# openGemini/openGemini

Measured on NVIDIA H100. Metric: decoded+aggregated rows/s, higher is better.
Workload: dtype f64

## Files before the change

include/ogpu.h:

```cpp
#ifndef OGPU_H
#define OGPU_H

#include <stddef.h>
#include <stdint.h>

#ifdef __cplusplus
extern "C" {
#endif

#define OG_API __attribute__((visibility("default")))

enum {
    OG_OK = 0,
    OG_EOF = 1,
    OG_E_INVAL = -1,
    OG_E_CUDA = -2,
    OG_E_NOMEM = -3,
    OG_E_UNSUPPORTED = -4,
    OG_E_CORRUPT = -5,
    OG_E_ABORTED = -6,
    OG_E_TYPE = -7,
    OG_E_STATE = -8
};

enum { OG_TYPE_INT = 1, OG_TYPE_FLOAT = 3, OG_TYPE_STRING = 4, OG_TYPE_BOOL = 5 };

enum { OG_AGG_COUNT = 1, OG_AGG_SUM = 2, OG_AGG_MIN = 3, OG_AGG_MAX = 4, OG_AGG_FIRST = 5, OG_AGG_LAST = 6 };

enum { OG_F_TERM = 0, OG_F_AND = 1, OG_F_OR = 2 };
enum { OG_OP_LT = 0, OG_OP_LTE = 1, OG_OP_GT = 2, OG_OP_GTE = 3, OG_OP_EQ = 4, OG_OP_NEQ = 5 };

typedef struct og_filter_item {
    int32_t kind;
    int32_t column;
    int32_t op;
    int32_t const_is_float;
    double fval;
    int64_t ival;
} og_filter_item;

typedef struct og_call {
    int32_t func;
    int32_t column;
} og_call;

enum { OG_GROUP_ALL = 0, OG_GROUP_PER_SERIES = 1, OG_GROUP_MAP = 2 };
enum {
    OG_Q_STRICT_ORDER = 1u << 0
    ,
    OG_Q_NO_FUSED = 1u << 1
    ,
    OG_Q_NO_FAST = 1u << 2
    ,
    OG_Q_RESERVED_8 = 1u << 3
    ,
    OG_Q_QUERY_GRID = 1u << 4
};

typedef struct og_query_desc {
    int64_t interval;
    int64_t offset;
    int64_t tmin, tmax;
    int32_t ascending;
    uint32_t n_calls;
    const og_call *calls;
    uint32_t n_filter;
    const og_filter_item *filter;
    int32_t group_mode;
    uint32_t n_groups;
    const uint32_t *series_group;
    int32_t chunk_size;
    uint32_t flags;
} og_query_desc;

typedef struct og_column_desc {
    const char *name;
    int32_t type;
    const uint64_t *page_off;
    const uint32_t *page_len;
} og_column_desc;

enum {
    OG_SHARD_DEVICE_DATA = 1u << 0
};

typedef struct og_shard_desc {
    const uint8_t *data;
    uint64_t data_len;
    uint32_t n_series;
    const uint64_t *sids;
    const uint32_t *series_seg_begin;
    uint32_t n_segments;
    const int64_t *seg_tmin;
    const int64_t *seg_tmax;
    uint32_t n_columns;
    const og_column_desc *columns;
    const uint64_t *time_page_off;
    const uint32_t *time_page_len;
    uint32_t flags;
} og_shard_desc;

typedef struct og_colval_view {
    const uint8_t *val;
    uint64_t val_bytes;
    const uint8_t *bitmap;
    const int64_t *times;
    int32_t type;
    int32_t len;
    int32_t nil_count;
    int32_t bitmap_offset;
} og_colval_view;

typedef struct og_record_view {
    uint32_t n_cols;
    const og_colval_view *cols;
    const int64_t *times;
    int32_t rows;
    uint32_t group;
    uint64_t sid;
} og_record_view;

typedef struct og_dense_col {
    void *values;
    uint8_t *valid;
    int64_t *times;
    int32_t type;
    int32_t func;
} og_dense_col;

typedef struct og_dense_view {
    uint32_t n_groups;
    uint32_t n_buckets;
    int64_t start;
    int64_t interval;
    uint32_t n_cols;
    const og_dense_col *cols;
    void *stream;
} og_dense_view;

typedef struct og_stats {
    uint64_t rows_decoded;
    uint64_t segments_scanned;
    uint64_t page_bytes;
    uint64_t dir_bytes;
    uint64_t out_bytes;
    double kernel_ms;
    double h2d_ms;
    double main_kernel_ms;
    uint32_t kernel_launches;
    int32_t path;
    int32_t il_state;
    int32_t per_series_cells_used;
    double il_build_ms;
    uint64_t il_bytes;
    uint64_t general_segments;
    double merge_ms;
    uint64_t il_packed_segments;
} og_stats;

typedef struct og_shard og_shard;
typedef struct og_query og_query;

OG_API int og_init(int device_ordinal);
OG_API int og_device_count(void);
OG_API const char *og_strerror(int status);
OG_API const char *og_last_error(void);
OG_API const char *og_version(void);
OG_API int og_release_cached_memory(void);

typedef struct og_tssp og_tssp;
OG_API int og_tssp_parse(const uint8_t *file, uint64_t len, og_tssp **out);
OG_API int og_tssp_desc(const og_tssp *t, og_shard_desc *out);
OG_API const char *og_tssp_measurement(const og_tssp *t);
OG_API int og_tssp_time_range(const og_tssp *t, int64_t *min_time, int64_t *max_time);
OG_API void og_tssp_free(og_tssp *t);

OG_API int og_shard_open(const og_shard_desc *desc, og_shard **out);
OG_API void og_shard_close(og_shard *s);
OG_API int og_shard_info(const og_shard *s, uint64_t *n_series, uint64_t *n_segments, uint64_t *n_rows,
                         uint64_t *page_bytes, int64_t *tmin, int64_t *tmax);

enum { OG_FILE_OUT_OF_ORDER = 1u << 0 };
OG_API int og_shard_open_files(const og_shard_desc *files, const uint32_t *file_flags, uint32_t n_files, og_shard **out);
typedef struct og_merge_info {
    uint32_t n_files, n_out_of_order_files;
    uint64_t series_merged;
    uint64_t out_of_order_rows;
    uint64_t rows_replaced;
    uint64_t rows_after_merge;
    uint64_t segments_kept;
    uint64_t segments_rewritten_in, segments_rewritten_out;
    double merge_ms;
} og_merge_info;
OG_API int og_shard_merge_info(const og_shard *s, og_merge_info *out);

OG_API int og_shard_append_files(og_shard *s, const og_shard_desc *files, const uint32_t *file_flags, uint32_t n_files);

OG_API int og_query_create(og_shard *s, const og_query_desc *desc, og_query **out);
OG_API int og_query_run(og_query *q);
OG_API int og_query_next(og_query *q, og_record_view *out);
OG_API int og_query_dense(og_query *q, og_dense_view *out);
OG_API int og_query_stats(const og_query *q, og_stats *out);
OG_API void og_query_abort(og_query *q);
OG_API void og_query_destroy(og_query *q);

OG_API int og_query_merge_dense(og_query *q, const og_dense_view *other);

typedef struct og_comm og_comm;
OG_API int og_comm_unique_id(uint8_t id[128]);
OG_API int og_comm_init_rank(const uint8_t id[128], int rank, int world, og_comm **out);
OG_API void og_comm_destroy(og_comm *c);
OG_API int og_comm_info(const og_comm *c, int *rank, int *world, int *nccl_version);
OG_API int og_comm_allreduce_f64(og_comm *c, double *vals, int n, int op_max);
OG_API int og_query_allreduce(og_query *q, og_comm *c);

OG_API int og_decode_segment(og_shard *s, uint32_t segment, og_record_view *out);
enum { OG_DECODE_DESCENDING = 1u << 0 };
OG_API int og_decode_segment_ex(og_shard *s, uint32_t segment, uint32_t flags, og_record_view *out);
OG_API int og_decode_column_device(og_shard *s, uint32_t column, uint32_t seg_begin, uint32_t seg_end,
                                   void *d_values, uint64_t value_stride_bytes, uint32_t *d_rows_out);

enum { OG_SYNTH_F_HI = 0, OG_SYNTH_F_LO = 1, OG_SYNTH_INT_WALK = 2, OG_SYNTH_BOOL = 3 };
typedef struct og_synth_column {
    int32_t type;
    int32_t dist;
    uint32_t null_permille;
} og_synth_column;
typedef struct og_synth_desc {
    uint32_t n_series;
    uint32_t rows_per_series;
    uint32_t rows_per_segment;
    int64_t t0;
    int64_t dt;
    uint64_t seed;
    uint32_t n_columns;
    const og_synth_column *columns;
    uint32_t series_base;
} og_synth_desc;
OG_API int og_shard_synth(const og_synth_desc *desc, og_shard **out);
typedef struct og_shard_layout {
    uint64_t data_len;
    uint32_t n_series, n_segments, n_columns;
} og_shard_layout;
OG_API int og_shard_layout_get(const og_shard *s, og_shard_layout *out);
OG_API int og_shard_export(const og_shard *s, uint8_t *data, uint64_t *sids, uint32_t *series_seg_begin,
                           int64_t *seg_tmin, int64_t *seg_tmax, uint64_t *page_off ,
                           uint32_t *page_len, int32_t *col_types );

OG_API int og_encode_pages(int32_t type, int32_t is_time, const void *d_values, const uint8_t *d_valid,
                           const uint32_t *d_rows , uint32_t n_segments,
                           uint32_t rows_per_segment, uint8_t *d_out, uint64_t out_cap, uint64_t *d_page_off,
                           uint32_t *d_page_len, uint64_t *total_bytes_out);

typedef struct og_downsampled og_downsampled;
OG_API int og_downsample(og_shard *s, uint32_t column, int64_t interval, int64_t tmin, int64_t tmax, og_downsampled **out);

typedef struct og_downsample_ops {
    int32_t type;
    uint32_t n_funcs;
    const int32_t *funcs;
} og_downsample_ops;
typedef struct og_downsample_desc {
    int64_t interval, tmin, tmax;
    uint32_t n_types;
    const og_downsample_ops *ops;
} og_downsample_desc;
OG_API int og_downsample_shard(og_shard *s, const og_downsample_desc *d, og_downsampled **out);
OG_API int og_downsampled_timing(const og_downsampled *d, double phase_ms[4]);
OG_API int og_downsampled_desc(const og_downsampled *d, og_shard_desc *desc, uint64_t *rows );
OG_API int og_downsampled_export(const og_downsampled *d, uint8_t *host_data );
OG_API void og_downsampled_free(og_downsampled *d);

typedef struct og_tssp_write_desc {
    const char *measurement;
    uint32_t series_begin, series_end;
    uint32_t flags;
} og_tssp_write_desc;
typedef struct og_tssp_image og_tssp_image;
OG_API int og_shard_write_tssp(og_shard *s, const og_tssp_write_desc *d, og_tssp_image **out);
OG_API int og_tssp_image_size(const og_tssp_image *f, uint64_t *bytes);
OG_API int og_tssp_image_export(const og_tssp_image *f, uint8_t *host);
OG_API int og_tssp_image_timing(const og_tssp_image *f, double phase_ms[4]);
OG_API void og_tssp_image_free(og_tssp_image *f);

#ifdef __cplusplus
}
#endif
#endif
```

opengemini_b200/_lib.py:

```python
import ctypes as C
import os

_HERE = os.path.dirname(os.path.abspath(__file__))
LIB_PATH = os.environ.get("OGPU_LIB") or os.path.join(_HERE, "libogpu.so")

OG_OK, OG_EOF = 0, 1
OG_E_INVAL, OG_E_CUDA, OG_E_NOMEM, OG_E_UNSUPPORTED, OG_E_CORRUPT, OG_E_ABORTED, OG_E_TYPE, OG_E_STATE = -1, -2, -3, -4, -5, -6, -7, -8
TYPE_INT, TYPE_FLOAT, TYPE_STRING, TYPE_BOOL = 1, 3, 4, 5
AGG_COUNT, AGG_SUM, AGG_MIN, AGG_MAX, AGG_FIRST, AGG_LAST = 1, 2, 3, 4, 5, 6
F_TERM, F_AND, F_OR = 0, 1, 2
OP_LT, OP_LTE, OP_GT, OP_GTE, OP_EQ, OP_NEQ = 0, 1, 2, 3, 4, 5
GROUP_ALL, GROUP_PER_SERIES, GROUP_MAP = 0, 1, 2
Q_STRICT_ORDER = 1
Q_NO_FUSED = 2
Q_NO_FAST = 4
Q_QUERY_GRID = 16
SYNTH_F_HI, SYNTH_F_LO, SYNTH_INT_WALK, SYNTH_BOOL = 0, 1, 2, 3
SHARD_DEVICE_DATA = 1
FILE_OUT_OF_ORDER = 1

u8p, u32p, u64p, i64p, i32p = C.POINTER(C.c_uint8), C.POINTER(C.c_uint32), C.POINTER(C.c_uint64), C.POINTER(C.c_int64), C.POINTER(C.c_int32)


class FilterItem(C.Structure):
    _fields_ = [("kind", C.c_int32), ("column", C.c_int32), ("op", C.c_int32), ("const_is_float", C.c_int32),
                ("fval", C.c_double), ("ival", C.c_int64)]


class Call(C.Structure):
    _fields_ = [("func", C.c_int32), ("column", C.c_int32)]


class QueryDesc(C.Structure):
    _fields_ = [("interval", C.c_int64), ("offset", C.c_int64), ("tmin", C.c_int64), ("tmax", C.c_int64),
                ("ascending", C.c_int32), ("n_calls", C.c_uint32), ("calls", C.POINTER(Call)),
                ("n_filter", C.c_uint32), ("filter", C.POINTER(FilterItem)), ("group_mode", C.c_int32),
                ("n_groups", C.c_uint32), ("series_group", u32p), ("chunk_size", C.c_int32), ("flags", C.c_uint32)]


class ColumnDesc(C.Structure):
    _fields_ = [("name", C.c_char_p), ("type", C.c_int32), ("page_off", u64p), ("page_len", u32p)]


class ShardDesc(C.Structure):
    _fields_ = [("data", u8p), ("data_len", C.c_uint64), ("n_series", C.c_uint32), ("sids", u64p),
                ("series_seg_begin", u32p), ("n_segments", C.c_uint32), ("seg_tmin", i64p), ("seg_tmax", i64p),
                ("n_columns", C.c_uint32), ("columns", C.POINTER(ColumnDesc)), ("time_page_off", u64p),
                ("time_page_len", u32p), ("flags", C.c_uint32)]


class ColValView(C.Structure):
    _fields_ = [("val", u8p), ("val_bytes", C.c_uint64), ("bitmap", u8p), ("times", i64p), ("type", C.c_int32),
                ("len", C.c_int32), ("nil_count", C.c_int32), ("bitmap_offset", C.c_int32)]


class RecordView(C.Structure):
    _fields_ = [("n_cols", C.c_uint32), ("cols", C.POINTER(ColValView)), ("times", i64p), ("rows", C.c_int32),
                ("group", C.c_uint32), ("sid", C.c_uint64)]


class DenseCol(C.Structure):
    _fields_ = [("values", C.c_void_p), ("valid", C.c_void_p), ("times", C.c_void_p), ("type", C.c_int32), ("func", C.c_int32)]


class DenseView(C.Structure):
    _fields_ = [("n_groups", C.c_uint32), ("n_buckets", C.c_uint32), ("start", C.c_int64), ("interval", C.c_int64),
                ("n_cols", C.c_uint32), ("cols", C.POINTER(DenseCol)), ("stream", C.c_void_p)]


class Stats(C.Structure):
    _fields_ = [("rows_decoded", C.c_uint64), ("segments_scanned", C.c_uint64), ("page_bytes", C.c_uint64),
                ("dir_bytes", C.c_uint64), ("out_bytes", C.c_uint64), ("kernel_ms", C.c_double), ("h2d_ms", C.c_double), ("main_kernel_ms", C.c_double),
                ("kernel_launches", C.c_uint32), ("path", C.c_int32), ("il_state", C.c_int32), ("per_series_cells_used", C.c_int32),
                ("il_build_ms", C.c_double), ("il_bytes", C.c_uint64), ("general_segments", C.c_uint64), ("merge_ms", C.c_double),
                ("il_packed_segments", C.c_uint64)]


class SynthColumn(C.Structure):
    _fields_ = [("type", C.c_int32), ("dist", C.c_int32), ("null_permille", C.c_uint32)]


class SynthDesc(C.Structure):
    _fields_ = [("n_series", C.c_uint32), ("rows_per_series", C.c_uint32), ("rows_per_segment", C.c_uint32),
                ("t0", C.c_int64), ("dt", C.c_int64), ("seed", C.c_uint64), ("n_columns", C.c_uint32),
                ("columns", C.POINTER(SynthColumn)), ("series_base", C.c_uint32)]


class ShardLayout(C.Structure):
    _fields_ = [("data_len", C.c_uint64), ("n_series", C.c_uint32), ("n_segments", C.c_uint32), ("n_columns", C.c_uint32)]


class DownsampleOps(C.Structure):
    _fields_ = [("type", C.c_int32), ("n_funcs", C.c_uint32), ("funcs", i32p)]


class DownsampleDesc(C.Structure):
    _fields_ = [("interval", C.c_int64), ("tmin", C.c_int64), ("tmax", C.c_int64), ("n_types", C.c_uint32),
                ("ops", C.POINTER(DownsampleOps))]


class MergeInfo(C.Structure):
    _fields_ = [("n_files", C.c_uint32), ("n_out_of_order_files", C.c_uint32), ("series_merged", C.c_uint64),
                ("out_of_order_rows", C.c_uint64), ("rows_replaced", C.c_uint64), ("rows_after_merge", C.c_uint64),
                ("segments_kept", C.c_uint64), ("segments_rewritten_in", C.c_uint64), ("segments_rewritten_out", C.c_uint64),
                ("merge_ms", C.c_double)]


class TsspWriteDesc(C.Structure):
    _fields_ = [("measurement", C.c_char_p), ("series_begin", C.c_uint32), ("series_end", C.c_uint32), ("flags", C.c_uint32)]


EXPORTS = [
    "og_init", "og_device_count", "og_strerror", "og_last_error", "og_version", "og_shard_open", "og_shard_close",
    "og_shard_info", "og_query_create", "og_query_run", "og_query_next", "og_query_dense", "og_query_stats",
    "og_query_abort", "og_query_destroy", "og_query_merge_dense", "og_decode_segment", "og_decode_segment_ex", "og_decode_column_device",
    "og_shard_synth", "og_shard_layout_get", "og_shard_export", "og_encode_pages",
    "og_release_cached_memory", "og_comm_unique_id", "og_comm_init_rank", "og_comm_destroy", "og_comm_info", "og_comm_allreduce_f64", "og_query_allreduce",
    "og_downsample", "og_downsampled_desc", "og_downsampled_export", "og_downsampled_free",
    "og_downsample_shard", "og_downsampled_timing",
    "og_tssp_parse", "og_tssp_desc", "og_tssp_measurement", "og_tssp_time_range", "og_tssp_free",
    "og_shard_open_files", "og_shard_merge_info", "og_shard_append_files",
    "og_shard_write_tssp", "og_tssp_image_size", "og_tssp_image_export", "og_tssp_image_timing", "og_tssp_image_free",
]

_lib = None


class OgpuError(RuntimeError):
    def __init__(self, status, where):
        self.status = status
        msg = lib().og_last_error().decode(errors="replace")
        super().__init__(f"{where}: {lib().og_strerror(status).decode()} ({status}) {msg}")


def lib():
    global _lib
    if _lib is not None:
        return _lib
    if not os.path.exists(LIB_PATH):
        raise RuntimeError(f"{LIB_PATH} is missing: run `python -c 'import __graft_entry__ as g; g.build()'` "
                           "(nvcc, sm_90a). There is no CPU fallback for the scan/aggregate path.")
    L = C.CDLL(LIB_PATH)
    L.og_strerror.restype = C.c_char_p
    L.og_strerror.argtypes = [C.c_int]
    L.og_last_error.restype = C.c_char_p
    L.og_version.restype = C.c_char_p
    L.og_init.argtypes = [C.c_int]
    L.og_shard_open.argtypes = [C.POINTER(ShardDesc), C.POINTER(C.c_void_p)]
    L.og_shard_open_files.argtypes = [C.POINTER(ShardDesc), u32p, C.c_uint32, C.POINTER(C.c_void_p)]
    L.og_shard_merge_info.argtypes = [C.c_void_p, C.POINTER(MergeInfo)]
    L.og_shard_append_files.argtypes = [C.c_void_p, C.POINTER(ShardDesc), u32p, C.c_uint32]
    L.og_shard_close.argtypes = [C.c_void_p]
    L.og_shard_close.restype = None
    L.og_shard_info.argtypes = [C.c_void_p, u64p, u64p, u64p, u64p, i64p, i64p]
    L.og_query_create.argtypes = [C.c_void_p, C.POINTER(QueryDesc), C.POINTER(C.c_void_p)]
    L.og_query_run.argtypes = [C.c_void_p]
    L.og_query_next.argtypes = [C.c_void_p, C.POINTER(RecordView)]
    L.og_query_dense.argtypes = [C.c_void_p, C.POINTER(DenseView)]
    L.og_query_stats.argtypes = [C.c_void_p, C.POINTER(Stats)]
    L.og_query_abort.argtypes = [C.c_void_p]
    L.og_query_abort.restype = None
    L.og_query_destroy.argtypes = [C.c_void_p]
    L.og_query_destroy.restype = None
    L.og_query_merge_dense.argtypes = [C.c_void_p, C.POINTER(DenseView)]
    L.og_decode_segment.argtypes = [C.c_void_p, C.c_uint32, C.POINTER(RecordView)]
    L.og_downsample.argtypes = [C.c_void_p, C.c_uint32, C.c_int64, C.c_int64, C.c_int64, C.POINTER(C.c_void_p)]
    L.og_downsample_shard.argtypes = [C.c_void_p, C.POINTER(DownsampleDesc), C.POINTER(C.c_void_p)]
    L.og_downsampled_timing.argtypes = [C.c_void_p, C.POINTER(C.c_double)]
    L.og_downsampled_desc.argtypes = [C.c_void_p, C.POINTER(ShardDesc), C.POINTER(C.c_uint64)]
    L.og_downsampled_export.argtypes = [C.c_void_p, C.c_void_p]
    L.og_downsampled_free.argtypes = [C.c_void_p]
    L.og_downsampled_free.restype = None
    L.og_tssp_parse.argtypes = [C.c_void_p, C.c_uint64, C.POINTER(C.c_void_p)]
    L.og_tssp_desc.argtypes = [C.c_void_p, C.POINTER(ShardDesc)]
    L.og_tssp_measurement.argtypes = [C.c_void_p]
    L.og_tssp_measurement.restype = C.c_char_p
    L.og_tssp_time_range.argtypes = [C.c_void_p, C.POINTER(C.c_int64), C.POINTER(C.c_int64)]
    L.og_tssp_free.argtypes = [C.c_void_p]
    L.og_tssp_free.restype = None
    L.og_shard_write_tssp.argtypes = [C.c_void_p, C.POINTER(TsspWriteDesc), C.POINTER(C.c_void_p)]
    L.og_tssp_image_size.argtypes = [C.c_void_p, u64p]
    L.og_tssp_image_export.argtypes = [C.c_void_p, C.c_void_p]
    L.og_tssp_image_timing.argtypes = [C.c_void_p, C.POINTER(C.c_double)]
    L.og_tssp_image_free.argtypes = [C.c_void_p]
    L.og_tssp_image_free.restype = None
    L.og_decode_segment_ex.argtypes = [C.c_void_p, C.c_uint32, C.c_uint32, C.POINTER(RecordView)]
    L.og_decode_column_device.argtypes = [C.c_void_p, C.c_uint32, C.c_uint32, C.c_uint32, C.c_void_p, C.c_uint64, C.c_void_p]
    L.og_shard_synth.argtypes = [C.POINTER(SynthDesc), C.POINTER(C.c_void_p)]
    L.og_shard_layout_get.argtypes = [C.c_void_p, C.POINTER(ShardLayout)]
    L.og_shard_export.argtypes = [C.c_void_p, C.c_void_p, C.c_void_p, C.c_void_p, C.c_void_p, C.c_void_p, C.c_void_p, C.c_void_p, C.c_void_p]
    L.og_encode_pages.argtypes = [C.c_int32, C.c_int32, C.c_void_p, C.c_void_p, C.c_void_p, C.c_uint32, C.c_uint32,
                                  C.c_void_p, C.c_uint64, C.c_void_p, C.c_void_p, u64p]
    L.og_comm_unique_id.argtypes = [C.c_void_p]
    L.og_comm_init_rank.argtypes = [C.c_void_p, C.c_int, C.c_int, C.POINTER(C.c_void_p)]
    L.og_comm_destroy.argtypes = [C.c_void_p]
    L.og_comm_destroy.restype = None
    L.og_comm_info.argtypes = [C.c_void_p, C.POINTER(C.c_int), C.POINTER(C.c_int), C.POINTER(C.c_int)]
    L.og_comm_allreduce_f64.argtypes = [C.c_void_p, C.POINTER(C.c_double), C.c_int, C.c_int]
    L.og_query_allreduce.argtypes = [C.c_void_p, C.c_void_p]
    _lib = L
    return L


def check(status, where):
    if status != OG_OK:
        raise OgpuError(status, where)
```

opengemini_b200/csrc/agg_kernels.cuh:

```cuda
#pragma once
#include "agg_ops.cuh"
#include "decode.cuh"
#include "internal.h"

namespace ogpu {

#define OG_NO_BUCKET 0xFFFFFFFFu

struct DirP {
    const uint8_t *data;
    const uint64_t *page_off;
    const uint32_t *page_len;
    const uint32_t *seg_series, *seg_rows, *series_seg_begin;
    const int64_t *seg_tmin, *seg_tmax;
    uint32_t n_segments, n_columns;
};

struct ChunkP {
    uint32_t series_begin, series_end;
    uint32_t seg_begin, seg_end;
    Tri cells[OG_MAX_CALLS];
    uint32_t nb;
    Tri edges[OG_MAX_CALLS];
    uint32_t *edge_bucket;
    Tri gcells[OG_MAX_CALLS];
    uint32_t gc_cols, gc_tail0, gc_edge0, gc_col0;
    uint32_t J;
    int *err;
    int *flags;
};

__device__ __forceinline__ size_t cell_idx(const ChunkP &ch, uint32_t series, uint32_t b) { return (size_t)(series - ch.series_begin) * ch.nb + b; }

__device__ __forceinline__ void report_err(int *err, int code, uint32_t seg) {
    if (atomicCAS(&err[0], 0, code) == 0) err[1] = (int)seg;
}

__device__ __forceinline__ void store_part(const Tri &a, size_t i, const Part &p) {
    a.val[i] = p.v; a.ok[i] = (uint8_t)p.ok;
    if (a.tim) a.tim[i] = p.t;
}
__device__ __forceinline__ Part load_part(const Tri &a, size_t i) {
    Part p; p.ok = a.ok[i]; p.v = a.val[i]; p.t = a.tim ? a.tim[i] : 0; return p;
}
__device__ __forceinline__ void store_cell(const ChunkP &ch, int call, uint32_t series, uint32_t b, const Part &p) {
    store_part(ch.cells[call], cell_idx(ch, series, b), p);
    ch.flags[0] = 1;
}

struct SegWindows {
    const QueryP &q; const ChunkP &ch;
    const uint32_t seg; const size_t e; const uint32_t series;
    uint32_t cur_b = OG_NO_BUCKET, head_b = OG_NO_BUCKET; bool head_done = false;
    int64_t we = 0;

    __device__ __forceinline__ SegWindows(const QueryP &q_, const ChunkP &ch_, uint32_t seg_, size_t e_, uint32_t series_)
        : q(q_), ch(ch_), seg(seg_), e(e_), series(series_) {}
    template <int NC> __device__ __forceinline__ void flush(const Part (&parts)[NC], bool final) {
        if (cur_b == OG_NO_BUCKET) return;
#pragma unroll
        for (int c = 0; c < NC; c++) {
            if (!head_done) store_part(ch.edges[c], e, parts[c]);
            else if (final) store_part(ch.edges[c], e + 1, parts[c]);
            else if (parts[c].ok) store_cell(ch, c, series, cur_b, parts[c]);
        }
        if (!head_done) { head_done = true; head_b = cur_b; }
    }
    template <int NC> __device__ __forceinline__ bool enter(int64_t t, Part (&parts)[NC]) {
        if (cur_b != OG_NO_BUCKET && t < we) return true;
        flush(parts, false);
        cur_b = bucket_of(t, q.start, q.interval);
        if (cur_b >= q.n_buckets) { report_err(ch.err, D_CORRUPT, seg); cur_b = OG_NO_BUCKET; return false; }
        we = q.start + (int64_t)(cur_b + 1) * q.interval;
#pragma unroll
        for (int c = 0; c < NC; c++) parts[c] = part_empty();
        return true;
    }
    template <int NC> __device__ __forceinline__ void end(const Part (&parts)[NC]) {
        const uint32_t last_b = cur_b;
        const bool single = !head_done;
        flush(parts, true);
        ch.edge_bucket[e] = head_b;
        ch.edge_bucket[e + 1] = (single || head_b == OG_NO_BUCKET) ? OG_NO_BUCKET : last_b;
        if (head_b != OG_NO_BUCKET) ch.flags[1] = 1;
    }
};

__global__ void k_validate(DirP d, const int32_t *col_types, uint32_t *seg_rows, unsigned long long *totals ,
                           uint32_t *max_rows, int *err) {
    uint32_t seg = blockIdx.x * blockDim.x + threadIdx.x;
    if (seg >= d.n_segments) return;
    size_t ti = (size_t)d.n_columns * d.n_segments + seg;
    TimeDesc t;
    int rc = parse_time_page(d.data + d.page_off[ti], d.page_len[ti], t);
    if (rc == D_OK && t.rows == 0) rc = D_CORRUPT;
    if (rc == D_OK) {
        int64_t last = t.t0; bool unsorted = false;
        if (t.kind == 0) last = (int64_t)((uint64_t)t.t0 + (uint64_t)(t.rows - 1) * t.delta);
        else {
            TimeIter it; it.init(t);
            for (uint32_t i = 0; i < t.rows; i++) { const int64_t x = it.next(); unsorted |= x < last; last = x; }
            it.finish(); rc = it.err;
        }
        if (rc == D_OK && (t.t0 < d.seg_tmin[seg] || last > d.seg_tmax[seg] || last < t.t0 || unsorted)) rc = D_CORRUPT;
    }
    if (rc != D_OK) { report_err(err, rc, seg); seg_rows[seg] = 0; return; }
    seg_rows[seg] = t.rows;
    unsigned long long bytes = d.page_len[ti];
    for (uint32_t c = 0; c < d.n_columns; c++) {
        size_t pi = (size_t)c * d.n_segments + seg;
        uint32_t len = d.page_len[pi];
        if (len == 0) continue;
        bytes += len;
        PageHdr h;
        rc = parse_field_header(d.data + d.page_off[pi], len, col_types[c], t.rows, h);
        if (rc == D_OK && h.rows != t.rows) rc = D_CORRUPT;
        if (rc == D_OK && h.bitmap && hdr_valid_rows(h) != h.rows - h.nil_count) rc = D_CORRUPT;
        if (rc == D_OK && !h.one_row && h.nil_count < h.rows) {
            if (h.block_len < 1) rc = D_CORRUPT;
            else {
                int tag = __ldg(h.block) >> 4, ty = col_types[c];
                if (ty == OG_TYPE_FLOAT) rc = (tag == 0 || tag == 3 || tag == 4 || tag == 5) ? D_OK : (tag == 1 || tag == 2 || tag == 6) ? D_UNSUPPORTED : D_CORRUPT;
                else if (ty == OG_TYPE_INT) rc = (tag == 1 || tag == 2 || tag == 4) ? D_OK : tag == 3 ? D_UNSUPPORTED : D_CORRUPT;
                else if (ty == OG_TYPE_BOOL) rc = tag == 1 ? D_OK : D_CORRUPT;
                else if (ty == OG_TYPE_STRING) rc = D_OK;
                else rc = D_UNSUPPORTED;
            }
        }
        if (rc != D_OK) { report_err(err, rc, seg); return; }
    }
    atomicAdd(&totals[0], (unsigned long long)t.rows);
    atomicAdd(&totals[1], bytes);
    atomicMax(max_rows, t.rows);
    if (t.kind != 0 && t.kind != 3) atomicAdd(&totals[2], 1ull);
}

__global__ void k_fill_seg_series(const uint32_t *series_seg_begin, uint32_t n_series, uint32_t *seg_series) {
    uint32_t s = blockIdx.x;
    if (s >= n_series) return;
    for (uint32_t g = series_seg_begin[s] + threadIdx.x; g < series_seg_begin[s + 1]; g += blockDim.x) seg_series[g] = s;
}

struct TileP {
    uint32_t tile_begin, tile_end, R;
    uint32_t S;
    uint64_t *vals[OG_MAX_COLS];
    uint8_t *okb[OG_MAX_COLS];
    int64_t *times;
    uint8_t *keep;
};

__global__ void k_decode_tile(DirP d, QueryP q, TileP tp, int *err) {
    uint32_t seg = tp.tile_begin + blockIdx.x * blockDim.x + threadIdx.x;
    if (seg >= tp.tile_end) return;
    uint32_t slot = blockIdx.y;
    const size_t base = seg - tp.tile_begin, S = tp.S;
    uint32_t rows = d.seg_rows[seg];
    if (slot == q.n_cols) {
        size_t ti = (size_t)d.n_columns * d.n_segments + seg;
        TimeDesc t;
        int rc = parse_time_page(d.data + d.page_off[ti], d.page_len[ti], t);
        if (rc == D_OK) {
            TimeIter it; it.init(t);
            for (uint32_t i = 0; i < t.rows; i++) tp.times[base + i * S] = it.next();
            it.finish(); rc = it.err;
        }
        if (rc != D_OK) report_err(err, rc, seg);
        return;
    }
    size_t pi = (size_t)q.col_index[slot] * d.n_segments + seg;
    uint64_t *out = tp.vals[slot] + base; uint8_t *okb = tp.okb[slot] + base;
    ColIter it;
    it.init(d.data + d.page_off[pi], d.page_len[pi], q.col_type[slot], rows);
    for (uint32_t i = 0; i < rows; i++) { uint64_t v = 0; okb[i * S] = it.next(v); out[i * S] = v; }
    it.finish();
    if (it.err != D_OK) report_err(err, it.err, seg);
}

__device__ __forceinline__ bool term_pass(const FilterP &f, uint64_t raw) {
    if (f.type == OG_TYPE_FLOAT || (f.type == OG_TYPE_INT && f.const_is_float)) {
        double v = f.type == OG_TYPE_FLOAT ? u2d(raw) : (double)(int64_t)raw;
        double c = f.const_is_float ? f.fval : (double)f.ival;
        switch (f.op) {
        case OG_OP_LT: return !(v >= c);
        case OG_OP_LTE: return !(v > c);
        case OG_OP_GT: return !(v <= c);
        case OG_OP_GTE: return !(v < c);
        case OG_OP_EQ: return !(v != c);
        default: return !(v == c);
        }
    }
    int64_t v = f.type == OG_TYPE_BOOL ? (int64_t)(raw != 0) : (int64_t)raw, c = f.ival;
    switch (f.op) {
    case OG_OP_LT: return !(v >= c);
    case OG_OP_LTE: return !(v > c);
    case OG_OP_GT: return !(v <= c);
    case OG_OP_GTE: return !(v < c);
    case OG_OP_EQ: return !(v != c);
    default: return !(v == c);
    }
}

__global__ void k_filter_tile(DirP d, QueryP q, TileP tp) {
    size_t idx = (size_t)blockIdx.x * blockDim.x + threadIdx.x;
    size_t total = (size_t)tp.S * tp.R;
    if (idx >= total) return;
    uint32_t row = (uint32_t)(idx / tp.S), sl = (uint32_t)(idx % tp.S);
    if (sl >= tp.tile_end - tp.tile_begin) return;
    if (row >= d.seg_rows[tp.tile_begin + sl]) { tp.keep[idx] = 0; return; }
    int64_t t = tp.times[idx];
    bool keep = t >= q.tmin && t <= q.tmax;
    if (keep && q.n_filter) {
        uint32_t stack = 0; int sp = 0;
        for (uint32_t i = 0; i < q.n_filter; i++) {
            const FilterP &f = q.filter[i];
            if (f.kind == OG_F_TERM) {
                bool pass = tp.okb[f.col_slot][idx] && term_pass(f, tp.vals[f.col_slot][idx]);
                stack |= (uint32_t)pass << sp; sp++;
            } else {
                uint32_t b = (stack >> (sp - 1)) & 1, a = (stack >> (sp - 2)) & 1;
                uint32_t r = f.kind == OG_F_AND ? (a & b) : (a | b);
                sp -= 2; stack &= ~(3u << sp); stack |= r << sp; sp++;
            }
        }
        keep = stack & 1;
    }
    tp.keep[idx] = keep;
}

__global__ void k_window_reduce(DirP d, QueryP q, TileP tp, ChunkP ch) {
    uint32_t sl = blockIdx.x * blockDim.x + threadIdx.x;
    uint32_t seg = tp.tile_begin + sl;
    if (seg >= tp.tile_end) return;
    const uint32_t rows = d.seg_rows[seg], series = d.seg_series[seg];
    const size_t S = tp.S, e = 2 * (size_t)(seg - ch.seg_begin);
    Part parts[OG_MAX_CALLS];
    uint32_t cur_b = OG_NO_BUCKET, head_b = OG_NO_BUCKET; bool head_done = false;
    int64_t we = 0;
    auto flush = [&](bool final) {
        if (cur_b == OG_NO_BUCKET) return;
        for (uint32_t c = 0; c < q.n_calls; c++) {
            if (!head_done) store_part(ch.edges[c], e, parts[c]);
            else if (final) store_part(ch.edges[c], e + 1, parts[c]);
            else if (parts[c].ok) store_cell(ch, (int)c, series, cur_b, parts[c]);
        }
        if (!head_done) { head_done = true; head_b = cur_b; }
    };
    for (uint32_t r = 0; r < rows; r++) {
        const size_t ix = (size_t)r * S + sl;
        const int64_t t = tp.times[ix];
        if (t < q.tmin) continue;
        if (t > q.tmax) break;
        if (cur_b == OG_NO_BUCKET || t >= we) {
            flush(false);
            cur_b = bucket_of(t, q.start, q.interval);
            if (cur_b >= q.n_buckets) { report_err(ch.err, D_CORRUPT, seg); cur_b = OG_NO_BUCKET; break; }
            we = q.start + (int64_t)(cur_b + 1) * q.interval;
#pragma unroll
            for (uint32_t c = 0; c < OG_MAX_CALLS; c++) parts[c] = part_empty();
        }
        if (!tp.keep[ix]) continue;
#pragma unroll
        for (uint32_t c = 0; c < OG_MAX_CALLS; c++) {
            if (c >= q.n_calls) break;
            const CallP &cp = q.calls[c];
            if (tp.okb[cp.col_slot][ix]) acc_row(cp.func, cp.type, parts[c], tp.vals[cp.col_slot][ix], t);
        }
    }
    flush(true);
    ch.edge_bucket[e] = head_b;
    ch.edge_bucket[e + 1] = (head_b == OG_NO_BUCKET || cur_b == head_b) ? OG_NO_BUCKET : cur_b;
}

struct EdgeRuns { uint32_t hb, tb, s_end; bool head_leader; };
__device__ __forceinline__ EdgeRuns edge_runs(const DirP &d, const ChunkP &ch, uint32_t seg, uint32_t series) {
    EdgeRuns r;
    const uint32_t s_first = d.series_seg_begin[series];
    r.s_end = d.series_seg_begin[series + 1];
    const uint32_t *eb = ch.edge_bucket;
    const size_t e = 2 * (size_t)(seg - ch.seg_begin);
    r.hb = eb[e]; r.tb = eb[e + 1];
    r.head_leader = true;
    if (r.hb != OG_NO_BUCKET && seg > s_first) {
        const size_t pe = e - 2;
        const uint32_t pb = eb[pe + 1] != OG_NO_BUCKET ? eb[pe + 1] : eb[pe];
        if (pb != OG_NO_BUCKET && pb == r.hb) r.head_leader = false;
    }
    return r;
}
__device__ __forceinline__ Part edge_stitch(const QueryP &q, const ChunkP &ch, const EdgeRuns &r, uint32_t seg, int which, uint32_t c) {
    const CallP &cp = q.calls[c];
    const uint32_t *eb = ch.edge_bucket;
    const size_t e = 2 * (size_t)(seg - ch.seg_begin);
    const uint32_t b = which == 0 ? r.hb : r.tb;
    Part acc = load_part(ch.edges[c], e + which);
    if (which == 1 || r.tb == OG_NO_BUCKET) {
        for (uint32_t nx = seg + 1; nx < r.s_end; nx++) {
            const size_t ne = 2 * (size_t)(nx - ch.seg_begin);
            if (eb[ne] != b) break;
            acc = series_merge(cp.func, cp.type, acc, load_part(ch.edges[c], ne));
            if (eb[ne + 1] != OG_NO_BUCKET) break;
        }
    }
    return acc;
}

__global__ void k_fix_edges(DirP d, QueryP q, ChunkP ch) {
    uint32_t seg = ch.seg_begin + blockIdx.x * blockDim.x + threadIdx.x;
    if (seg >= ch.seg_end) return;
    const uint32_t series = d.seg_series[seg];
    const EdgeRuns r = edge_runs(d, ch, seg, series);
    if (r.hb == OG_NO_BUCKET) return;
    for (int which = 0; which < 2; which++) {
        if (which == 0 && !r.head_leader) continue;
        if (which == 1 && r.tb == OG_NO_BUCKET) continue;
        const uint32_t b = which == 0 ? r.hb : r.tb;
        if (b >= q.n_buckets) { report_err(ch.err, D_CORRUPT, seg); continue; }
        for (uint32_t c = 0; c < q.n_calls; c++) {
            const Part acc = edge_stitch(q, ch, r, seg, which, c);
            if (acc.ok) store_cell(ch, (int)c, series, b, acc);
        }
    }
}

__device__ __forceinline__ Part shfl_xor_part(const Part &p, int o, bool with_time) {
    Part r; r.v = __shfl_xor_sync(0xffffffffu, p.v, o); r.ok = __shfl_xor_sync(0xffffffffu, p.ok, o);
    r.t = with_time ? __shfl_xor_sync(0xffffffffu, p.t, o) : 0;
    return r;
}
__device__ __forceinline__ Part warp_fold(int func, int type, bool multi, Part p, bool with_time) {
#pragma unroll
    for (int o = 16; o; o >>= 1) { const Part other = shfl_xor_part(p, o, with_time); group_update(func, type, multi, p, other); }
    return p;
}
__device__ __forceinline__ bool call_has_time(const QueryP &q, uint32_t c) { return q.calls[c].func >= OG_AGG_MIN && !(q.multi && q.calls[c].func <= OG_AGG_MAX); }
__device__ __forceinline__ int call_ftype(const QueryP &q, uint32_t c) { return q.calls[c].func == OG_AGG_COUNT ? OG_TYPE_INT : q.calls[c].type; }

__global__ void k_fix_edges_fold(DirP d, QueryP q, ChunkP ch) {
    if (ch.flags[1] == 0) return;
    const uint32_t w = (blockIdx.x * blockDim.x + threadIdx.x) >> 5, lane = threadIdx.x & 31;
    const uint32_t n_blk = (ch.series_end - ch.series_begin + 31) / 32;
    if (w >= n_blk * ch.J) return;
    const uint32_t blk = w / ch.J, j = w % ch.J;
    const uint32_t series = ch.series_begin + blk * 32 + lane;
    const bool in = series < ch.series_end;
    const uint32_t seg = in ? d.series_seg_begin[series] + j : 0;
    EdgeRuns r; r.hb = r.tb = OG_NO_BUCKET; r.head_leader = false; r.s_end = 0;
    if (in) r = edge_runs(d, ch, seg, series);
    const uint32_t n_bk = (ch.gc_cols - ch.gc_edge0) / 3;
    for (int which = 0; which < 2; which++) {
        const uint32_t gcol = ch.gc_edge0 + (which ? 2u : (j & 1u)) * n_bk + ch.series_begin / 32 + blk - ch.gc_col0;
        const bool has = r.hb != OG_NO_BUCKET && (which == 0 ? r.head_leader : r.tb != OG_NO_BUCKET);
        const uint32_t b = which == 0 ? r.hb : r.tb;
        const uint32_t hm = __ballot_sync(0xffffffffu, has);
        if (hm == 0) continue;
        const int leader = __ffs(hm) - 1;
        const uint32_t bL = __shfl_sync(0xffffffffu, b, leader);
        const bool unif = __all_sync(0xffffffffu, !has || b == bL) && bL < q.n_buckets;
        if (!unif && has && b >= q.n_buckets) { report_err(ch.err, D_CORRUPT, seg); continue; }
        for (uint32_t c = 0; c < q.n_calls; c++) {
            Part acc = part_empty();
            if (has) acc = edge_stitch(q, ch, r, seg, which, c);
            if (unif) {
                acc = warp_fold(q.calls[c].func, call_ftype(q, c), q.multi != 0, acc, call_has_time(q, c));
                if ((int)lane == leader && acc.ok) store_part(ch.gcells[c], (size_t)bL * ch.gc_cols + gcol, acc);
            } else if (has && acc.ok) store_cell(ch, (int)c, series, b, acc);
        }
    }
}

struct GroupP {
    const uint32_t *grp_begin;
    const uint32_t *grp_series;
    uint32_t n_groups;
    Tri dense[OG_MAX_CALLS];
};

__global__ void k_merge_groups(QueryP q, ChunkP ch, GroupP gp) {
    if (ch.flags[0] == 0) return;
    size_t idx = (size_t)blockIdx.x * blockDim.x + threadIdx.x;
    size_t total = (size_t)gp.n_groups * q.n_buckets;
    if (idx >= total) return;
    uint32_t g = (uint32_t)(idx / q.n_buckets), b = (uint32_t)(idx % q.n_buckets);
    uint32_t lo = gp.grp_begin[g], hi = gp.grp_begin[g + 1];
    {
        uint32_t a = lo, z = hi;
        while (a < z) { uint32_t m = (a + z) >> 1; if (gp.grp_series[m] < ch.series_begin) a = m + 1; else z = m; }
        lo = a;
    }
    if (lo >= hi || gp.grp_series[lo] >= ch.series_end) return;
    {
        const uint32_t c = blockIdx.y;
        const CallP &cp = q.calls[c];
        Part acc = load_part(gp.dense[c], idx);
        const Tri cells = ch.cells[c];
        constexpr int U = 16;
        for (uint32_t i = lo; i < hi; i += U) {
            uint32_t okv[U]; uint64_t vv[U]; int64_t tt[U];
#pragma unroll
            for (int u = 0; u < U; u++) {
                uint32_t ii = i + u;
                uint32_t s = ii < hi ? gp.grp_series[ii] : 0xffffffffu;
                bool in = s < ch.series_end;
                size_t ci = in ? cell_idx(ch, s, b) : 0;
                okv[u] = in ? cells.ok[ci] : 0;
                vv[u] = okv[u] ? cells.val[ci] : 0;
                tt[u] = (okv[u] && cells.tim) ? cells.tim[ci] : 0;
            }
#pragma unroll
            for (int u = 0; u < U; u++) {
                if (!okv[u]) continue;
                Part p; p.ok = 1; p.v = vv[u]; p.t = tt[u];
                group_update(cp.func, cp.out_type == OG_TYPE_INT && cp.func == OG_AGG_COUNT ? OG_TYPE_INT : cp.type, q.multi != 0, acc, p);
            }
        }
        store_part(gp.dense[c], idx, acc);
    }
}

__global__ void k_merge_per_series(QueryP q, ChunkP ch, GroupP gp) {
    const uint32_t c = blockIdx.y;
    const size_t n = (size_t)(ch.series_end - ch.series_begin) * q.n_buckets;
    const size_t i = (size_t)blockIdx.x * blockDim.x + threadIdx.x;
    if (i >= n) return;
    const CallP &cp = q.calls[c];
    const int ftype = cp.out_type == OG_TYPE_INT && cp.func == OG_AGG_COUNT ? OG_TYPE_INT : cp.type;
    const uint32_t b = (uint32_t)(i % q.n_buckets);
    Part p; p.ok = ch.cells[c].ok[i]; p.v = p.ok ? ch.cells[c].val[i] : 0; p.t = (p.ok && ch.cells[c].tim) ? ch.cells[c].tim[i] : 0;
    Part a; a.v = 0; a.ok = 0; a.t = q.multi ? 0 : q.start + (int64_t)b * q.interval;
    group_update(cp.func, ftype, q.multi != 0, a, p);
    store_part(gp.dense[c], (size_t)ch.series_begin * q.n_buckets + i, a);
}

#define OG_MERGE_SB 256u
__global__ void __launch_bounds__(128) k_merge_all_blocks(QueryP q, ChunkP ch, GroupP gp) {
    if (ch.flags[0] == 0) return;
    const uint32_t b = blockIdx.x * blockDim.x + threadIdx.x, blk = blockIdx.y, c = blockIdx.z;
    if (b >= q.n_buckets) return;
    const uint32_t nS = ch.series_end - ch.series_begin;
    const uint32_t s0 = blk * OG_MERGE_SB, s1 = min(nS, s0 + OG_MERGE_SB);
    const int func = q.calls[c].func, ftype = call_ftype(q, c);
    const bool multi = q.multi != 0;
    const Tri cells = ch.cells[c];
    Part acc = part_empty();
    constexpr int U = 8;
    for (uint32_t s = s0; s < s1; s += U) {
        uint32_t okv[U]; uint64_t vv[U]; int64_t tt[U];
#pragma unroll
        for (int u = 0; u < U; u++) {
            const bool in = s + u < s1;
            const size_t ci = in ? (size_t)(s + u) * ch.nb + b : 0;
            okv[u] = in ? cells.ok[ci] : 0;
            vv[u] = okv[u] ? cells.val[ci] : 0;
            tt[u] = (okv[u] && cells.tim) ? cells.tim[ci] : 0;
        }
#pragma unroll
        for (int u = 0; u < U; u++) {
            if (!okv[u]) continue;
            Part p; p.ok = 1; p.v = vv[u]; p.t = tt[u];
            group_update(func, ftype, multi, acc, p);
        }
    }
    if (acc.ok) store_part(ch.gcells[c], (size_t)b * ch.gc_cols + blk, acc);
}

__global__ void k_merge_folded(QueryP q, ChunkP ch, GroupP gp) {
    const uint32_t b = (blockIdx.x * blockDim.x + threadIdx.x) >> 5, lane = threadIdx.x & 31, c = blockIdx.y;
    if (b >= q.n_buckets) return;
    const int func = q.calls[c].func, ftype = call_ftype(q, c);
    const bool wt = call_has_time(q, c), multi = q.multi != 0;
    const Tri g = ch.gcells[c];
    Part acc = part_empty();
    const size_t row = (size_t)b * ch.gc_cols;
    for (uint32_t col = lane; col < ch.gc_cols; col += 32) {
        if (!g.ok[row + col]) continue;
        Part p; p.ok = 1; p.v = g.val[row + col]; p.t = wt ? g.tim[row + col] : 0;
        group_update(func, ftype, multi, acc, p);
    }
    acc = warp_fold(func, ftype, multi, acc, wt);
    if (lane == 0 && acc.ok) {
        Part a = load_part(gp.dense[c], b);
        group_update(func, ftype, multi, a, acc);
        store_part(gp.dense[c], b, a);
    }
}

__global__ void k_init_dense(QueryP q, GroupP gp) {
    size_t idx = (size_t)blockIdx.x * blockDim.x + threadIdx.x;
    size_t total = (size_t)gp.n_groups * q.n_buckets;
    if (idx >= total) return;
    uint32_t b = (uint32_t)(idx % q.n_buckets);
    for (uint32_t c = 0; c < q.n_calls; c++) {
        gp.dense[c].val[idx] = 0; gp.dense[c].ok[idx] = 0;
        if (gp.dense[c].tim) gp.dense[c].tim[idx] = q.multi ? 0 : q.start + (int64_t)b * q.interval;
    }
}

__global__ void k_merge_dense(QueryP q, GroupP mine, GroupP other) {
    size_t idx = (size_t)blockIdx.x * blockDim.x + threadIdx.x;
    size_t total = (size_t)mine.n_groups * q.n_buckets;
    if (idx >= total) return;
    for (uint32_t c = 0; c < q.n_calls; c++) {
        const CallP &cp = q.calls[c];
        Part a = load_part(mine.dense[c], idx), p = load_part(other.dense[c], idx);
        group_update(cp.func, cp.func == OG_AGG_COUNT ? OG_TYPE_INT : cp.type, q.multi != 0, a, p);
        store_part(mine.dense[c], idx, a);
    }
}

}
```

opengemini_b200/csrc/api.cu:

```cuda
#include <algorithm>
#include <cstdarg>
#include <cstdio>
#include <cstring>
#include <numeric>

#include "agg_kernels.cuh"
#include "il_build.cuh"
#include "fused_multi.cuh"
#include "fused_cols.cuh"
#include "snappy_load.cuh"
#include <cub/device/device_scan.cuh>
#include <cub/device/device_radix_sort.cuh>
#include "internal.h"

namespace ogpu {

static thread_local char g_err[512] = "";
void set_error(const char *fmt, ...) {
    va_list ap; va_start(ap, fmt); vsnprintf(g_err, sizeof g_err, fmt, ap); va_end(ap);
}
int cuda_fail(cudaError_t e, const char *what, const char *file, int line) {
    set_error("CUDA error %d (%s) at %s:%d: %s", (int)e, cudaGetErrorString(e), file, line, what);
    return OG_E_CUDA;
}
// ... 247 lines not shown
}

OG_API int og_shard_export(const og_shard *s, uint8_t *data, uint64_t *sids, uint32_t *series_seg_begin, int64_t *seg_tmin,
                           int64_t *seg_tmax, uint64_t *page_off, uint32_t *page_len, int32_t *col_types) {
    if (!s) return OG_E_INVAL;
    CU(cudaSetDevice(s->device));
    size_t nseg = s->n_segments, ncol1 = (size_t)s->n_columns + 1;
    if (data) CU(cudaMemcpy(data, s->d_data, s->data_len, cudaMemcpyDeviceToHost));
    if (sids) memcpy(sids, s->sids.data(), s->sids.size() * 8);
    if (series_seg_begin) memcpy(series_seg_begin, s->h_series_seg_begin.data(), s->h_series_seg_begin.size() * 4);
    if (seg_tmin) CU(cudaMemcpy(seg_tmin, s->d_tmin, nseg * 8, cudaMemcpyDeviceToHost));
    if (seg_tmax) CU(cudaMemcpy(seg_tmax, s->d_tmax, nseg * 8, cudaMemcpyDeviceToHost));
    if (page_off) CU(cudaMemcpy(page_off, s->d_page_off, ncol1 * nseg * 8, cudaMemcpyDeviceToHost));
    if (page_len) CU(cudaMemcpy(page_len, s->d_page_len, ncol1 * nseg * 4, cudaMemcpyDeviceToHost));
    if (col_types) memcpy(col_types, s->col_types.data(), s->col_types.size() * 4);
    return OG_OK;
}

static const int64_t MIN_TIME = INT64_MIN + 2, MAX_TIME = INT64_MAX - 1;
static void window_of(int64_t interval, int64_t offset, int64_t tmin, int64_t tmax, int64_t t, int64_t *s, int64_t *e) {
    if (interval == 0) { *s = tmin; *e = tmax + 1; return; }
    t -= offset;
    int64_t dt = t % interval;
    if (dt < 0) dt += interval;
    int64_t st = ((int64_t)((uint64_t)MIN_TIME + (uint64_t)dt) >= t) ? MIN_TIME : t - dt;
    st += offset;
    int64_t d2 = interval - dt;
    int64_t en = (MAX_TIME - d2 <= t) ? MAX_TIME : t + d2;
    en += offset;
    *s = st; *e = en;
}
static bool window_clamped(int64_t interval, int64_t offset, int64_t t) {
    const __int128 x = (__int128)t - offset;
    __int128 r = x % interval;
    if (r < 0) r += interval;
    const __int128 s = x - r, e = s + interval;
    return s < MIN_TIME || e > MAX_TIME || s + offset < INT64_MIN || e + offset > INT64_MAX;
}

}
namespace { void free_plan(void *plan); }
extern "C" void og_query_free_merge_state(void *p);
og_query::~og_query() {
    if (stream) cudaStreamSynchronize(stream);
    if (live) { std::lock_guard<std::mutex> lock(live->mu); live->n--; }
    og_query_free_merge_state(merge_state);
    free_plan(plan);
    if (ev0) cudaEventDestroy(ev0);
    if (ev1) cudaEventDestroy(ev1);
    for (cudaEvent_t e : main_ev) cudaEventDestroy(e);
    if (stream) cudaStreamDestroy(stream);
}
extern "C" {
OG_API void og_query_destroy(og_query *q) { delete q; }

OG_API int og_query_create(og_shard *s, const og_query_desc *d_in, og_query **out) {
    if (!s || !d_in || !out) { set_error("null argument"); return OG_E_INVAL; }
    *out = nullptr;
    og_query_desc d_clamped = *d_in;
    d_clamped.tmin = std::max(d_in->tmin, MIN_TIME); d_clamped.tmax = std::min(d_in->tmax, MAX_TIME);
    const og_query_desc *d = &d_clamped;
    CU(cudaSetDevice(s->device));
    if (d->n_calls == 0 || d->n_calls > OG_MAX_CALLS) { set_error("n_calls must be 1..%d", OG_MAX_CALLS); return OG_E_INVAL; }
    if (d->n_filter > OG_MAX_FILTER) { set_error("filter too long (max %d items)", OG_MAX_FILTER); return OG_E_INVAL; }
    if (d->interval < 0 || d->tmin > d->tmax) { set_error("bad interval or time range"); return OG_E_INVAL; }
    std::unique_ptr<og_query> q(new og_query);
    {
        std::lock_guard<std::mutex> lock(s->live->mu);
        s->live->n++;
        q->sh = s; q->live = s->live;
    }
    q->desc = *d;
    q->calls.assign(d->calls, d->calls + d->n_calls);
    if (d->n_filter) q->filter.assign(d->filter, d->filter + d->n_filter);
    q->desc.calls = q->calls.data(); q->desc.filter = q->filter.data();
    QueryP &p = q->qp;
    memset(&p, 0, sizeof p);
    auto slot_of = [&](int col) -> int {
        for (uint32_t i = 0; i < p.n_cols; i++) if (p.col_index[i] == col) return (int)i;
        if (p.n_cols >= OG_MAX_COLS) return -1;
        p.col_index[p.n_cols] = col; p.col_type[p.n_cols] = s->col_types[col];
        return (int)p.n_cols++;
    };
    for (uint32_t i = 0; i < d->n_calls; i++) {
        const og_call &c = d->calls[i];
        if (c.column < 0 || (uint32_t)c.column >= s->n_columns || c.func < OG_AGG_COUNT || c.func > OG_AGG_LAST) { set_error("call %u: bad column or function", i); return OG_E_INVAL; }
        int type = s->col_types[c.column];
        if (type == OG_TYPE_STRING && c.func != OG_AGG_COUNT) { set_error("call %u: only count() is pushed down for string columns (their values are never decoded on the GPU path)", i); return OG_E_UNSUPPORTED; }
        if (c.func == OG_AGG_SUM && type == OG_TYPE_BOOL) { set_error("sum() over a boolean column (unsupported sum iterator type, series_call_processor.go:140)"); return OG_E_INVAL; }
        int sl = slot_of(c.column);
        if (sl < 0) { set_error("too many distinct columns"); return OG_E_INVAL; }
        p.calls[i].func = c.func; p.calls[i].col_slot = sl; p.calls[i].type = type;
        p.calls[i].out_type = c.func == OG_AGG_COUNT ? OG_TYPE_INT : type;
    }
    p.n_calls = d->n_calls; p.multi = d->n_calls > 1;
    int sp = 0;
    for (uint32_t i = 0; i < d->n_filter; i++) {
        const og_filter_item &f = d->filter[i];
        FilterP &fp = p.filter[i];
        fp.kind = f.kind;
        if (f.kind == OG_F_TERM) {
            if (f.column < 0 || (uint32_t)f.column >= s->n_columns || f.op < OG_OP_LT || f.op > OG_OP_NEQ) { set_error("filter item %u: bad column or op", i); return OG_E_INVAL; }
            if (s->col_types[f.column] == OG_TYPE_STRING) { set_error("filter item %u: WHERE on a string column is not pushed down", i); return OG_E_UNSUPPORTED; }
            int sl = slot_of(f.column);
            if (sl < 0) { set_error("too many distinct columns"); return OG_E_INVAL; }
            fp.col_slot = sl; fp.op = f.op; fp.type = s->col_types[f.column]; fp.const_is_float = f.const_is_float; fp.fval = f.fval; fp.ival = f.ival;
            sp++;
        } else if (f.kind == OG_F_AND || f.kind == OG_F_OR) {
            if (sp < 2) { set_error("filter RPN underflow at item %u", i); return OG_E_INVAL; }
            sp--;
        } else { set_error("filter item %u: bad kind", i); return OG_E_INVAL; }
    }
    if (d->n_filter && sp != 1) { set_error("filter RPN does not reduce to one value"); return OG_E_INVAL; }
    p.n_filter = d->n_filter;
    int64_t gmin = std::max(d->tmin, s->tmin), gmax = std::min(d->tmax, s->tmax);
    bool overlap = gmin <= gmax;
    if (!overlap) gmin = gmax = d->tmin;
    if (d->flags & OG_Q_QUERY_GRID) {
        if (d_in->tmin <= MIN_TIME || d_in->tmax >= MAX_TIME) { set_error("OG_Q_QUERY_GRID needs a bounded time range"); return OG_E_INVAL; }
        gmin = d->tmin; gmax = d->tmax; overlap = true;
    }
    int64_t s0, e0, s1, e1;
    if (d->interval == 0) { s0 = gmin; e0 = gmax + 1; s1 = s0; e1 = e0; }
    else {
        if (overlap && (window_clamped(d->interval, d->offset, gmin) || window_clamped(d->interval, d->offset, gmax))) {
            set_error("the first or last window of the range is clamped at the int64 time limits"); return OG_E_UNSUPPORTED;
        }
        window_of(d->interval, d->offset, d->tmin, d->tmax, gmin, &s0, &e0);
        window_of(d->interval, d->offset, d->tmin, d->tmax, gmax + 1, &s1, &e1);
    }
    p.tmin = d->tmin; p.tmax = d->tmax; p.start = s0; p.interval = e0 - s0;
    if (p.interval <= 0) { set_error("degenerate window"); return OG_E_INVAL; }
    uint64_t nb = d->interval ? (uint64_t)(e1 - s0) / (uint64_t)p.interval : 1;
    if (nb == 0 || nb > 0x7fffffffull) { set_error("query range yields %llu buckets", (unsigned long long)nb); return OG_E_INVAL; }
    p.n_buckets = (uint32_t)nb;
    q->n_groups = d->group_mode == OG_GROUP_ALL ? 1 : d->group_mode == OG_GROUP_PER_SERIES ? s->n_series : d->n_groups;
    if (d->group_mode == OG_GROUP_MAP) {
        if (!d->series_group || d->n_groups == 0) { set_error("OG_GROUP_MAP needs series_group and n_groups"); return OG_E_INVAL; }
        q->series_group.assign(d->series_group, d->series_group + s->n_series);
        for (uint32_t g : q->series_group) if (g >= d->n_groups) { set_error("series_group entry out of range"); return OG_E_INVAL; }
    } else if (d->group_mode != OG_GROUP_ALL && d->group_mode != OG_GROUP_PER_SERIES) { set_error("bad group_mode"); return OG_E_INVAL; }
    if (q->n_groups == 0) q->n_groups = 1;
    cudaError_t e = cudaStreamCreateWithFlags(&q->stream, cudaStreamNonBlocking);
    if (e != cudaSuccess) return cuda_fail(e, "cudaStreamCreate", __FILE__, __LINE__);
    cudaEventCreate(&q->ev0); cudaEventCreate(&q->ev1);
    *out = q.release();
    return OG_OK;
}

OG_API void og_query_abort(og_query *q) { if (q) q->aborted = 1; }

}
namespace {
struct Plan {
    ChunkP ch; TileP tp; GroupP gp;
    bool fused;
    bool cols;
    bool multi;
    bool fast;
    bool blockmerge;
    bool fold;
    int fm; bool times;
    IlP il;
    const og_shard::IlCol *ic;
};
void free_plan(void *plan) { delete (Plan *)plan; }

template <int NC> void launch_fused(const DirP &d, const QueryP &p, const ChunkP &ch, const uint32_t *list, uint32_t n, cudaStream_t st) {
    if (n) k_fused_segment<NC><<<(n + 127) / 128, 128, 0, st>>>(d, p, ch, list, n);
}
template <int FM, bool TIMES> void launch_fast_t(bool fold, const IlP &il, uint32_t g0, uint32_t g1, const QueryP &p, const ChunkP &ch, cudaStream_t st) {
    constexpr uint32_t WPB = OG_FAST_THREADS / 32;
    dim3 grid((g1 - g0 + WPB - 1) / WPB), block(OG_FAST_THREADS);
    if (fold) k_fused_il<FM, TIMES, true><<<grid, block, WPB * il_acc_bytes(p.n_calls, TIMES), st>>>(p, ch, il, g0, g1);
    else k_fused_il<FM, TIMES, false><<<grid, block, 0, st>>>(p, ch, il, g0, g1);
}
void launch_fast(int fm, bool times, bool fold, const IlP &il, uint32_t g0, uint32_t g1, const QueryP &p, const ChunkP &ch, cudaStream_t st) {
    if (g1 <= g0) return;
    if (!times) {
        switch (fm) {
        case FM_SUM | FM_COUNT: return launch_fast_t<FM_SUM | FM_COUNT, false>(fold, il, g0, g1, p, ch, st);
        case FM_SUM | FM_COUNT | FM_MAX: return launch_fast_t<FM_SUM | FM_COUNT | FM_MAX, false>(fold, il, g0, g1, p, ch, st);
        case FM_SUM | FM_COUNT | FM_MIN | FM_MAX: return launch_fast_t<FM_SUM | FM_COUNT | FM_MIN | FM_MAX, false>(fold, il, g0, g1, p, ch, st);
        case FM_COUNT: return launch_fast_t<FM_COUNT, false>(fold, il, g0, g1, p, ch, st);
        default: break;
        }
    } else {
        switch (fm) {
        case FM_MAX | FM_COUNT: return launch_fast_t<FM_MAX | FM_COUNT, true>(fold, il, g0, g1, p, ch, st);
        case FM_MIN | FM_COUNT: return launch_fast_t<FM_MIN | FM_COUNT, true>(fold, il, g0, g1, p, ch, st);
        default: break;
        }
    }
    return launch_fast_t<63, true>(fold, il, g0, g1, p, ch, st);
}

template <int NCOL, int NCALL> void launch_multi_t(const QueryP &p, const DirP &d, const ChunkP &ch, uint32_t nseg, cudaStream_t st) {
    bool simple = true;
    for (uint32_t c = 0; c < p.n_calls; c++) simple &= p.calls[c].func == OG_AGG_COUNT || p.calls[c].func == OG_AGG_SUM;
    const unsigned gb = (nseg + 127) / 128;
    if (simple) k_fused_multi<NCOL, NCALL, true><<<gb, 128, 0, st>>>(d, p, ch);
    else k_fused_multi<NCOL, NCALL, false><<<gb, 128, 0, st>>>(d, p, ch);
}
template <int NCOL> void launch_multi_c(const QueryP &p, const DirP &d, const ChunkP &ch, uint32_t nseg, cudaStream_t st) {
    switch (p.n_calls) {
    case 1: return launch_multi_t<NCOL, 1>(p, d, ch, nseg, st);
    case 2: return launch_multi_t<NCOL, 2>(p, d, ch, nseg, st);
    case 3: return launch_multi_t<NCOL, 3>(p, d, ch, nseg, st);
    case 4: return launch_multi_t<NCOL, 4>(p, d, ch, nseg, st);
    case 5: return launch_multi_t<NCOL, 5>(p, d, ch, nseg, st);
    case 6: return launch_multi_t<NCOL, 6>(p, d, ch, nseg, st);
    case 7: return launch_multi_t<NCOL, 7>(p, d, ch, nseg, st);
    default: return launch_multi_t<NCOL, 8>(p, d, ch, nseg, st);
    }
}
void launch_cols(const QueryP &p, const DirP &d, const ChunkP &ch, uint32_t nseg, cudaStream_t st) {
    bool simple = true;
    for (uint32_t c = 0; c < p.n_calls; c++) simple &= p.calls[c].func == OG_AGG_COUNT || p.calls[c].func == OG_AGG_SUM;
    const unsigned gb = (nseg + 127) / 128;
    if (simple) k_fused_cols<true><<<gb, 128, 0, st>>>(d, p, ch);
    else k_fused_cols<false><<<gb, 128, 0, st>>>(d, p, ch);
}
void launch_multi(const QueryP &p, const DirP &d, const ChunkP &ch, uint32_t nseg, cudaStream_t st) {
    switch (p.n_cols) {
    case 1: return launch_multi_c<1>(p, d, ch, nseg, st);
    case 2: return launch_multi_c<2>(p, d, ch, nseg, st);
    case 3: return launch_multi_c<3>(p, d, ch, nseg, st);
#ifdef OG_WIDE_MULTI
    case 5: return launch_multi_c<5>(p, d, ch, nseg, st);
    case 6: return launch_multi_c<6>(p, d, ch, nseg, st);
    case 7: return launch_multi_c<7>(p, d, ch, nseg, st);
    case 8: return launch_multi_c<8>(p, d, ch, nseg, st);
#endif
    default: return launch_multi_c<4>(p, d, ch, nseg, st);
    }
}

int ensure_il(og_shard *s, int col, cudaStream_t st) {
    std::lock_guard<std::mutex> lock(s->il_mu);
    if (s->il.size() != s->n_columns) s->il.resize(s->n_columns);
    og_shard::IlCol &ic = s->il[col];
    if (ic.state != 0) return OG_OK;
    ic.state = -1;
    if (s->n_segments == 0 || s->col_types[col] != OG_TYPE_FLOAT) return OG_OK;
    const uint32_t nseg = s->n_segments;
    uint32_t J = s->n_series ? s->h_series_seg_begin[1] - s->h_series_seg_begin[0] : 0;
    for (uint32_t i = 0; i < s->n_series && J; i++) if (s->h_series_seg_begin[i + 1] - s->h_series_seg_begin[i] != J) J = 0;
    const uint32_t n_super = J ? (s->n_series + OG_IL_SUPER - 1) / OG_IL_SUPER : 1;
    const uint64_t n_dom64 = J ? (uint64_t)n_super * J : 1;
    if (n_dom64 >= (1ull << 31)) return OG_OK;
    const uint32_t n_dom = (uint32_t)n_dom64;
    int rc;
    struct Ev { cudaEvent_t e = nullptr; Ev() { cudaEventCreate(&e); } ~Ev() { if (e) cudaEventDestroy(e); } } ev0, ev1;
    cudaEventRecord(ev0.e, st);
    Scratch tmp(st);
    IlScanOut so{};
    uint32_t *seg_words; uint64_t *keys2; uint32_t *vals2;
    if ((rc = tmp.get(&so.seg_win, nseg)) || (rc = tmp.get(&so.n_packed, 1)) ||
        (rc = tmp.get(&seg_words, nseg)) || (rc = tmp.get(&so.seg_t0, nseg)) || (rc = tmp.get(&so.seg_dt, nseg)) || (rc = tmp.get(&so.keys, nseg)) ||
        (rc = tmp.get(&so.vals, nseg)) || (rc = tmp.get(&keys2, nseg)) || (rc = tmp.get(&vals2, nseg)) || (rc = tmp.get(&so.dom_cnt, n_dom))) return rc;
    so.seg_words = seg_words;
    if ((rc = tmp.get(&so.misaligned, 1))) return rc;
    CU(cudaMemsetAsync(so.dom_cnt, 0, (size_t)n_dom * 4, st));
    CU(cudaMemsetAsync(so.misaligned, 0, 4, st));
    CU(cudaMemsetAsync(so.n_packed, 0, 8, st));
    DirP d = make_dir(s);
    k_il_scan<<<(nseg + 255) / 256, 256, 0, st>>>(d, col, s->col_types[col], J, so);
    CU(cudaGetLastError());
    int dbits = 1; while ((1ull << dbits) < n_dom64 + 1) dbits++;
    {
        size_t tb = 0;
        CU(cub::DeviceRadixSort::SortPairs(nullptr, tb, so.keys, keys2, so.vals, vals2, (int)nseg, 0, (int)OG_IL_WORD_BITS + dbits, st));
        void *dtmp; if ((rc = tmp.get((uint8_t **)&dtmp, tb))) return rc;
        CU(cub::DeviceRadixSort::SortPairs(dtmp, tb, so.keys, keys2, so.vals, vals2, (int)nseg, 0, (int)OG_IL_WORD_BITS + dbits, st));
    }
    std::vector<uint32_t> dom_cnt(n_dom); uint32_t misaligned = 1; unsigned long long n_packed = 0;
    CU(cudaMemcpyAsync(dom_cnt.data(), so.dom_cnt, (size_t)n_dom * 4, cudaMemcpyDeviceToHost, st));
    CU(cudaMemcpyAsync(&misaligned, so.misaligned, 4, cudaMemcpyDeviceToHost, st));
    CU(cudaMemcpyAsync(&n_packed, so.n_packed, 8, cudaMemcpyDeviceToHost, st));
    CU(cudaStreamSynchronize(st));
    std::vector<uint32_t> elem_first(n_dom), grp_first(n_dom);
    uint64_t n_elig = 0, ng64 = 0;
    for (uint32_t i = 0; i < n_dom; i++) { elem_first[i] = (uint32_t)n_elig; grp_first[i] = (uint32_t)ng64; n_elig += dom_cnt[i]; ng64 += (dom_cnt[i] + 31) / 32; }
    const uint32_t n_gen = nseg - (uint32_t)n_elig;
    if (n_gen) {
        if ((rc = dalloc(&ic.gen_list, (size_t)n_gen))) return rc;
        CU(cudaMemcpyAsync(ic.gen_list, vals2 + n_elig, (size_t)n_gen * 4, cudaMemcpyDeviceToDevice, st));
        ic.gen_host.resize(n_gen);
        CU(cudaMemcpyAsync(ic.gen_host.data(), vals2 + n_elig, (size_t)n_gen * 4, cudaMemcpyDeviceToHost, st));
        CU(cudaStreamSynchronize(st));
    }
    if (n_elig == 0) return OG_OK;
    const uint32_t ng = (uint32_t)ng64;
    ic.n_groups = ng; ic.J = J; ic.aligned = J != 0 && misaligned == 0; ic.n_super = n_super; ic.cols_per_super = OG_IL_SUPER / 32 + 1;
    ic.super_grp_first.assign(n_super + 1, ng);
    for (uint32_t sp = 0; sp < n_super; sp++) ic.super_grp_first[sp] = grp_first[J ? sp * J : 0];
    uint32_t *d_elem_first, *d_grp_first;
    if ((rc = tmp.get(&d_elem_first, n_dom)) || (rc = tmp.get(&d_grp_first, n_dom))) return rc;
    CU(cudaMemcpyAsync(d_elem_first, elem_first.data(), (size_t)n_dom * 4, cudaMemcpyHostToDevice, st));
    CU(cudaMemcpyAsync(d_grp_first, grp_first.data(), (size_t)n_dom * 4, cudaMemcpyHostToDevice, st));
    const size_t n_slots = (size_t)ng * 32;
    if ((rc = dalloc(&ic.lane_seg, n_slots)) || (rc = dalloc(&ic.lane_rows, n_slots)) || (rc = dalloc(&ic.lane_win, n_slots)) || (rc = dalloc(&ic.lane_series, n_slots)) ||
        (rc = dalloc(&ic.lane_t0, n_slots)) || (rc = dalloc(&ic.lane_dt, n_slots)) || (rc = dalloc(&ic.grp_col, (size_t)ng)) ||
        (rc = dalloc(&ic.grp_rows, (size_t)ng)) || (rc = dalloc(&ic.grp_off, (size_t)ng))) return rc;
    CU(cudaMemsetAsync(ic.lane_seg, 0xff, n_slots * 4, st));
    CU(cudaMemsetAsync(ic.lane_rows, 0, n_slots * 4, st));
    CU(cudaMemsetAsync(ic.lane_win, 0, n_slots * 2, st));
    IlAssign as{};
    as.keys = keys2; as.segs = vals2; as.elem_first = d_elem_first; as.grp_first = d_grp_first;
    as.seg_words = seg_words; as.seg_t0 = so.seg_t0; as.seg_dt = so.seg_dt; as.seg_win = so.seg_win;
    as.lane_seg = ic.lane_seg; as.lane_rows = ic.lane_rows; as.lane_series = ic.lane_series; as.grp_col = ic.grp_col; as.lane_win = ic.lane_win; as.lane_t0 = ic.lane_t0; as.lane_dt = ic.lane_dt;
    as.n_elig = (uint32_t)n_elig; as.J = J; as.cols_per_super = ic.cols_per_super;
    k_il_assign<<<(unsigned)((n_elig + 255) / 256), 256, 0, st>>>(d, as);
    k_il_group_rows<<<(unsigned)((n_slots + 255) / 256), 256, 0, st>>>(ng, ic.lane_seg, seg_words, ic.grp_rows);
    CU(cudaGetLastError());
    std::vector<uint32_t> gw(ng); std::vector<uint64_t> go(ng);
    CU(cudaMemcpyAsync(gw.data(), ic.grp_rows, (size_t)ng * 4, cudaMemcpyDeviceToHost, st));
    CU(cudaStreamSynchronize(st));
    uint64_t total = 0;
    for (uint32_t g = 0; g < ng; g++) { go[g] = total; total += (uint64_t)gw[g] * 32; }
    size_t free_b = 0, total_b = 0;
    CU(dev_mem_info(&free_b, &total_b));
    size_t headroom = (size_t)8 << 30;
    if (const char *ov = getenv("OGPU_IL_HEADROOM_MB")) headroom = (size_t)atoll(ov) << 20;
    if (total * 4 + headroom > free_b || dev_malloc((void **)&ic.words, total * 4) != cudaSuccess) {
        cudaGetLastError(); ic.words = nullptr; ic.state = -2;
        return OG_OK;
    }
    CU(cudaMemcpyAsync(ic.grp_off, go.data(), (size_t)ng * 8, cudaMemcpyHostToDevice, st));
    k_il_repack<<<(unsigned)((n_slots + 127) / 128), 128, 0, st>>>(d, col, ic.lane_seg, ic.lane_win, ic.grp_off, ic.grp_rows, ng, ic.words);
    CU(cudaGetLastError());
    cudaEventRecord(ev1.e, st);
    CU(cudaStreamSynchronize(st));
    float ms = 0; cudaEventElapsedTime(&ms, ev0.e, ev1.e);
    ic.n_words = total; ic.n_packed = n_packed; ic.build_ms = ms; ic.state = 1;
    return OG_OK;
}

int build_plan(og_query *q) {
    og_shard *s = q->sh;
    const QueryP &p = q->qp;
    cudaStream_t st = q->stream;
    int rc;
    Plan *pl = new Plan;
    memset((void *)pl, 0, sizeof *pl);
    q->plan = pl;
    size_t cells_dense = (size_t)q->n_groups * p.n_buckets;
    for (uint32_t c = 0; c < p.n_calls; c++) {
        bool sel = p.calls[c].func >= OG_AGG_MIN && !(p.multi && p.calls[c].func <= OG_AGG_MAX);
        if ((rc = q->bufs.get(&q->dense[c].val, cells_dense))) return rc;
        if ((rc = q->bufs.get(&q->dense[c].ok, cells_dense))) return rc;
        if (sel && (rc = q->bufs.get(&q->dense[c].tim, cells_dense))) return rc;
    }
    std::vector<uint32_t> grp_begin(q->n_groups + 1, 0), grp_series(s->n_series);
    if (q->desc.group_mode == OG_GROUP_MAP) {
        for (uint32_t sr = 0; sr < s->n_series; sr++) grp_begin[q->series_group[sr] + 1]++;
        for (uint32_t g = 0; g < q->n_groups; g++) grp_begin[g + 1] += grp_begin[g];
        std::vector<uint32_t> cur(grp_begin.begin(), grp_begin.end() - 1);
        for (uint32_t sr = 0; sr < s->n_series; sr++) grp_series[cur[q->series_group[sr]]++] = sr;
    } else if (q->desc.group_mode == OG_GROUP_PER_SERIES) {
        for (uint32_t g = 0; g <= q->n_groups; g++) grp_begin[g] = std::min(g, s->n_series);
        std::iota(grp_series.begin(), grp_series.end(), 0u);
    } else { grp_begin[1] = s->n_series; std::iota(grp_series.begin(), grp_series.end(), 0u); }
    uint32_t *d_grp_begin, *d_grp_series;
    if ((rc = q->bufs.get(&d_grp_begin, grp_begin.size()))) return rc;
    if ((rc = q->bufs.get(&d_grp_series, grp_series.size()))) return rc;
    if ((rc = q->bufs.get(&q->d_err, 16))) return rc;
    CU(cudaMemcpyAsync(d_grp_begin, grp_begin.data(), grp_begin.size() * 4, cudaMemcpyHostToDevice, st));
    CU(cudaMemcpyAsync(d_grp_series, grp_series.data(), grp_series.size() * 4, cudaMemcpyHostToDevice, st));
    CU(cudaStreamSynchronize(st));
    pl->gp.grp_begin = d_grp_begin; pl->gp.grp_series = d_grp_series; pl->gp.n_groups = q->n_groups;
    for (uint32_t c = 0; c < p.n_calls; c++) pl->gp.dense[c] = q->dense[c];

    bool has_string = false;
    for (uint32_t k = 0; k < p.n_cols; k++) has_string |= p.col_type[k] == OG_TYPE_STRING;
    pl->fused = p.n_cols == 1 && p.n_filter == 0 && !has_string && !(q->desc.flags & OG_Q_NO_FUSED);
    const bool multi_ok = !pl->fused && (has_string || !(q->desc.flags & OG_Q_NO_FUSED));
    pl->cols = false;
    if (multi_ok && !(q->desc.flags & OG_Q_NO_FAST) && s->irregular_time_pages == 0 && s->max_seg_rows <= OG_COLS_MAXROWS &&
        (p.n_filter == 0 || (p.n_filter == 1 && p.filter[0].kind == OG_F_TERM)) && !getenv("OGPU_NO_COLS")) {
        pl->cols = true;
        for (uint32_t k = 0; k < p.n_cols; k++) {
            int n = 0;
            for (uint32_t c = 0; c < p.n_calls; c++) n += p.calls[c].col_slot == (int)k;
            if (n > OG_COLS_MAXMINE) pl->cols = false;
        }
    }
    if (has_string && !pl->cols && p.n_cols > OG_MULTI_MAXC) { set_error("a query that counts a string column may touch at most %d columns on this shard", OG_MULTI_MAXC); return OG_E_UNSUPPORTED; }
    pl->multi = pl->cols || (multi_ok && p.n_cols <= OG_MULTI_MAXC);
    q->path_used = pl->fused ? 1 : pl->cols ? 5 : pl->multi ? 4 : 0;
    const bool want_fast = pl->fused && p.col_type[0] == OG_TYPE_FLOAT && !(q->desc.flags & OG_Q_NO_FAST) && s->n_segments;
    if (want_fast && (rc = ensure_il(s, p.col_index[0], st))) return rc;
    pl->fast = want_fast && s->il[p.col_index[0]].state == 1;
    const og_shard::IlCol *ic = pl->fast ? &s->il[p.col_index[0]] : nullptr;
    pl->ic = ic;
    pl->fold = pl->fast && ic->J != 0 && ic->aligned && q->desc.group_mode == OG_GROUP_ALL && !(q->desc.flags & OG_Q_STRICT_ORDER);

    size_t cell_bytes_per_series = 0;
    for (uint32_t c = 0; c < p.n_calls; c++) cell_bytes_per_series += (size_t)p.n_buckets * (9 + (p.calls[c].func >= OG_AGG_MIN ? 8 : 0));
    size_t free_b = 0, total_b = 0;
    CU(dev_mem_info(&free_b, &total_b));
    size_t budget = std::min<size_t>(free_b / 3, (size_t)24 << 30);
    q->chunk_series = (uint32_t)std::max<size_t>(1, std::min<size_t>(s->n_series, budget / std::max<size_t>(1, cell_bytes_per_series)));
    if (const char *ov = getenv("OGPU_CHUNK_SERIES")) {
        long v = atol(ov);
        if (v > 0) q->chunk_series = (uint32_t)std::min<long>(v, (long)std::max<uint32_t>(1, s->n_series));
    }
    if (q->chunk_series < s->n_series) {
        if (q->chunk_series >= OG_IL_SUPER) q->chunk_series = q->chunk_series / OG_IL_SUPER * OG_IL_SUPER;
        else q->chunk_series = std::max<uint32_t>(32, q->chunk_series & ~31u);
    }
    uint32_t max_chunk_segs = 0;
    for (uint32_t a = 0; a < s->n_series; a += q->chunk_series) {
        uint32_t b = std::min(s->n_series, a + q->chunk_series);
        max_chunk_segs = std::max(max_chunk_segs, s->h_series_seg_begin[b] - s->h_series_seg_begin[a]);
    }
    ChunkP &ch = pl->ch;
    ch.err = q->d_err; ch.flags = q->d_err + 2;
    ch.nb = p.n_buckets;
    ch.J = ic ? ic->J : 0;
    size_t chunk_cells = (size_t)std::min(q->chunk_series, s->n_series) * p.n_buckets;
    for (uint32_t c = 0; c < p.n_calls; c++) {
        bool sel = p.calls[c].func >= OG_AGG_MIN;
        if ((rc = q->bufs.get(&ch.cells[c].val, chunk_cells))) return rc;
        if ((rc = q->bufs.get(&ch.cells[c].ok, chunk_cells))) return rc;
        if (sel && (rc = q->bufs.get(&ch.cells[c].tim, chunk_cells))) return rc;
        if ((rc = q->bufs.get(&ch.edges[c].val, 2 * (size_t)max_chunk_segs))) return rc;
        if ((rc = q->bufs.get(&ch.edges[c].ok, 2 * (size_t)max_chunk_segs))) return rc;
        if (sel && (rc = q->bufs.get(&ch.edges[c].tim, 2 * (size_t)max_chunk_segs))) return rc;
    }
    if ((rc = q->bufs.get(&ch.edge_bucket, 2 * (size_t)max_chunk_segs))) return rc;
    pl->blockmerge = !pl->fold && q->desc.group_mode == OG_GROUP_ALL && !(q->desc.flags & OG_Q_STRICT_ORDER) &&
                     (s->n_series > 2 * OG_MERGE_SB || getenv("OGPU_FORCE_BLOCKMERGE") );
    if (pl->blockmerge) {
        ch.gc_edge0 = 0; ch.gc_col0 = 0;
        ch.gc_cols = (std::min(q->chunk_series, s->n_series) + OG_MERGE_SB - 1) / OG_MERGE_SB;
        const size_t n = (size_t)p.n_buckets * ch.gc_cols;
        for (uint32_t c = 0; c < p.n_calls; c++) {
            bool sel = p.calls[c].func >= OG_AGG_MIN;
            if ((rc = q->bufs.get(&ch.gcells[c].val, n))) return rc;
            if ((rc = q->bufs.get(&ch.gcells[c].ok, n))) return rc;
            if (sel && (rc = q->bufs.get(&ch.gcells[c].tim, n))) return rc;
        }
    }
    if (pl->fold) {
        ch.gc_tail0 = ic->n_super * ic->cols_per_super; ch.gc_edge0 = 2 * ch.gc_tail0; ch.gc_col0 = 0;
        ch.gc_cols = ch.gc_edge0 + 3 * ((s->n_series + 31) / 32);
        const size_t n = (size_t)p.n_buckets * ch.gc_cols;
        for (uint32_t c = 0; c < p.n_calls; c++) {
            bool sel = p.calls[c].func >= OG_AGG_MIN;
            if ((rc = q->bufs.get(&ch.gcells[c].val, n))) return rc;
            if ((rc = q->bufs.get(&ch.gcells[c].ok, n))) return rc;
            if (sel && (rc = q->bufs.get(&ch.gcells[c].tim, n))) return rc;
        }
    }
    if (pl->fast) {
        pl->il.words = ic->words; pl->il.grp_off = ic->grp_off; pl->il.grp_rows = ic->grp_rows; pl->il.grp_col = ic->grp_col;
        pl->il.lane_seg = ic->lane_seg; pl->il.lane_rows = ic->lane_rows; pl->il.lane_win = ic->lane_win; pl->il.lane_series = ic->lane_series; pl->il.lane_t0 = ic->lane_t0; pl->il.lane_dt = ic->lane_dt;
        pl->fm = 0; pl->times = false;
        for (uint32_t c = 0; c < p.n_calls; c++) {
            pl->fm |= 1 << (p.calls[c].func - 1);
            if (p.calls[c].func >= OG_AGG_MIN && !(p.multi && p.calls[c].func <= OG_AGG_MAX)) pl->times = true;
        }
        pl->fm |= FM_COUNT;
        q->path_used = pl->fold ? 3 : 2;
    }
    if (!pl->fused && !pl->multi) {
        TileP &tp = pl->tp;
        tp.R = std::max<uint32_t>(1, s->max_seg_rows);
        size_t per_seg = (size_t)tp.R * (p.n_cols * 9 + 8 + 1);
        size_t fb = 0, tb = 0;
        CU(dev_mem_info(&fb, &tb));
        const size_t tile_budget = std::max<size_t>((size_t)96 << 20, std::min<size_t>(fb / 4, (size_t)12 << 30));
        q->tile_segs = (uint32_t)std::max<size_t>(1, std::min<size_t>(std::max<uint32_t>(1, max_chunk_segs), tile_budget / per_seg));
        q->tile_segs = std::max<uint32_t>(32, q->tile_segs & ~31u);
        tp.S = q->tile_segs;
        for (uint32_t k = 0; k < p.n_cols; k++) {
            if ((rc = q->bufs.get(&tp.vals[k], (size_t)q->tile_segs * tp.R))) return rc;
            if ((rc = q->bufs.get(&tp.okb[k], (size_t)q->tile_segs * tp.R))) return rc;
        }
        if ((rc = q->bufs.get(&tp.times, (size_t)q->tile_segs * tp.R))) return rc;
        if ((rc = q->bufs.get(&tp.keep, (size_t)q->tile_segs * tp.R))) return rc;
    }
    q->planned = true;
    return OG_OK;
}
}
extern "C" {

OG_API int og_query_run(og_query *q) {
    if (!q) return OG_E_INVAL;
    og_shard *s = q->sh;
    CU(cudaSetDevice(s->device));
    const QueryP &p = q->qp;
    cudaStream_t st = q->stream;
    int rc;
    q->host_ready = false; q->next_group = 0; q->next_row = 0;
    if (!q->planned) {
        if (q->plan) { set_error("query plan failed earlier"); return OG_E_STATE; }
        if ((rc = build_plan(q))) return rc;
    }
    Plan *pl = (Plan *)q->plan;
    ChunkP ch = pl->ch; TileP tp = pl->tp; const GroupP &gp = pl->gp;
    size_t cells_dense = (size_t)q->n_groups * p.n_buckets;
    DirP dir = make_dir(s);
    uint32_t launches = 0, n_chunks = (s->n_series + q->chunk_series - 1) / q->chunk_series;
    while (q->main_ev.size() < 2 * (size_t)n_chunks) { cudaEvent_t e; CU(cudaEventCreate(&e)); q->main_ev.push_back(e); }
    CU(cudaMemsetAsync(q->d_err, 0, 64, st));
    CU(cudaEventRecord(q->ev0, st));
    const bool per_series = q->desc.group_mode == OG_GROUP_PER_SERIES;
    if (!per_series) { k_init_dense<<<(unsigned)((cells_dense + 255) / 256), 256, 0, st>>>(p, gp); launches++; }
    const bool clear_cells = !pl->fold || q->cells_dirty || n_chunks > 1;
    uint64_t segs_scanned = 0; uint32_t ci = 0, chunks_run = 0;
    for (uint32_t a = 0; a < s->n_series; a += q->chunk_series, ci++) {
        if (q->aborted) { cudaStreamSynchronize(st); set_error("query aborted"); return OG_E_ABORTED; }
        uint32_t b = std::min(s->n_series, a + q->chunk_series);
        ch.series_begin = a; ch.series_end = b;
        ch.seg_begin = s->h_series_seg_begin[a]; ch.seg_end = s->h_series_seg_begin[b];
        uint32_t nseg = ch.seg_end - ch.seg_begin;
        const size_t chunk_cells = (size_t)(b - a) * p.n_buckets;
        if (nseg == 0) {
            if (per_series) {
                for (uint32_t c = 0; c < p.n_calls; c++) CU(cudaMemsetAsync(ch.cells[c].ok, 0, chunk_cells, st));
                k_merge_per_series<<<dim3((unsigned)((chunk_cells + 255) / 256), p.n_calls), 256, 0, st>>>(p, ch, gp);
                launches++;
            }
            continue;
        }
        segs_scanned += nseg;
        if (clear_cells) for (uint32_t c = 0; c < p.n_calls; c++) CU(cudaMemsetAsync(ch.cells[c].ok, 0, chunk_cells, st));
        if (pl->fold || pl->blockmerge) for (uint32_t c = 0; c < p.n_calls; c++) CU(cudaMemsetAsync(ch.gcells[c].ok, 0, (size_t)p.n_buckets * ch.gc_cols, st));
        if (pl->fold && ci > 0) CU(cudaMemsetAsync(ch.flags + 1, 0, sizeof(int), st));
        CU(cudaEventRecord(q->main_ev[2 * chunks_run], st));
        if (pl->fused) {
            const uint32_t *gl = nullptr; uint32_t gn = nseg;
            if (pl->fast) {
                const og_shard::IlCol &ic = *pl->ic;
                uint32_t g0 = 0, g1 = ic.n_groups;
                if (ic.J) { g0 = ic.super_grp_first[a / OG_IL_SUPER]; g1 = ic.super_grp_first[std::min<uint32_t>(ic.n_super, (b + OG_IL_SUPER - 1) / OG_IL_SUPER)]; }
                launch_fast(pl->fm, pl->times, pl->fold, pl->il, g0, g1, p, ch, st); launches++;
                auto lo = std::lower_bound(ic.gen_host.begin(), ic.gen_host.end(), ch.seg_begin);
                auto hi = std::lower_bound(ic.gen_host.begin(), ic.gen_host.end(), ch.seg_end);
                gl = ic.gen_list + (lo - ic.gen_host.begin()); gn = (uint32_t)(hi - lo);
            }
            if (gn) {
                switch (p.n_calls) {
                case 1: launch_fused<1>(dir, p, ch, gl, gn, st); break;
                case 2: launch_fused<2>(dir, p, ch, gl, gn, st); break;
                case 3: launch_fused<3>(dir, p, ch, gl, gn, st); break;
                case 4: launch_fused<4>(dir, p, ch, gl, gn, st); break;
                case 5: launch_fused<5>(dir, p, ch, gl, gn, st); break;
                case 6: launch_fused<6>(dir, p, ch, gl, gn, st); break;
                case 7: launch_fused<7>(dir, p, ch, gl, gn, st); break;
                default: launch_fused<8>(dir, p, ch, gl, gn, st); break;
                }
                launches++;
            }
        } else if (pl->cols) {
            launch_cols(p, dir, ch, nseg, st);
        } else if (pl->multi) {
            launch_multi(p, dir, ch, nseg, st);
            launches++;
        } else {
            for (uint32_t t0 = ch.seg_begin; t0 < ch.seg_end; t0 += q->tile_segs) {
                tp.tile_begin = t0; tp.tile_end = std::min(ch.seg_end, t0 + q->tile_segs);
                uint32_t n = tp.tile_end - tp.tile_begin;
                dim3 g((n + 127) / 128, p.n_cols + 1);
                k_decode_tile<<<g, 128, 0, st>>>(dir, p, tp, q->d_err);
                size_t rows_total = (size_t)tp.S * tp.R;
                k_filter_tile<<<(unsigned)((rows_total + 255) / 256), 256, 0, st>>>(dir, p, tp);
                k_window_reduce<<<(n + 127) / 128, 128, 0, st>>>(dir, p, tp, ch);
                launches += 3;
            }
        }
        CU(cudaEventRecord(q->main_ev[2 * chunks_run + 1], st));
        chunks_run++;
        if (pl->fold) k_fix_edges_fold<<<(unsigned)(((size_t)((b - a + 31) / 32) * ch.J * 32 + 127) / 128), 128, 0, st>>>(dir, p, ch);
        else k_fix_edges<<<(nseg + 127) / 128, 128, 0, st>>>(dir, p, ch);
        if (per_series) k_merge_per_series<<<dim3((unsigned)((chunk_cells + 255) / 256), p.n_calls), 256, 0, st>>>(p, ch, gp);
        else if (pl->blockmerge) k_merge_all_blocks<<<dim3((p.n_buckets + 127) / 128, (b - a + OG_MERGE_SB - 1) / OG_MERGE_SB, p.n_calls), 128, 0, st>>>(p, ch, gp);
        else k_merge_groups<<<dim3((unsigned)((cells_dense + 127) / 128), p.n_calls), 128, 0, st>>>(p, ch, gp);
        launches += 2;
        if (pl->fold || pl->blockmerge) { k_merge_folded<<<dim3((unsigned)(((size_t)p.n_buckets * 32 + 127) / 128), p.n_calls), 128, 0, st>>>(p, ch, gp); launches++; }
    }
    CU(cudaEventRecord(q->ev1, st));
    CU(cudaGetLastError());
    CU(cudaStreamSynchronize(st));
    int err[16];
    CU(cudaMemcpy(err, q->d_err, 64, cudaMemcpyDeviceToHost));
    if (getenv("OGPU_IL_STATS")) {
        unsigned long long wait, life, pro, epi;
        memcpy(&wait, err + 8, 8); memcpy(&life, err + 10, 8); memcpy(&pro, err + 12, 8); memcpy(&epi, err + 14, 8);
        const double pc = life ? 100.0 / (double)life : 0.0;
        fprintf(stderr, "[ogpu] fused rounds: common %d rare %d (lanes not resident in %d, sit-outs %d); warp cycles: %llu waiting for batches of %llu (%.1f %%), "
                "prologue %llu (%.1f %%), epilogue %llu (%.1f %%)\n",
                err[4], err[5], err[6], err[7], wait, life, pc * (double)wait, pro, pc * (double)pro, epi, pc * (double)epi);
    }
    q->cells_dirty = err[2] != 0;
    if (err[0]) { set_error("segment %d failed to decode (device code %d)", err[1], err[0]); return map_dev_err(err[0]); }
    float ms = 0; cudaEventElapsedTime(&ms, q->ev0, q->ev1);
    double main_ms = 0;
    for (uint32_t i = 0; i < chunks_run; i++) { float m = 0; cudaEventElapsedTime(&m, q->main_ev[2 * i], q->main_ev[2 * i + 1]); main_ms += m; }
    og_stats &stt = q->stats;
    uint64_t keep_pb = stt.page_bytes, keep_rows = stt.rows_decoded, keep_segs = stt.segments_scanned;
    memset(&stt, 0, sizeof stt);
    stt.kernel_ms = ms; stt.main_kernel_ms = main_ms; stt.kernel_launches = launches; stt.path = q->path_used;
    stt.page_bytes = keep_pb; stt.rows_decoded = keep_pb ? keep_rows : s->n_rows; stt.segments_scanned = keep_pb ? keep_segs : segs_scanned;
    stt.dir_bytes = (uint64_t)segs_scanned * 32;
    stt.out_bytes = 0;
    for (uint32_t c = 0; c < p.n_calls; c++) stt.out_bytes += cells_dense * (9 + (q->dense[c].tim ? 8 : 0));
    if (p.n_cols == 1 && p.col_type[0] == OG_TYPE_FLOAT && p.col_index[0] < (int)s->il.size()) {
        const og_shard::IlCol &ic = s->il[p.col_index[0]];
        stt.il_state = ic.state; stt.il_build_ms = ic.build_ms; stt.il_bytes = ic.n_words * 4; stt.il_packed_segments = ic.state == 1 ? ic.n_packed : 0;
        stt.general_segments = ic.state == 1 ? (uint64_t)ic.gen_host.size() : s->n_segments;
    }
    stt.per_series_cells_used = err[2] != 0;
    q->ran = true;
    return OG_OK;
}

OG_API int og_query_dense(og_query *q, og_dense_view *out) {
    if (!q || !out) return OG_E_INVAL;
    if (!q->ran) { set_error("og_query_dense before og_query_run"); return OG_E_STATE; }
    const QueryP &p = q->qp;
    out->n_groups = q->n_groups; out->n_buckets = p.n_buckets; out->start = q->desc.interval ? p.start : 0; out->interval = q->desc.interval ? p.interval : 0;
    out->n_cols = p.n_calls;
    for (uint32_t c = 0; c < p.n_calls; c++) {
        q->dense_cols[c].values = q->dense[c].val; q->dense_cols[c].valid = q->dense[c].ok; q->dense_cols[c].times = q->dense[c].tim;
        q->dense_cols[c].type = p.calls[c].out_type; q->dense_cols[c].func = p.calls[c].func;
    }
    out->cols = q->dense_cols; out->stream = q->stream;
    return OG_OK;
}

}
namespace {
__global__ void k_sum_page_bytes(DirP d, QueryP q, int64_t tmin, int64_t tmax, unsigned long long *out ) {
    uint32_t seg = blockIdx.x * blockDim.x + threadIdx.x;
    if (seg >= d.n_segments) return;
    if (d.seg_tmax[seg] < tmin || d.seg_tmin[seg] > tmax) return;
    unsigned long long b = d.page_len[(size_t)d.n_columns * d.n_segments + seg];
    for (uint32_t k = 0; k < q.n_cols; k++) b += d.page_len[(size_t)q.col_index[k] * d.n_segments + seg];
    atomicAdd(&out[0], b); atomicAdd(&out[1], (unsigned long long)d.seg_rows[seg]); atomicAdd(&out[2], 1ull);
}
}
extern "C" {

OG_API int og_query_stats(const og_query *q, og_stats *out) {
    if (!q || !out) return OG_E_INVAL;
    og_query *mq = const_cast<og_query *>(q);
    if (q->ran && q->stats.page_bytes == 0) {
        CU(cudaSetDevice(q->sh->device));
        Scratch tmp;
        unsigned long long *d_o; int rc = tmp.get(&d_o, 3); if (rc) return rc;
        cudaMemset(d_o, 0, 24);
        if (q->sh->n_segments) k_sum_page_bytes<<<(q->sh->n_segments + 255) / 256, 256>>>(make_dir(q->sh), q->qp, q->qp.tmin, q->qp.tmax, d_o);
        unsigned long long h[3]; CU(cudaMemcpy(h, d_o, 24, cudaMemcpyDeviceToHost));
        mq->stats.page_bytes = h[0]; mq->stats.rows_decoded = h[1]; mq->stats.segments_scanned = h[2];
    }
    *out = q->stats;
    return OG_OK;
}

OG_API int og_query_merge_dense(og_query *q, const og_dense_view *other) {
    if (!q || !other) return OG_E_INVAL;
    if (!q->ran) return OG_E_STATE;
    const QueryP &p = q->qp;
    if (other->n_groups != q->n_groups || other->n_buckets != p.n_buckets || other->n_cols != p.n_calls) { set_error("dense shapes differ"); return OG_E_INVAL; }
    if (other->start != (q->desc.interval ? p.start : 0) || other->interval != (q->desc.interval ? p.interval : 0)) {
        set_error("dense grids differ (start %lld vs %lld, interval %lld vs %lld): create the queries with OG_Q_QUERY_GRID", (long long)other->start,
                  (long long)(q->desc.interval ? p.start : 0), (long long)other->interval, (long long)(q->desc.interval ? p.interval : 0));
        return OG_E_INVAL;
    }
    CU(cudaSetDevice(q->sh->device));
    GroupP mine, oth; memset(&mine, 0, sizeof mine); memset(&oth, 0, sizeof oth);
    mine.n_groups = oth.n_groups = q->n_groups;
    for (uint32_t c = 0; c < p.n_calls; c++) {
        mine.dense[c] = q->dense[c];
        oth.dense[c].val = (uint64_t *)other->cols[c].values; oth.dense[c].ok = other->cols[c].valid; oth.dense[c].tim = other->cols[c].times;
        if ((q->dense[c].tim != nullptr) != (oth.dense[c].tim != nullptr)) { set_error("dense column %u: times presence differs", c); return OG_E_INVAL; }
    }
    size_t total = (size_t)q->n_groups * p.n_buckets;
    k_merge_dense<<<(unsigned)((total + 255) / 256), 256, 0, q->stream>>>(p, mine, oth);
    CU(cudaGetLastError());
    CU(cudaStreamSynchronize(q->stream));
    q->host_ready = false;
    return OG_OK;
}

OG_API int og_query_next(og_query *q, og_record_view *out) {
    if (!q || !out) return OG_E_INVAL;
    if (!q->ran) { set_error("og_query_next before og_query_run"); return OG_E_STATE; }
    if (q->aborted) return OG_E_ABORTED;
    const QueryP &p = q->qp;
    size_t total = (size_t)q->n_groups * p.n_buckets;
    if (!q->host_ready) {
        CU(cudaSetDevice(q->sh->device));
        for (uint32_t c = 0; c < p.n_calls; c++) {
            q->h_val[c].resize(total); q->h_ok[c].resize(total);
            CU(cudaMemcpy(q->h_val[c].data(), q->dense[c].val, total * 8, cudaMemcpyDeviceToHost));
            CU(cudaMemcpy(q->h_ok[c].data(), q->dense[c].ok, total, cudaMemcpyDeviceToHost));
            if (q->dense[c].tim) { q->h_tim[c].resize(total); CU(cudaMemcpy(q->h_tim[c].data(), q->dense[c].tim, total * 8, cudaMemcpyDeviceToHost)); }
        }
        q->host_ready = true; q->next_group = 0; q->next_row = 0;
    }
    int chunk = q->desc.chunk_size > 0 ? q->desc.chunk_size : 1024;
    uint32_t nc = p.n_calls;
    q->rv_val.assign(nc, {}); q->rv_bitmap.assign(nc, {}); q->rv_coltimes.assign(nc, {}); q->rv_times.clear(); q->rv_cols.assign(nc, og_colval_view{});
    while (q->next_group < q->n_groups) {
        uint32_t g = q->next_group;
        std::vector<int32_t> nil(nc, 0);
        int rows = 0;
        uint32_t b = q->next_row;
        uint32_t b_end = (uint32_t)std::min<uint64_t>(p.n_buckets, (uint64_t)b + (uint64_t)chunk);
        for (; b < b_end; b++) {
            const uint32_t bb = q->desc.ascending ? b : p.n_buckets - 1 - b;
            size_t i = (size_t)g * p.n_buckets + bb;
            bool any = false;
            for (uint32_t c = 0; c < nc; c++) any |= q->h_ok[c][i] != 0;
            if (!any) continue;
            int64_t row_time = p.start + (int64_t)bb * p.interval;
            if (q->desc.interval == 0) row_time = 0;
            for (uint32_t c = 0; c < nc; c++) {
                bool ok = q->h_ok[c][i] != 0;
                if ((size_t)(rows >> 3) >= q->rv_bitmap[c].size()) q->rv_bitmap[c].push_back(0);
                if (ok) {
                    q->rv_bitmap[c][rows >> 3] |= (uint8_t)(1 << (rows & 7));
                    if (p.calls[c].out_type == OG_TYPE_BOOL) q->rv_val[c].push_back((uint8_t)(q->h_val[c][i] != 0));
                    else { const uint8_t *pv = (const uint8_t *)&q->h_val[c][i]; q->rv_val[c].insert(q->rv_val[c].end(), pv, pv + 8); }
                } else nil[c]++;
                if (q->dense[c].tim) {
                    if (p.multi) q->rv_coltimes[c].push_back(ok ? q->h_tim[c][i] : 0);
                    else if (ok) row_time = q->h_tim[c][i];
                }
            }
            q->rv_times.push_back(row_time);
            rows++;
        }
        q->next_row = b_end;
        if (q->next_row >= p.n_buckets) { q->next_group++; q->next_row = 0; }
        if (rows == 0) continue;
        for (uint32_t c = 0; c < nc; c++) {
            og_colval_view &v = q->rv_cols[c];
            v.val = q->rv_val[c].data(); v.val_bytes = q->rv_val[c].size(); v.bitmap = q->rv_bitmap[c].data();
            v.times = (p.multi && q->dense[c].tim) ? q->rv_coltimes[c].data() : nullptr;
            v.type = p.calls[c].out_type; v.len = rows; v.nil_count = nil[c]; v.bitmap_offset = 0;
        }
        out->n_cols = nc; out->cols = q->rv_cols.data(); out->times = q->rv_times.data(); out->rows = rows; out->group = g;
        out->sid = q->desc.group_mode == OG_GROUP_PER_SERIES ? q->sh->sids[g] : 0;
        return OG_OK;
    }
    return OG_EOF;
}

}
namespace {
__global__ void k_decode_column(DirP d, uint32_t column, int type, uint32_t seg_begin, uint32_t seg_end, uint8_t *out, uint64_t stride,
                                uint32_t *rows_out, uint8_t *bitmap_out, uint32_t bitmap_stride, int *err) {
    uint32_t seg = seg_begin + blockIdx.x * blockDim.x + threadIdx.x;
    if (seg >= seg_end) return;
    uint8_t *o = out + (size_t)(seg - seg_begin) * stride;
    uint32_t rows = d.seg_rows[seg];
    size_t pi = (size_t)column * d.n_segments + seg;
    if (column == d.n_columns) {
        TimeDesc t;
        int rc = parse_time_page(d.data + d.page_off[pi], d.page_len[pi], t);
        if (rc == D_OK) {
            TimeIter it; it.init(t);
            for (uint32_t i = 0; i < t.rows; i++) ((int64_t *)o)[i] = it.next();
            it.finish(); rc = it.err;
        }
        if (rc != D_OK) report_err(err, rc, seg);
        if (rows_out) rows_out[seg - seg_begin] = rows;
        return;
    }
    uint32_t len = d.page_len[pi];
    uint8_t *bm = bitmap_out ? bitmap_out + (size_t)(seg - seg_begin) * bitmap_stride : nullptr;
    if (len == 0) {
        if (rows_out) rows_out[seg - seg_begin] = 0;
        if (bm) for (uint32_t i = 0; i < (rows + 7) / 8; i++) bm[i] = 0;
        return;
    }
    ColIter it;
    it.init(d.data + d.page_off[pi], len, type, rows);
    int rc = it.err;
    if (rc == D_OK && type == OG_TYPE_STRING) rc = D_UNSUPPORTED;
    if (rc == D_OK) {
        const PageHdr &h = it.h;
        for (uint32_t r = 0, j = 0; r < rows; r++) {
            uint64_t v;
            if (!it.next(v)) continue;
            if (type == OG_TYPE_BOOL) o[j++] = (uint8_t)v; else ((uint64_t *)o)[j++] = v;
        }
        it.finish(); rc = it.err;
        if (rows_out) rows_out[seg - seg_begin] = h.rows - h.nil_count;
        if (bm) {
            for (uint32_t i = 0; i < (rows + 7) / 8; i++) {
                uint8_t v = 0;
                for (uint32_t k = 0; k < 8 && i * 8 + k < rows; k++) v |= (uint8_t)(hdr_row_valid(h, i * 8 + k) ? 1 : 0) << k;
                bm[i] = v;
            }
        }
    }
    if (rc != D_OK) report_err(err, rc, seg);
}
}
extern "C" {

OG_API int og_decode_column_device(og_shard *s, uint32_t column, uint32_t seg_begin, uint32_t seg_end, void *d_values,
                                   uint64_t value_stride_bytes, uint32_t *d_rows_out) {
    if (!s || !d_values || column > s->n_columns || seg_begin > seg_end || seg_end > s->n_segments) { set_error("bad argument"); return OG_E_INVAL; }
    CU(cudaSetDevice(s->device));
    if (seg_begin == seg_end) return OG_OK;
    int *d_err; int rc = dalloc(&d_err, 2); if (rc) return rc;
    cudaMemset(d_err, 0, 8);
    int type = column == s->n_columns ? OG_TYPE_INT : s->col_types[column];
    uint32_t n = seg_end - seg_begin;
    k_decode_column<<<(n + 127) / 128, 128>>>(make_dir(s), column, type, seg_begin, seg_end, (uint8_t *)d_values, value_stride_bytes, d_rows_out, nullptr, 0, d_err);
    int err[2]; cudaError_t e = cudaMemcpy(err, d_err, 8, cudaMemcpyDeviceToHost); dev_free(d_err);
    if (e != cudaSuccess) return cuda_fail(e, "k_decode_column", __FILE__, __LINE__);
    if (err[0]) { set_error("segment %d failed to decode (device code %d)", err[1], err[0]); return map_dev_err(err[0]); }
    return OG_OK;
}

__global__ void k_reverse_segment(uint8_t *vals, uint32_t elem_bytes, uint32_t n_vals, uint8_t *bitmap, uint32_t rows) {
    for (uint32_t i = threadIdx.x; i < n_vals / 2; i += blockDim.x) {
        const uint32_t j = n_vals - 1 - i;
        if (elem_bytes == 8) { uint64_t *v = (uint64_t *)vals; const uint64_t a = v[i]; v[i] = v[j]; v[j] = a; }
        else { const uint8_t a = vals[i]; vals[i] = vals[j]; vals[j] = a; }
    }
    if (!bitmap) return;
    __syncthreads();
    __shared__ uint8_t sbm[8192];
    const uint32_t nb = (rows + 7) / 8;
    for (uint32_t i = threadIdx.x; i < nb; i += blockDim.x) sbm[i] = bitmap[i];
    __syncthreads();
    for (uint32_t i = threadIdx.x; i < nb; i += blockDim.x) {
        uint8_t o = 0;
        for (uint32_t k = 0; k < 8 && i * 8 + k < rows; k++) { const uint32_t src = rows - 1 - (i * 8 + k); o |= (uint8_t)((sbm[src >> 3] >> (src & 7)) & 1) << k; }
        bitmap[i] = o;
    }
}
}
static int decode_segment_impl(og_shard *s, uint32_t segment, uint32_t flags, og_record_view *out);
extern "C" {
OG_API int og_decode_segment(og_shard *s, uint32_t segment, og_record_view *out) { return decode_segment_impl(s, segment, 0, out); }
OG_API int og_decode_segment_ex(og_shard *s, uint32_t segment, uint32_t flags, og_record_view *out) { return decode_segment_impl(s, segment, flags, out); }
}
static int decode_segment_impl(og_shard *s, uint32_t segment, uint32_t flags, og_record_view *out) {
    if (!s || !out || segment >= s->n_segments) { set_error("bad argument"); return OG_E_INVAL; }
    CU(cudaSetDevice(s->device));
    uint32_t R = std::max<uint32_t>(1, s->max_seg_rows);
    size_t ncol1 = (size_t)s->n_columns + 1;
    size_t val_stride = (size_t)R * 8, bm_stride = (((size_t)R + 7) / 8 + 7) & ~(size_t)7;
    size_t need = ncol1 * (val_stride + bm_stride + 16);
    if (s->d_seg_buf_bytes < need || s->h_seg_buf_bytes < need) {
        dev_free(s->d_seg_buf); s->d_seg_buf = nullptr; s->d_seg_buf_bytes = 0;
        if (s->h_seg_buf) cudaFreeHost(s->h_seg_buf);
        s->h_seg_buf = nullptr; s->h_seg_buf_bytes = 0;
        CU(dev_malloc(&s->d_seg_buf, need)); s->d_seg_buf_bytes = need;
        CU(cudaMallocHost(&s->h_seg_buf, need)); s->h_seg_buf_bytes = need;
    }
    uint8_t *dv = (uint8_t *)s->d_seg_buf, *dbm = dv + ncol1 * val_stride;
    uint32_t *drows = (uint32_t *)(dbm + ncol1 * bm_stride);
    int *d_err; int rc = dalloc(&d_err, 2); if (rc) return rc;
    cudaMemset(d_err, 0, 8);
    DirP dir = make_dir(s);
    for (uint32_t c = 0; c <= s->n_columns; c++) {
        int type = c == s->n_columns ? OG_TYPE_INT : s->col_types[c];
        k_decode_column<<<1, 32>>>(dir, c, type, segment, segment + 1, dv + c * val_stride, val_stride, drows + c, dbm + c * bm_stride, (uint32_t)bm_stride, d_err);
    }
    int err[2]; cudaError_t e = cudaMemcpy(err, d_err, 8, cudaMemcpyDeviceToHost); dev_free(d_err);
    if (e != cudaSuccess) return cuda_fail(e, "k_decode_column", __FILE__, __LINE__);
    if (err[0]) { set_error("segment %d failed to decode (device code %d)", err[1], err[0]); return map_dev_err(err[0]); }
    if (flags & OG_DECODE_DESCENDING) {
        if (R > 65536) { set_error("descending materialisation supports segments of up to 65536 rows"); return OG_E_UNSUPPORTED; }
        uint32_t hr[65];
        CU(cudaMemcpy(hr, drows, (ncol1) * 4, cudaMemcpyDeviceToHost));
        const uint32_t rows_seg = hr[s->n_columns];
        for (uint32_t c = 0; c <= s->n_columns; c++) {
            const bool is_time = c == s->n_columns;
            const uint32_t eb = (!is_time && s->col_types[c] == OG_TYPE_BOOL) ? 1 : 8;
            k_reverse_segment<<<1, 256>>>(dv + c * val_stride, eb, is_time ? rows_seg : hr[c], is_time ? nullptr : dbm + c * bm_stride, rows_seg);
        }
        CU(cudaGetLastError());
    }
    CU(cudaMemcpy(s->h_seg_buf, s->d_seg_buf, need, cudaMemcpyDeviceToHost));
    uint8_t *hv = (uint8_t *)s->h_seg_buf, *hbm = hv + ncol1 * val_stride;
    uint32_t *hrows = (uint32_t *)(hbm + ncol1 * bm_stride);
    uint32_t rows = hrows[s->n_columns];
    s->seg_views.assign(s->n_columns, og_colval_view{});
    for (uint32_t c = 0; c < s->n_columns; c++) {
        og_colval_view &v = s->seg_views[c];
        uint32_t nv = hrows[c];
        v.val = hv + c * val_stride; v.val_bytes = (uint64_t)nv * (s->col_types[c] == OG_TYPE_BOOL ? 1 : 8);
        v.bitmap = hbm + c * bm_stride; v.times = nullptr; v.type = s->col_types[c]; v.len = (int32_t)rows; v.nil_count = (int32_t)(rows - nv); v.bitmap_offset = 0;
    }
    out->n_cols = s->n_columns; out->cols = s->seg_views.data(); out->times = (const int64_t *)(hv + s->n_columns * val_stride); out->rows = (int32_t)rows; out->group = 0;
    uint32_t sr = (uint32_t)(std::upper_bound(s->h_series_seg_begin.begin(), s->h_series_seg_begin.end(), segment) - s->h_series_seg_begin.begin()) - 1;
    out->sid = s->sids[sr];
    return OG_OK;
}
```

opengemini_b200/csrc/fused_il.cuh:

```cuda
#pragma once
#include "agg_kernels.cuh"

namespace ogpu {

__device__ __forceinline__ uint32_t smem_u32(const void *p) { return (uint32_t)__cvta_generic_to_shared(p); }
__device__ __forceinline__ uint32_t opaque(uint32_t x) { asm volatile("mov.u32 %0, %0;" : "+r"(x)); return x; }
template <int OFF> __device__ __forceinline__ uint32_t lds32o(uint32_t a) { uint32_t v; asm volatile("ld.shared.u32 %0, [%1+%2];" : "=r"(v) : "r"(a), "n"(OFF)); return v; }
__device__ __forceinline__ void mbar_init(uint32_t bar, uint32_t count) { asm volatile("mbarrier.init.shared::cta.b64 [%0], %1;" ::"r"(bar), "r"(count) : "memory"); }
__device__ __forceinline__ void mbar_init_fence() { asm volatile("fence.mbarrier_init.release.cluster;\nfence.proxy.async.shared::cta;" ::: "memory"); }
__device__ __forceinline__ void mbar_expect_tx(uint32_t bar, uint32_t bytes) { asm volatile("mbarrier.arrive.expect_tx.shared::cta.b64 _, [%0], %1;" ::"r"(bar), "r"(bytes) : "memory"); }
__device__ __forceinline__ void bulk_g2s(uint32_t dst, const void *src, uint32_t bytes, uint32_t bar) {
    asm volatile("cp.async.bulk.shared::cluster.global.mbarrier::complete_tx::bytes [%0], [%1], %2, [%3];" ::"r"(dst), "l"(src), "r"(bytes), "r"(bar) : "memory");
}
__device__ __forceinline__ bool mbar_wait(uint32_t bar, uint32_t parity) {
#pragma unroll 1
    for (uint32_t i = 0; i < (1u << 16); i++) {
        uint32_t ok;
        asm volatile("{\n.reg .pred p;\nmbarrier.try_wait.parity.shared::cta.b64 p, [%1], %2;\nselp.u32 %0, 1, 0, p;\n}" : "=r"(ok) : "r"(bar), "r"(parity) : "memory");
        if (ok) return true;
    }
    return false;
}

enum { FM_COUNT = 1, FM_SUM = 2, FM_MIN = 4, FM_MAX = 8, FM_FIRST = 16, FM_LAST = 32 };
enum { SEG_GENERAL = 0, SEG_FAST = 1, SEG_PACKED = 2 };

#ifndef OG_FAST_THREADS
#define OG_FAST_THREADS 128
#endif
#ifndef OG_FAST_MAXREG
#define OG_FAST_MAXREG 80
#endif
#ifndef OG_IL_NW
#define OG_IL_NW 64u
#endif
#ifndef OG_IL_B
#define OG_IL_B 16u
#endif
#ifndef OG_IL_K
#define OG_IL_K 10u
#endif
#ifndef OG_IL_UNROLL
#define OG_IL_UNROLL 2
#endif
#define OG_IL_NB (OG_IL_NW / OG_IL_B)
#define OG_IL_ROWS (OG_IL_NW + 2u)
#define OG_IL_PAD_WORDS 6u
#define OG_IL_HDR 7u
#define OG_IL_RAW_HDR 6u
#define OG_IL_NONE 0xffffffffu
#define OG_IL_PACKED 0x8000u
#define OG_IL_LOOKBITS (77u * OG_IL_K + 29u + 13u + 64u + 64u)
static_assert(OG_IL_K >= 2, "packed lanes: K*64 + 63 + 128 <= OG_IL_LOOKBITS needs K >= 2");
static_assert(OG_IL_NW % OG_IL_B == 0 && (OG_IL_NW & (OG_IL_NW - 1)) == 0, "ring geometry");
static_assert(OG_IL_NW - OG_IL_B > (OG_IL_LOOKBITS + 31u) / 32u + 2u, "ring too small for the round length: the slowest lane could not proceed");

struct IlP {
    const uint32_t *words;
    const uint64_t *grp_off;
    const uint32_t *grp_rows;
    const uint32_t *grp_col;
    const uint32_t *lane_seg;
    const uint32_t *lane_rows;
    const uint16_t *lane_win;
    const uint32_t *lane_series;
    const int64_t *lane_t0;
    const uint64_t *lane_dt;
};

__device__ __forceinline__ uint64_t udiv_est(uint64_t a, uint64_t b, double inv_b) {
    const double qd = __ull2double_rn(a) * inv_b;
    if ((a >> 63) || !(qd < 1125899906842624.0)) return a / b;
    uint64_t q = (uint64_t)qd;
    uint64_t r = a - q * b;
    if ((int64_t)r < 0) { do { q--; r += b; } while ((int64_t)r < 0); }
    else while (r >= b) { q++; r -= b; }
    return q;
}

__device__ __forceinline__ uint64_t fetch64(uint32_t col, uint32_t p) {
    uint32_t a = col + ((p << 2) & ((OG_IL_NW - 1) << 7));
    uint32_t a0 = lds32o<0>(a), a1 = lds32o<128>(a), a2 = lds32o<256>(a);
    uint32_t hi = __funnelshift_l(a1, a0, p), lo = __funnelshift_l(a2, a1, p);
    return ((uint64_t)hi << 32) | lo;
}

__device__ __forceinline__ Part fold32(int func, int type, bool multi, Part p, bool with_time) {
    constexpr uint32_t FULL = 0xffffffffu;
    if (func == OG_AGG_COUNT) { p.v = __reduce_add_sync(FULL, p.ok ? (uint32_t)p.v : 0u); p.ok = p.v != 0; return p; }
    if (type == OG_TYPE_FLOAT && func == OG_AGG_SUM) {
        double s = p.ok ? u2d(p.v) : 0.0;
#pragma unroll
        for (int o = 16; o; o >>= 1) s += __shfl_xor_sync(FULL, s, o);
        p.ok = __any_sync(FULL, p.ok != 0); p.v = d2u(s); return p;
    }
    if (type == OG_TYPE_FLOAT && !with_time && (func == OG_AGG_MIN || func == OG_AGG_MAX)) {
        double v = u2d(p.v); uint32_t ok = p.ok;
#pragma unroll
        for (int o = 16; o; o >>= 1) {
            const double ov = __shfl_xor_sync(FULL, v, o); const uint32_t ook = __shfl_xor_sync(FULL, ok, o);
            const bool keep = ok && (func == OG_AGG_MIN ? v <= ov : v >= ov);
            if (ook && !keep) v = ov;
            ok |= ook;
        }
        p.v = d2u(v); p.ok = ok; return p;
    }
    return warp_fold(func, type, multi, p, with_time);
}

#define OG_IL_WCAP 24u
__host__ __device__ inline uint32_t il_acc_bytes(uint32_t n_calls, bool times) { return OG_IL_WCAP * n_calls * (times ? 17u : 9u) + 8u & ~7u; }

template <int FM, bool TIMES, bool FOLD>
__global__ void __maxnreg__(OG_FAST_MAXREG) k_fused_il(QueryP q, ChunkP ch, IlP il, uint32_t grp_begin, uint32_t grp_end) {
    constexpr uint32_t NW = OG_IL_NW, B = OG_IL_B, NB = OG_IL_NB, K = OG_IL_K;
    constexpr uint32_t FULL = 0xffffffffu;
    constexpr uint32_t WPB = OG_FAST_THREADS / 32;
    constexpr int UNR = OG_IL_UNROLL;
    __shared__ __align__(128) uint32_t s_win[WPB * OG_IL_ROWS * 32];
    __shared__ __align__(8) uint64_t s_bar[WPB * NB];
    extern __shared__ __align__(8) uint8_t s_acc[];

#ifdef OG_IL_STATS
    const long long st_clk0 = clock64();
    long long st_wait = 0;
#endif
    const uint32_t lane = threadIdx.x & 31;
    const uint32_t wid = __reduce_max_sync(FULL, threadIdx.x >> 5);
    const uint32_t grp = grp_begin + blockIdx.x * WPB + wid;
    if (grp >= grp_end) return;
    const uint32_t rows_w = __reduce_max_sync(FULL, il.grp_rows[grp]);
    if (rows_w == 0) return;
    const size_t slot = (size_t)grp * 32 + lane;
    const uint32_t seg = il.lane_seg[slot];
    bool active = seg != OG_IL_NONE && seg >= ch.seg_begin && seg < ch.seg_end;
    if (!__any_sync(FULL, active)) return;
    const size_t e = 2 * (size_t)(seg - ch.seg_begin);

    uint32_t rows = 0, series = 0, r_lo = 0, r_hi = 0, lwin = 0;
    int64_t t0 = 0, dt = 1; uint64_t dtu = 1; double inv_dt = 1.0;
    const double inv_iv = 1.0 / __ull2double_rn((uint64_t)q.interval);
    if (active) {
        rows = il.lane_rows[slot]; lwin = il.lane_win[slot]; series = il.lane_series[slot];
        t0 = il.lane_t0[slot]; dtu = il.lane_dt[slot]; dt = (int64_t)dtu;
        inv_dt = 1.0 / __ull2double_rn(dtu);
        r_lo = 0; r_hi = rows - 1;
        if (t0 < q.tmin) { uint64_t k = udiv_est((uint64_t)(q.tmin - t0) + dtu - 1, dtu, inv_dt); r_lo = k > rows ? rows : (uint32_t)k; }
        { int64_t t_last = t0 + (int64_t)(rows - 1) * dt; if (t_last > q.tmax) { if (q.tmax < t0) r_lo = rows; else r_hi = (uint32_t)udiv_est((uint64_t)(q.tmax - t0), dtu, inv_dt); } }
        const uint64_t span = (uint64_t)q.n_buckets * (uint64_t)q.interval;
        const bool outside = r_lo <= r_hi && r_lo < rows &&
                             ((uint64_t)(t0 + (int64_t)r_lo * dt - q.start) >= span || (uint64_t)(t0 + (int64_t)r_hi * dt - q.start) >= span);
        if (outside) report_err(ch.err, D_CORRUPT, seg);
        if (r_lo > r_hi || r_lo >= rows || outside) { *(uint2 *)(ch.edge_bucket + e) = make_uint2(OG_NO_BUCKET, OG_NO_BUCKET); active = false; }
    }
    if (!__any_sync(FULL, active)) return;

    const uint32_t win = smem_u32(s_win) + wid * (OG_IL_ROWS * 128);
    const uint32_t col = opaque(win + lane * 4);
    const uint32_t bar0 = smem_u32(s_bar) + wid * (NB * 8);
    if (lane == 0) {
#pragma unroll
        for (uint32_t i = 0; i < NB; i++) mbar_init(bar0 + i * 8, 1);
        mbar_init_fence();
    }
    __syncwarp();
    const uint32_t total_b = rows_w / B;
    uint64_t goff = il.grp_off[grp];
    goff = ((uint64_t)__reduce_max_sync(FULL, (uint32_t)(goff >> 32)) << 32) | __reduce_max_sync(FULL, (uint32_t)goff);
    const uint32_t *gsrc = il.words + goff;
    uint32_t issued_b = 0, ready_b = 0;
    uint32_t hung = 0;
    uint64_t pol;
    asm("createpolicy.fractional.L2::evict_first.b64 %0, 1.0;" : "=l"(pol));
    auto issue = [&](uint32_t k_any) {
        const uint32_t k = __reduce_max_sync(FULL, k_any);
        const uint32_t s = k % NB, dst = win + s * (B * 128), bar = bar0 + s * 8;
        const uint32_t *src = gsrc + (size_t)k * (B * 32);
        if (s == 0)
            asm volatile("{\n.reg .pred p;\nelect.sync _|p, 0xffffffff;\n@p mbarrier.arrive.expect_tx.shared::cta.b64 _, [%0], %1;\n"
                         "@p cp.async.bulk.shared::cluster.global.mbarrier::complete_tx::bytes.L2::cache_hint [%2], [%3], %4, [%0], %6;\n"
                         "@p cp.async.bulk.shared::cluster.global.mbarrier::complete_tx::bytes.L2::cache_hint [%5], [%3], 256, [%0], %6;\n}"
                         ::"r"(bar), "r"(B * 128 + 256u), "r"(dst), "l"(src), "r"(B * 128), "r"(win + NW * 128), "l"(pol) : "memory");
        else
            asm volatile("{\n.reg .pred p;\nelect.sync _|p, 0xffffffff;\n@p mbarrier.arrive.expect_tx.shared::cta.b64 _, [%0], %1;\n"
                         "@p cp.async.bulk.shared::cluster.global.mbarrier::complete_tx::bytes.L2::cache_hint [%2], [%3], %1, [%0], %4;\n}"
                         ::"r"(bar), "r"(B * 128), "r"(dst), "l"(src), "l"(pol) : "memory");
    };
    {
        const uint32_t first = total_b < NB ? total_b : NB;
        for (uint32_t k = 0; k < first; k++) issue(k);
        issued_b = first;
    }

    uint32_t cur_b = 0, rb = 0xffffffffu, step_q = 0; uint64_t rem = 0, step_r = 0;
    if (active) {
        const int64_t t_lo = t0 + (int64_t)r_lo * dt;
        cur_b = (uint32_t)udiv_est((uint64_t)(t_lo - q.start), (uint64_t)q.interval, inv_iv);
        const uint64_t ivl = (uint64_t)q.interval;
        const uint64_t sq64 = udiv_est(ivl, dtu, inv_dt);
        step_q = sq64 > 0xffffffffull ? 0xffffffffu : (uint32_t)sq64;
        step_r = ivl - sq64 * dtu;
        uint64_t D = (uint64_t)(q.start + (int64_t)(cur_b + 1) * q.interval - t0) + dtu - 1;
        uint64_t qq = udiv_est(D, dtu, inv_dt); rem = D - qq * dtu; rb = qq > 0xffffffffull ? 0xffffffffu : (uint32_t)qq;
    }

    bool uni = false; uint32_t b0 = 0, b_end = 0;
    uint64_t *acc_v = nullptr; int64_t *acc_t = nullptr; uint8_t *acc_k = nullptr;
    if (FOLD) {
        const int leader = __ffs(__ballot_sync(FULL, active)) - 1;
        const int64_t t0L = __shfl_sync(FULL, t0, leader); const uint64_t dtL = __shfl_sync(FULL, dtu, leader);
        const uint32_t loL = __shfl_sync(FULL, r_lo, leader), hiL = __shfl_sync(FULL, r_hi, leader);
        b0 = __shfl_sync(FULL, cur_b, leader);
        const bool same = t0 == t0L && dtu == dtL && r_lo == loL && r_hi == hiL;
        const uint32_t b_last = active ? (uint32_t)udiv_est((uint64_t)(t0 + (int64_t)r_hi * dt - q.start), (uint64_t)q.interval, inv_iv) : b0;
        uni = __all_sync(FULL, !active || (same && b_last - b0 < OG_IL_WCAP));
        if (uni) {
            b_end = __reduce_max_sync(FULL, active ? b_last : 0u);
            const uint32_t nacc = OG_IL_WCAP * q.n_calls;
            uint8_t *base = s_acc + (size_t)wid * il_acc_bytes(q.n_calls, TIMES);
            acc_v = (uint64_t *)base; acc_t = (int64_t *)(base + (size_t)nacc * 8); acc_k = base + (size_t)nacc * (TIMES ? 16 : 8);
            for (uint32_t i = lane; i < nacc; i += 32) acc_k[i] = 0;
            __syncwarp();
        }
    }
    const uint32_t gcol = FOLD ? il.grp_col[grp] - ch.gc_col0 : 0;
    const bool fold_edges = FOLD && uni && b_end > b0;

    double sum = 0.0, mn = 0.0, mx = 0.0; uint64_t fi = 0, lastv = 0;
    uint32_t n_mn = 0, n_mx = 0;
    uint32_t w_row0 = r_lo;
    bool head_done = false; uint32_t head_b = OG_NO_BUCKET;
    uint32_t stop = 0, n_ev = 0;
    auto part_of = [&](int func, uint32_t cnt) -> Part {
        Part pp; pp.ok = cnt != 0; pp.v = 0; pp.t = 0;
        switch (func) {
        case OG_AGG_COUNT: pp.v = cnt; break;
        case OG_AGG_SUM: if (FM & FM_SUM) pp.v = d2u(sum); break;
        case OG_AGG_MIN: if (FM & FM_MIN) { pp.v = d2u(mn); if (TIMES) pp.t = t0 + (int64_t)(stop - n_mn) * dt; } break;
        case OG_AGG_MAX: if (FM & FM_MAX) { pp.v = d2u(mx); if (TIMES) pp.t = t0 + (int64_t)(stop - n_mx) * dt; } break;
        case OG_AGG_FIRST: if (FM & FM_FIRST) { pp.v = fi; pp.t = t0 + (int64_t)w_row0 * dt; } break;
        default: if (FM & FM_LAST) { pp.v = lastv; pp.t = t0 + (int64_t)(stop - 1) * dt; } break;
        }
        return pp;
    };
    auto kind_of = [&]() -> int { return !head_done ? 0 : stop > r_hi ? 1 : 2; };
    auto flush_lane = [&](int kind) {
        const uint32_t cnt = stop - w_row0;
#pragma unroll 1
        for (uint32_t c = 0; c < q.n_calls; c++) {
            const Part pp = part_of(q.calls[c].func, cnt);
            if (kind == 2) { if (pp.ok) store_cell(ch, (int)c, series, cur_b, pp); }
            else store_part(ch.edges[c], e + kind, pp);
        }
        if (kind == 0) { head_done = true; head_b = cur_b; }
    };
    auto flush_fold = [&](bool ev) {
        uint32_t pend = __ballot_sync(FULL, ev);
#pragma unroll 1
        while (pend) {
            const int leader = __ffs(pend) - 1;
            const uint32_t bL = __shfl_sync(FULL, cur_b, leader);
            const bool mine = ev && cur_b == bL;
            const uint32_t cnt = mine ? stop - w_row0 : 0;
            const uint32_t w = bL - b0;
#pragma unroll 1
            for (uint32_t c = 0; c < q.n_calls; c++) {
                const int func = q.calls[c].func, ftype = func == OG_AGG_COUNT ? OG_TYPE_INT : q.calls[c].type;
                const bool wt = func >= OG_AGG_MIN && !(q.multi && func <= OG_AGG_MAX);
                Part pp = fold32(func, ftype, q.multi != 0, part_of(func, cnt), wt);
                if ((int)lane == leader && pp.ok) {
                    const uint32_t i = c * OG_IL_WCAP + w;
                    Part a; a.ok = acc_k[i]; a.v = a.ok ? acc_v[i] : 0; a.t = (TIMES && a.ok) ? acc_t[i] : 0;
                    group_update(func, ftype, q.multi != 0, a, pp);
                    acc_v[i] = a.v; acc_k[i] = 1; if (TIMES) acc_t[i] = a.t;
                }
            }
            pend &= ~__ballot_sync(FULL, mine);
        }
        __syncwarp();
    };

    uint32_t qp = 0, sr = 0, kfast = 0, CM = 0, CE = 0, m = 64, tr = 0, bad = 0; uint64_t MASK = 0;
    bool done = !active;
    uint64_t val = 0;

#ifdef OG_IL_STATS
    long long st_w0 = clock64();
#endif
    if (issued_b && !mbar_wait(bar0, 0)) hung = 1; else ready_b = issued_b ? 1 : 0;
#ifdef OG_IL_STATS
    st_wait += clock64() - st_w0;
#endif
    if (active && !hung) {
        val = fetch64(col, 0); qp = 64;
        if (lwin & OG_IL_PACKED) {
            const uint32_t lead = (lwin >> 8) & 63u, mw = lwin & 127u;
            qp = 64 - lead; kfast = mw;
            MASK = mw ? (~0ull >> (64 - mw)) << (64 - lead - mw) : 0ull;
        } else { CM = 0; CE = 1; }
    }

    bool skipping = r_lo > 0;
    stop = skipping ? r_lo : (rb < r_hi + 1 ? rb : r_hi + 1);
    n_ev = stop;
    if (!skipping) { fi = val; mn = mx = u2d(val); n_mn = n_mx = n_ev; }
    if (done) n_ev = 0xffffffffu;

    auto retire = [&]() { done = true; n_ev = 0xffffffffu; CM = 0; CE = 0; MASK = 0; kfast = 0; };
    auto advance = [&]() {
        bool fin = false;
        if (skipping) { skipping = false; sum = 0.0; }
        else {
            fin = stop > r_hi;
            sum = 0.0;
            if (!fin) while (stop >= rb) {
                cur_b++;
                rem += step_r; uint32_t adv = step_q;
                if (rem >= dtu) { rem -= dtu; adv++; }
                rb = (rb > 0xffffffffu - adv) ? 0xffffffffu : rb + adv;
            }
        }
        if (fin) retire();
        else {
            w_row0 = stop;
            uint32_t nstop = rb < r_hi + 1 ? rb : r_hi + 1;
            n_ev = nstop - stop; stop = nstop;
            fi = val; mn = mx = u2d(val); n_mn = n_mx = n_ev;
        }
    };
    auto slow_record = [&]() {
        uint32_t p = qp + sr;
        const uint64_t x = fetch64(col, p);
        const uint32_t ctrl = (uint32_t)(x >> 62);
        if (ctrl < 2) { qp += 1; return; }
        if (ctrl == 3) {
            const uint32_t lm = (uint32_t)(x >> 51) & 0x7ff;
            uint32_t lead = lm >> 6; m = lm & 0x3f;
            if (m == 0) { m = 64; tr = 0; lead = 0; }
            else { if (lead + m > 64) { if (!done) bad = 1; lead = 0; m = 64; } tr = 64 - lead - m; }
            p += 13;
            const bool slowwin = lead < 2;
            sr = slowwin ? 0 : lead - 2;
            CM = slowwin ? 0u : 3u << (30 - sr); CE = slowwin ? 1u : 2u << (30 - sr);
            kfast = 2 + m;
            MASK = (m == 64 ? ~0ull : ((1ull << m) - 1)) << tr;
        } else p += 2;
        const uint64_t y = fetch64(col, p);
        const uint64_t sig = m == 64 ? y : (y >> (64 - m));
        p += m;
        val ^= sig << tr;
        qp = p - sr;
    };
    auto accumulate = [&](uint32_t k_in_run) {
        if (FM & FM_SUM) sum = sum + u2d(val);
        if (FM & FM_MIN) { if (mn > u2d(val)) { mn = u2d(val); if (TIMES) n_mn = n_ev - k_in_run; } }
        if (FM & FM_MAX) { if (mx < u2d(val)) { mx = u2d(val); if (TIMES) n_mx = n_ev - k_in_run; } }
        if (FM & FM_LAST) lastv = val;
    };
    auto record = [&](uint32_t k_in_run) {
        accumulate(k_in_run);
        const uint64_t x = fetch64(col, qp);
        const bool slow = (((uint32_t)(x >> 32) & CM) ^ CE) != 0;
        if (slow) slow_record();
        else { val ^= x & MASK; qp += kfast; }
    };
    auto record2 = [&](uint32_t k_in_run) {
        const uint64_t x0 = fetch64(col, qp), x1 = fetch64(col, qp + kfast);
        accumulate(k_in_run);
#ifdef OG_IL_REC2B
        uint64_t x1b = x1;
        if ((((uint32_t)(x0 >> 32) & CM) ^ CE) != 0) { slow_record(); x1b = fetch64(col, qp); }
        else { val ^= x0 & MASK; qp += kfast; }
        accumulate(k_in_run + 1);
        if ((((uint32_t)(x1b >> 32) & CM) ^ CE) != 0) slow_record();
        else { val ^= x1b & MASK; qp += kfast; }
#else
        if ((((uint32_t)(x0 >> 32) & CM) ^ CE) != 0) { slow_record(); record(k_in_run + 1); return; }
        val ^= x0 & MASK; qp += kfast;
        accumulate(k_in_run + 1);
        if ((((uint32_t)(x1 >> 32) & CM) ^ CE) != 0) slow_record();
        else { val ^= x1 & MASK; qp += kfast; }
#endif
    };

    uint32_t rounds_left = hung ? 0u : 40u * (__reduce_max_sync(FULL, rows) / K + 8u);
#ifdef OG_IL_STATS
    uint32_t st_common = 0, st_rare = 0, st_sit = 0, st_notgo = 0;
    const long long st_pro = clock64() - st_clk0;
#endif
    for (;;) {
        const uint32_t qmin = __reduce_min_sync(FULL, done ? 0xffffffffu : qp);
        if (qmin == 0xffffffffu) break;
        const uint32_t f = qmin < 32 ? 0u : (qmin - 32) >> 5;
#pragma unroll 1
        while (issued_b < total_b && (issued_b + 1) * B <= f + NW) { issue(issued_b); issued_b++; }
        const uint32_t qmax = __reduce_max_sync(FULL, done ? 0u : qp);
        uint32_t need_max = ((qmax + OG_IL_LOOKBITS) >> 5) + 1; if (need_max > rows_w) need_max = rows_w;
        uint32_t want_b = (need_max + B - 1) / B; if (want_b > issued_b) want_b = issued_b;
#ifdef OG_IL_STATS
        st_w0 = clock64();
#endif
#pragma unroll 1
        while (ready_b < want_b) { if (!mbar_wait(bar0 + (ready_b % NB) * 8, (ready_b / NB) & 1)) { hung = 1; break; } ready_b++; }
#ifdef OG_IL_STATS
        st_wait += clock64() - st_w0;
#endif
        if (hung) break;
        uint32_t need = ((qp + OG_IL_LOOKBITS) >> 5) + 1; if (need > rows_w) need = rows_w;
        bool go = done || need <= ready_b * B;
        uint32_t run = __reduce_min_sync(FULL, go ? n_ev : 0u);
        if (run >= K) {
            static_assert(K % 2 == 0, "records are decoded in pairs");
#pragma unroll UNR
            for (uint32_t k = 0; k < K; k += 2) record2(k);
            n_ev -= K;
#ifdef OG_IL_STATS
            st_common++;
#endif
            continue;
        }
#ifdef OG_IL_STATS
        st_rare++;
#endif
        if (rounds_left-- == 0) { hung = 2; break; }
        const bool all_go = __all_sync(FULL, go);
#ifdef OG_IL_STATS
        if (!all_go) { st_notgo++; st_sit += __popc(__ballot_sync(FULL, !go)); }
#endif
        uint32_t left = K;
        for (;;) {
            run = __reduce_min_sync(FULL, go ? n_ev : 0xffffffffu);
            if (run > left) run = left;
            if (all_go) {
#pragma unroll 1
                for (uint32_t k = 0; k < run; k++) record(k);
            } else {
#pragma unroll 1
                for (uint32_t k = 0; k < run; k++) if (go) record(k);
            }
            if (go) n_ev -= run;
            left -= run;
            if (left == 0) break;
            const bool ev = go && !done && n_ev == 0;
            if (FOLD && uni) {
                const bool fl = ev && !skipping;
                const int kind = kind_of();
                const bool to_acc = fl && (kind == 2 || fold_edges);
                if (fl && !to_acc) flush_lane(kind);
                if (__any_sync(FULL, to_acc)) flush_fold(to_acc);
                if (to_acc && kind == 0) head_done = true;
            } else if (ev && !skipping) flush_lane(kind_of());
            if (ev) advance();
            if (__all_sync(FULL, ev || done)) break;
        }
    }
    if (active && (qp >> 5) >= rows_w) bad = 1;
#ifdef OG_IL_STATS
    const long long st_e0 = clock64();
    if (lane == 0) { atomicAdd((unsigned *)&ch.err[4], st_common); atomicAdd((unsigned *)&ch.err[5], st_rare); atomicAdd((unsigned *)&ch.err[6], st_notgo); atomicAdd((unsigned *)&ch.err[7], st_sit); }
#endif
    while (ready_b < issued_b && hung != 1) { if (!mbar_wait(bar0 + (ready_b % NB) * 8, (ready_b / NB) & 1)) hung = 1; ready_b++; }
    if (hung && lane == 0) report_err(ch.err, D_WATCHDOG, (grp << 2) | hung);
    if (FOLD && uni) {
        __syncwarp();
        const uint32_t w_tail = fold_edges ? b_end - b0 : OG_IL_WCAP;
        for (uint32_t i = lane; i < OG_IL_WCAP * q.n_calls; i += 32) {
            if (!acc_k[i]) continue;
            const uint32_t c = i / OG_IL_WCAP, w = i % OG_IL_WCAP;
            Part a; a.ok = 1; a.v = acc_v[i]; a.t = TIMES ? acc_t[i] : 0;
            store_part(ch.gcells[c], (size_t)(b0 + w) * ch.gc_cols + (w == w_tail ? ch.gc_tail0 + gcol : gcol), a);
        }
    }
    if (FOLD && __any_sync(FULL, active && head_b != OG_NO_BUCKET) && lane == 0) ch.flags[1] = 1;
    if (active) {
        if (bad) report_err(ch.err, D_CORRUPT, seg);
        *(uint2 *)(ch.edge_bucket + e) = make_uint2(head_b, (head_b == OG_NO_BUCKET || cur_b == head_b) ? OG_NO_BUCKET : cur_b);
    }
#ifdef OG_IL_STATS
    if (lane == 0) {
        atomicAdd((unsigned long long *)(ch.err + 8), (unsigned long long)st_wait);
        const long long st_end = clock64();
        atomicAdd((unsigned long long *)(ch.err + 10), (unsigned long long)(st_end - st_clk0));
        atomicAdd((unsigned long long *)(ch.err + 12), (unsigned long long)st_pro);
        atomicAdd((unsigned long long *)(ch.err + 14), (unsigned long long)(st_end - st_e0));
    }
#endif
}

}
```

opengemini_b200/csrc/il_build.cuh:

```cuda
#pragma once
#include "fused_il.cuh"

namespace ogpu {

#define OG_IL_SUPER 4096u
#define OG_IL_WORD_BITS 24u

struct IlScanOut {
    uint32_t *seg_words;
    uint16_t *seg_win;
    unsigned long long *n_packed;
    int64_t *seg_t0;
    uint64_t *seg_dt;
    uint64_t *keys;
    uint32_t *vals;
    uint32_t *dom_cnt;
    uint32_t *misaligned;
};

__device__ inline bool il_delta_window(const uint8_t *page, uint32_t len, uint32_t rows, uint32_t m_stop, uint32_t &lead, uint32_t &m) {
    ColIter it;
    it.init(page, len, OG_TYPE_FLOAT, rows);
    uint64_t prev = 0, acc = 0;
    if (it.err != D_OK || !it.next(prev)) return false;
    for (uint32_t r = 1; r < rows && it.err == D_OK; r++) {
        uint64_t v = 0;
        if (!it.next(v)) return false;
        acc |= v ^ prev; prev = v;
        if ((r & 31) == 0 && m_stop < 64 && acc && 64 - __clzll((long long)acc) - (__ffsll((long long)acc) - 1) >= (int)m_stop) return false;
    }
    if (it.err != D_OK) return false;
    lead = acc ? (uint32_t)__clzll((long long)acc) : 0u;
    m = acc ? 64u - lead - (uint32_t)(__ffsll((long long)acc) - 1) : 0u;
    return true;
}

__global__ void k_il_scan(DirP d, int col, int col_type, uint32_t J, IlScanOut o) {
    uint32_t seg = blockIdx.x * blockDim.x + threadIdx.x;
    if (seg >= d.n_segments) return;
    uint8_t c = SEG_GENERAL; uint32_t nw = 0; int64_t t0 = 0; uint64_t dt = 0; uint16_t win = 0;
    const uint32_t rows = d.seg_rows[seg];
    if (rows >= 2 && rows < (1u << 22) && col_type == OG_TYPE_FLOAT) {
        size_t pi = (size_t)col * d.n_segments + seg, ti = (size_t)d.n_columns * d.n_segments + seg;
        const uint8_t *p = d.data + d.page_off[pi], *t = d.data + d.page_off[ti];
        uint32_t len = d.page_len[pi], tlen = d.page_len[ti];
        TimeDesc td;
        if (len >= 16 && tlen >= 16 && __ldg(p) == 31 && __ldg(t) == 32 && (__ldg(t + 5) >> 4) == 1 && ld_be32(p + 1) == rows &&
            parse_time_page(t, tlen, td) == D_OK && td.kind == 0 && td.delta > 0 && td.delta < (1ull << 40)) {
            const int tag = __ldg(p + 5) >> 4;
            if (tag == 3 && __ldg(p + 6) == 0x10) {
                c = SEG_FAST; nw = (len - OG_IL_HDR + 3) / 4 + OG_IL_PAD_WORDS;
            } else if (tag == 0 && len == OG_IL_RAW_HDR + 8 * (size_t)rows) {
                c = SEG_PACKED; nw = 2 * rows + OG_IL_PAD_WORDS; win = OG_IL_PACKED | 64u;
            }
            uint32_t m_stop = 64, lead, m;
            if (c == SEG_FAST) {
                const uint32_t T = nw > 2 + OG_IL_PAD_WORDS ? nw - 2 - OG_IL_PAD_WORDS : 0;
                const uint64_t ms = T ? (32ull * (T - 1)) / (rows - 1) + 1 : 0;
                m_stop = ms < 64 ? (uint32_t)ms : 64u;
            }
            if (c != SEG_GENERAL && il_delta_window(p, len, rows, m_stop, lead, m)) {
                const uint32_t pw = 2u + (uint32_t)(((uint64_t)(rows - 1) * m + 31) / 32) + OG_IL_PAD_WORDS;
                if (c == SEG_PACKED || pw < nw) { c = SEG_PACKED; nw = pw; win = (uint16_t)(OG_IL_PACKED | lead << 8 | m); }
            }
            if (nw >= (1u << OG_IL_WORD_BITS)) { c = SEG_GENERAL; nw = 0; win = 0; }
            t0 = td.t0; dt = td.delta;
        }
    }
    o.seg_words[seg] = nw; o.seg_win[seg] = win; o.seg_t0[seg] = t0; o.seg_dt[seg] = dt; o.vals[seg] = seg;
    {
        const unsigned am = __activemask(), pm = __ballot_sync(am, c == SEG_PACKED);
        if (pm && (threadIdx.x & 31) == (unsigned)(__ffs(am) - 1)) atomicAdd(o.n_packed, (unsigned long long)__popc(pm));
    }
    const uint32_t series = d.seg_series[seg];
    if (J) {
        const uint32_t ref = d.series_seg_begin[series / OG_IL_SUPER * OG_IL_SUPER] + (seg - d.series_seg_begin[series]);
        if (d.seg_tmin[seg] != d.seg_tmin[ref] || d.seg_tmax[seg] != d.seg_tmax[ref]) *o.misaligned = 1;
    }
    if (c == SEG_GENERAL) { o.keys[seg] = ~0ull; return; }
    const uint32_t dom = J ? (series / OG_IL_SUPER) * J + (seg - d.series_seg_begin[series]) : 0u;
    o.keys[seg] = ((uint64_t)dom << OG_IL_WORD_BITS) | nw;
    atomicAdd(&o.dom_cnt[dom], 1u);
}

struct IlAssign {
    const uint64_t *keys; const uint32_t *segs;
    const uint32_t *elem_first, *grp_first;
    const uint32_t *seg_words; const int64_t *seg_t0; const uint64_t *seg_dt; const uint16_t *seg_win;
    uint32_t *lane_seg, *lane_rows, *lane_series, *grp_col; uint16_t *lane_win; int64_t *lane_t0; uint64_t *lane_dt;
    uint32_t n_elig, J, cols_per_super;
};
__global__ void k_il_assign(DirP d, IlAssign a) {
    uint32_t i = blockIdx.x * blockDim.x + threadIdx.x;
    if (i >= a.n_elig) return;
    const uint32_t seg = a.segs[i], dom = (uint32_t)(a.keys[i] >> OG_IL_WORD_BITS);
    const uint32_t rank = i - a.elem_first[dom], g = a.grp_first[dom] + rank / 32;
    const size_t slot = (size_t)g * 32 + (rank & 31);
    a.lane_seg[slot] = seg;
    a.lane_rows[slot] = d.seg_rows[seg];
    a.lane_win[slot] = a.seg_win[seg];
    a.lane_series[slot] = d.seg_series[seg];
    a.lane_t0[slot] = a.seg_t0[seg]; a.lane_dt[slot] = a.seg_dt[seg];
    if ((rank & 31) == 0) a.grp_col[g] = (a.J ? dom / a.J : 0u) * a.cols_per_super + rank / 32;
}

__global__ void k_il_group_rows(uint32_t n_groups, const uint32_t *lane_seg, const uint32_t *seg_words, uint32_t *grp_rows) {
    uint32_t g = (blockIdx.x * blockDim.x + threadIdx.x) >> 5, lane = threadIdx.x & 31;
    if (g >= n_groups) return;
    uint32_t seg = lane_seg[(size_t)g * 32 + lane];
    uint32_t w = seg != OG_IL_NONE ? seg_words[seg] : 0;
#pragma unroll
    for (int o = 16; o; o >>= 1) w = max(w, __shfl_xor_sync(0xffffffffu, w, o));
    if (lane == 0) grp_rows[g] = (w + OG_IL_B - 1) / OG_IL_B * OG_IL_B;
}

__global__ void k_il_repack(DirP d, int col, const uint32_t *lane_seg, const uint16_t *lane_win, const uint64_t *grp_off, const uint32_t *grp_rows,
                            uint32_t n_groups, uint32_t *il) {
    uint32_t g = (blockIdx.x * blockDim.x + threadIdx.x) >> 5, lane = threadIdx.x & 31;
    if (g >= n_groups) return;
    const uint32_t nw = grp_rows[g];
    if (nw == 0) return;
    const size_t slot = (size_t)g * 32 + lane;
    const uint32_t seg = lane_seg[slot];
    const bool live = seg != OG_IL_NONE;
    const uint32_t win = live ? lane_win[slot] : 0u;
    const bool packed = (win & OG_IL_PACKED) != 0;
    const uint32_t *base = nullptr; uint32_t sh = 0, own_words = 0, a = 0, sel = 0;
    ColIter it;
    uint64_t prev = 0, pend = 0, acc = 0; uint32_t pbits = 0, nb = 0, left = 0, mw = 0, tr = 0;
    if (live) {
        const size_t pi = (size_t)col * d.n_segments + seg;
        const uint8_t *page = d.data + d.page_off[pi];
        if (packed) {
            it.init(page, d.page_len[pi], OG_TYPE_FLOAT, d.seg_rows[seg]);
            it.next(prev);
            pend = prev; pbits = 64;
            mw = win & 127u;
            tr = mw ? 64u - ((win >> 8) & 63u) - mw : 0u;
            left = mw ? d.seg_rows[seg] - 1 : 0u;
        } else {
            const uint8_t *s = page + OG_IL_HDR;
            base = (const uint32_t *)((uintptr_t)s & ~(uintptr_t)3);
            sh = (uint32_t)((uintptr_t)s & 3);
            own_words = (d.page_len[pi] - OG_IL_HDR + 3) / 4 + OG_IL_PAD_WORDS;
            a = __ldg(base);
            sel = sh == 0 ? 0x0123u : sh == 1 ? 0x1234u : sh == 2 ? 0x2345u : 0x3456u;
        }
    }
    uint32_t *out = il + grp_off[g] + lane;
    for (uint32_t w = 0; w < nw; w++) {
        uint32_t v = 0;
        if (packed) {
            while (nb < 32) {
                if (pbits == 0) {
                    if (left == 0) break;
                    uint64_t x = 0;
                    it.next(x);
                    pend = (x ^ prev) >> tr; prev = x; pbits = mw; left--;
                }
                const uint32_t k = pbits < 32 ? pbits : 32;
                acc |= ((pend >> (pbits - k)) & (~0ull >> (64 - k))) << (64 - nb - k);
                nb += k; pbits -= k;
            }
            v = (uint32_t)(acc >> 32);
            acc <<= 32; nb = nb > 32 ? nb - 32 : 0;
        } else if (w < own_words) {
            const uint32_t b = __ldg(base + w + 1);
            v = __byte_perm(a, b, sel);
            a = b;
        }
        out[(size_t)w * 32] = v;
    }
}

}
```

opengemini_b200/csrc/internal.h:

```cpp
#pragma once
#include <cuda_runtime.h>

#include <cstdint>
#include <memory>
#include <string>
#include <mutex>
#include <vector>

#include "../../include/ogpu.h"

#define OG_MAX_CALLS 8
#define OG_MAX_FILTER 16
#define OG_MAX_COLS 8

namespace ogpu {

void set_error(const char *fmt, ...);
int cuda_fail(cudaError_t e, const char *what, const char *file, int line);
int ensure_device();

inline cudaError_t dev_malloc(void **p, size_t bytes) { return cudaMallocAsync(p, bytes ? bytes : 1, (cudaStream_t)0); }
inline void dev_free(void *p) { if (p) cudaFreeAsync(p, (cudaStream_t)0); }
template <class... T> void dev_free_all(T *...p) { (dev_free((void *)p), ...); }
cudaError_t dev_mem_info(size_t *free_b, size_t *total_b);
#define CU(call) do { cudaError_t e__ = (call); if (e__ != cudaSuccess) return ::ogpu::cuda_fail(e__, #call, __FILE__, __LINE__); } while (0)

template <class T> int dalloc(T **p, size_t n) {
    *p = nullptr;
    if (n == 0) n = 1;
    cudaError_t e = dev_malloc((void **)p, n * sizeof(T));
    if (e != cudaSuccess) { set_error("cudaMalloc(%zu bytes) failed: %s", n * sizeof(T), cudaGetErrorString(e)); return e == cudaErrorMemoryAllocation ? OG_E_NOMEM : OG_E_CUDA; }
    return OG_OK;
}

struct Scratch {
    cudaStream_t stream = nullptr;
    std::vector<void *> bufs;
    Scratch() = default;
    explicit Scratch(cudaStream_t st) : stream(st) {}
    Scratch(const Scratch &) = delete;
    Scratch &operator=(const Scratch &) = delete;
    ~Scratch() {
        if (stream && !bufs.empty()) cudaStreamSynchronize(stream);
        for (void *p : bufs) dev_free(p);
    }
    template <class T> int get(T **p, size_t n) { int rc = dalloc(p, n); if (rc == OG_OK) bufs.push_back(*p); return rc; }
};

struct LiveQueries { std::mutex mu; uint32_t n = 0; };

struct ShardState {
    int device = 0;
    uint8_t *d_data = nullptr; uint64_t data_len = 0; bool owns_data = true;
    uint32_t n_series = 0, n_segments = 0, n_columns = 0;
    uint32_t max_seg_rows = 0;
    uint64_t irregular_time_pages = 0;
    uint64_t n_rows = 0, page_bytes = 0;
    uint64_t snappy_pages = 0, snappy_bytes_in = 0, snappy_bytes_out = 0;
    og_merge_info merge{1, 0, 0, 0, 0, 0, 0, 0, 0, 0};
    bool rows_merged = false;
    int64_t tmin = 0, tmax = 0;
    std::vector<uint64_t> sids;
    std::vector<int32_t> col_types;
    std::vector<std::string> col_names;
    std::vector<uint32_t> h_series_seg_begin;
    uint32_t *d_series_seg_begin = nullptr;
    uint32_t *d_seg_series = nullptr;
    uint32_t *d_seg_rows = nullptr;
    int64_t *d_tmin = nullptr, *d_tmax = nullptr;
    uint64_t *d_page_off = nullptr;
    uint32_t *d_page_len = nullptr;
    uint64_t *d_sids = nullptr;
};

}

struct og_shard : ogpu::ShardState {
    void *h_seg_buf = nullptr; size_t h_seg_buf_bytes = 0;
    void *d_seg_buf = nullptr; size_t d_seg_buf_bytes = 0;
    std::vector<og_colval_view> seg_views;
    struct IlCol { int state = 0;
                   uint32_t *words = nullptr; uint64_t *grp_off = nullptr; uint32_t *grp_rows = nullptr, *grp_col = nullptr;
                   uint32_t *lane_seg = nullptr, *lane_rows = nullptr, *lane_series = nullptr; uint16_t *lane_win = nullptr; int64_t *lane_t0 = nullptr; uint64_t *lane_dt = nullptr;
                   uint32_t *gen_list = nullptr; std::vector<uint32_t> gen_host;
                   uint32_t n_groups = 0, J = 0;
                   bool aligned = false;
                   uint32_t n_super = 1, cols_per_super = 0; std::vector<uint32_t> super_grp_first;
                   uint64_t n_words = 0, n_packed = 0;  double build_ms = 0; };
    std::vector<IlCol> il;
    std::mutex il_mu;
    std::shared_ptr<ogpu::LiveQueries> live = std::make_shared<ogpu::LiveQueries>();
    ~og_shard() {
        using ogpu::dev_free_all;
        if (owns_data) dev_free_all(d_data);
        dev_free_all(d_series_seg_begin, d_seg_series, d_seg_rows, d_tmin, d_tmax, d_page_off, d_page_len, d_sids, d_seg_buf);
        if (h_seg_buf) cudaFreeHost(h_seg_buf);
        for (IlCol &c : il)
            dev_free_all(c.words, c.grp_off, c.grp_rows, c.grp_col, c.lane_seg, c.lane_rows, c.lane_series, c.lane_win, c.lane_t0, c.lane_dt, c.gen_list);
    }
};

namespace ogpu {

struct CallP { int32_t func, col_slot, type, out_type; };
struct FilterP { int32_t kind, col_slot, op, type, const_is_float; double fval; int64_t ival; };

struct Tri { uint64_t *val; int64_t *tim; uint8_t *ok; };

struct QueryP {
    int64_t tmin, tmax, start, interval;
    uint32_t n_buckets, n_calls, n_filter, n_cols;
    int32_t multi;
    CallP calls[OG_MAX_CALLS];
    FilterP filter[OG_MAX_FILTER];
    int32_t col_index[OG_MAX_COLS];
    int32_t col_type[OG_MAX_COLS];
};

}

struct og_query {
    og_shard *sh = nullptr;
    std::shared_ptr<ogpu::LiveQueries> live;
    og_query_desc desc{};
    std::vector<og_call> calls;
    std::vector<og_filter_item> filter;
    std::vector<uint32_t> series_group;
    cudaStream_t stream = nullptr;
    cudaEvent_t ev0 = nullptr, ev1 = nullptr;
    ogpu::QueryP qp{};
    uint32_t n_groups = 0;
    bool ran = false; volatile int aborted = 0;
    ogpu::Tri dense[OG_MAX_CALLS]{};
    og_dense_col dense_cols[OG_MAX_CALLS]{};
    ogpu::Scratch bufs;
    og_stats stats{};
    std::vector<uint64_t> h_val[OG_MAX_CALLS];
    std::vector<uint8_t> h_ok[OG_MAX_CALLS];
    std::vector<int64_t> h_tim[OG_MAX_CALLS];
    bool host_ready = false;
    uint32_t next_group = 0, next_row = 0;
    std::vector<std::vector<uint8_t>> rv_val, rv_bitmap;
    std::vector<std::vector<int64_t>> rv_coltimes;
    std::vector<int64_t> rv_times;
    std::vector<og_colval_view> rv_cols;
    int path_used = 0;
    bool cells_dirty = true;
    bool planned = false;
    uint32_t chunk_series = 0, tile_segs = 0;
    int *d_err = nullptr;
    void *plan = nullptr;
    std::vector<cudaEvent_t> main_ev;
    void *merge_state = nullptr;
    ~og_query();
};
```

opengemini_b200/csrc/merge.cu:

```cuda
#include <algorithm>
#include <cstdio>
#include <cstdlib>
#include <cstring>
#include <map>
#include <string>
#include <vector>

#include <cub/device/device_scan.cuh>
#include <cub/device/device_segmented_sort.cuh>

#include "decode.cuh"
#include "internal.h"

namespace ogpu {

int shard_finalize(og_shard *s, bool scan_snappy);
int check_desc(const og_shard_desc *d);
int upload_dir(og_shard *s, const uint32_t *series_seg_begin, const int64_t *seg_tmin, const int64_t *seg_tmax, const uint64_t *page_off,
               const uint32_t *page_len, const uint64_t *sids);
int encode_pages(int32_t type, int32_t is_time, const void *d_values, const uint8_t *d_valid, const uint32_t *d_rows, uint32_t n_segments,
                 uint32_t rps, uint8_t *d_out, uint64_t out_cap, uint64_t *d_page_off, uint32_t *d_page_len, uint64_t *total_bytes_out,
                 bool nan_raw);

#define MERGE_RPS 1000u
// ... 315 lines not shown
                if (d->columns[c].page_len[g]) { fd.off[(size_t)col_of[c] * NSRC + gs] = fd.base[f] + d->columns[c].page_off[g]; fd.len[(size_t)col_of[c] * NSRC + gs] = d->columns[c].page_len[g]; }
            fd.off[(size_t)nc * NSRC + gs] = fd.base[f] + d->time_page_off[g]; fd.len[(size_t)nc * NSRC + gs] = d->time_page_len[g];
        }
        for (uint32_t s = 0; s < d->n_series; s++) fd.ssb.push_back((uint32_t)(fd.seg0[f] + d->series_seg_begin[s]));
    }
    fd.ssb.push_back(NSRC);
    return OG_OK;
}

static int upload_files(const og_shard_desc *files, uint32_t n_files, const std::vector<std::string> &names, const std::vector<int32_t> &types,
                        int dev, FileDir &fd, std::unique_ptr<og_shard> &out, std::vector<uint32_t> &rows) {
    int rc;
    std::unique_ptr<og_shard> src(new og_shard);
    src->device = dev; src->n_series = (uint32_t)fd.ser0[n_files]; src->n_segments = fd.n; src->n_columns = (uint32_t)names.size();
    src->col_types = types; src->col_names = names; src->data_len = fd.data_len;
    src->h_series_seg_begin = fd.ssb;
    for (uint32_t f = 0; f < n_files; f++) src->sids.insert(src->sids.end(), files[f].sids, files[f].sids + files[f].n_series);
    if ((rc = dalloc(&src->d_data, fd.data_len + 1024))) return rc;
    CU(cudaMemset(src->d_data, 0, fd.data_len + 1024));
    for (uint32_t f = 0; f < n_files; f++)
        if (files[f].data_len) CU(cudaMemcpy(src->d_data + fd.base[f], files[f].data, files[f].data_len, cudaMemcpyHostToDevice));
    if ((rc = upload_dir(src.get(), fd.ssb.data(), fd.tmin.data(), fd.tmax.data(), fd.off.data(), fd.len.data(), src->sids.data()))) return rc;
    if ((rc = shard_finalize(src.get(), true))) return rc;
    CU(cudaMemcpy(fd.off.data(), src->d_page_off, fd.off.size() * 8, cudaMemcpyDeviceToHost));
    CU(cudaMemcpy(fd.len.data(), src->d_page_len, fd.len.size() * 4, cudaMemcpyDeviceToHost));
    rows.resize(fd.n);
    CU(cudaMemcpy(rows.data(), src->d_seg_rows, fd.n * 4ull, cudaMemcpyDeviceToHost));
    out = std::move(src);
    return OG_OK;
}

static bool file_is_ooo(const uint32_t *file_flags, uint32_t f) { return file_flags && (file_flags[f] & OG_FILE_OUT_OF_ORDER); }

static int split_segments(const og_shard_desc *files, uint32_t n_files, const uint32_t *file_flags, const FileDir &fd,
                          std::map<uint64_t, uint32_t> &series_of_sid, const std::vector<uint64_t> &sids,
                          std::vector<std::vector<uint32_t>> &ordered, std::vector<std::vector<uint32_t>> &ooo, og_merge_info &info) {
    for (uint32_t f = 0; f < n_files; f++) {
        const og_shard_desc *d = &files[f];
        const bool late = file_is_ooo(file_flags, f);
        if (late) info.n_out_of_order_files++;
        for (uint32_t s = 0; s < d->n_series; s++) {
            const uint32_t u = series_of_sid[d->sids[s]];
            for (uint32_t g = d->series_seg_begin[s]; g < d->series_seg_begin[s + 1]; g++) {
                const uint32_t gs = (uint32_t)(fd.seg0[f] + g);
                if (late) { ooo[u].push_back(gs); continue; }
                if (!ordered[u].empty() && fd.tmin[gs] <= fd.tmax[ordered[u].back()]) {
                    set_error("series sid %llu: ordered files %u and %u overlap in time (%lld <= %lld); only out-of-order files may overlap",
                              (unsigned long long)sids[u], fd.src_file[ordered[u].back()], f, (long long)fd.tmin[gs], (long long)fd.tmax[ordered[u].back()]);
                    return OG_E_UNSUPPORTED;
                }
                ordered[u].push_back(gs);
            }
        }
    }
    return OG_OK;
}

static void span_hull(const std::vector<uint32_t> &ooo, const FileDir &fd, int64_t *lo, int64_t *hi) {
    *lo = INT64_MAX; *hi = INT64_MIN;
    for (uint32_t g : ooo) { *lo = std::min(*lo, fd.tmin[g]); *hi = std::max(*hi, fd.tmax[g]); }
}

static void span_bounds(const std::vector<uint32_t> &o, const FileDir &fd, int64_t lo, int64_t hi, uint32_t *a, uint32_t *b) {
    uint32_t i = 0;
    while (i < o.size() && fd.tmax[o[i]] < lo) i++;
    *a = i;
    while (i < o.size() && fd.tmin[o[i]] <= hi) i++;
    *b = i;
}

static void sort_oldest_first(std::vector<uint32_t> &segs, const FileDir &fd, const uint32_t *file_flags) {
    auto rank = [&](uint32_t g) { return std::make_pair(file_is_ooo(file_flags, fd.src_file[g]) ? 1 : 0, fd.src_file[g]); };
    std::stable_sort(segs.begin(), segs.end(), [&](uint32_t x, uint32_t y) { return rank(x) < rank(y); });
}


struct SegSrc {
    const uint64_t *off; const uint32_t *len, *rows; const int64_t *tmin, *tmax;
    const uint32_t *seg_region; uint32_t region;
    const int32_t *col; uint32_t n_segments, n_columns;
};
struct SpliceP {
    SegSrc src[3];
    const Run *runs; uint32_t n_runs, n_out, n_columns;
    uint64_t *off; uint32_t *len, *rows, *series, *region; int64_t *tmin, *tmax;
};

__global__ void k_append_splice(SpliceP p) {
    const uint32_t g = blockIdx.x * blockDim.x + threadIdx.x;
    if (g >= p.n_out) return;
    uint32_t lo = 0, hi = p.n_runs;
    while (hi - lo > 1) { const uint32_t m = (lo + hi) / 2; if (p.runs[m].out0 <= g) lo = m; else hi = m; }
    const Run r = p.runs[lo];
    const SegSrc &S = p.src[r.kind];
    const uint32_t i = r.src0 + (g - r.out0);
    p.tmin[g] = S.tmin[i]; p.tmax[g] = S.tmax[i]; p.rows[g] = S.rows[i]; p.series[g] = r.series;
    p.region[g] = S.seg_region ? S.seg_region[i] : S.region;
    for (uint32_t c = 0; c <= p.n_columns; c++) {
        const int sc = c == p.n_columns ? (int)S.n_columns : S.col[c];
        const size_t o = (size_t)c * p.n_out + g;
        if (sc < 0) { p.off[o] = 0; p.len[o] = 0; continue; }
        const size_t pi = (size_t)sc * S.n_segments + i;
        p.off[o] = S.off[pi]; p.len[o] = S.len[pi];
    }
}

__global__ void k_append_sizes(const uint32_t *len, uint64_t n_pages, uint64_t *sizes) {
    const uint64_t i = (uint64_t)blockIdx.x * blockDim.x + threadIdx.x;
    if (i <= n_pages) sizes[i] = i < n_pages ? len[i] : 0;
}

constexpr int APPEND_GATHER_THREADS = 256;
__global__ void __launch_bounds__(APPEND_GATHER_THREADS) k_append_gather(const uint8_t *const *regions, const uint32_t *seg_region, const uint64_t *src_off,
                                                                         const uint32_t *len, uint64_t *dst_off, uint32_t n_segments, uint64_t n_pages, uint8_t *out) {
    const uint64_t page = ((uint64_t)blockIdx.x * APPEND_GATHER_THREADS + threadIdx.x) >> 5;
    const uint32_t lane = threadIdx.x & 31;
    if (page >= n_pages) return;
    const uint32_t l = len[page];
    if (l == 0) { if (lane == 0) dst_off[page] = 0; return; }
    const uint8_t *src = regions[seg_region[page % n_segments]] + src_off[page];
    uint8_t *dst = out + dst_off[page];
    const uint32_t head = min((uint32_t)((16 - ((uintptr_t)dst & 15)) & 15), l);
    const uint32_t n_blocks = (l - head) / 16, tail = head + n_blocks * 16;
    if (lane < head) dst[lane] = __ldg(src + lane);
    for (uint32_t k = lane; k < n_blocks; k += 32) {
        const uintptr_t sa = (uintptr_t)(src + head + 16 * k);
        const uint64_t *q = (const uint64_t *)(sa & ~(uintptr_t)7);
        const unsigned sh = (unsigned)(sa & 7) * 8;
        uint64_t a = __ldg(q), b = __ldg(q + 1);
        if (sh) { const uint64_t c = __ldg(q + 2); a = (a >> sh) | (b << (64 - sh)); b = (b >> sh) | (c << (64 - sh)); }
        *(uint4 *)(dst + head + 16 * k) = make_uint4((uint32_t)a, (uint32_t)(a >> 32), (uint32_t)b, (uint32_t)(b >> 32));
    }
    for (uint32_t i = tail + lane; i < l; i += 32) dst[i] = __ldg(src + i);
}

__global__ void k_append_probe(const uint32_t *series_seg_begin, const int64_t *seg_tmin, const int64_t *seg_tmax, const uint32_t *series,
                               const int64_t *lo, const int64_t *hi, uint32_t n, int64_t *last, uint32_t *a_out, uint32_t *b_out) {
    const uint32_t k = blockIdx.x * blockDim.x + threadIdx.x;
    if (k >= n) return;
    const uint32_t g0 = series_seg_begin[series[k]], g1 = series_seg_begin[series[k] + 1];
    last[k] = g1 > g0 ? seg_tmax[g1 - 1] : INT64_MIN;
    uint32_t a = g0, e = g1;
    while (a < e) { const uint32_t m = (a + e) / 2; if (seg_tmax[m] < lo[k]) a = m + 1; else e = m; }
    uint32_t b = a; e = g1;
    while (b < e) { const uint32_t m = (b + e) / 2; if (seg_tmin[m] <= hi[k]) b = m + 1; else e = m; }
    a_out[k] = a - g0; b_out[k] = b - g0;
}

__global__ void k_append_stats(const uint8_t *data, const uint64_t *off, const uint32_t *len, const uint32_t *rows, const int64_t *tmin,
                               const int64_t *tmax, uint32_t n_segments, uint32_t n_columns, unsigned long long *tot, uint32_t *max_rows,
                               long long *range, int *err) {
    const uint32_t g = blockIdx.x * blockDim.x + threadIdx.x;
    if (g >= n_segments) return;
    unsigned long long bytes = 0;
    for (uint32_t c = 0; c <= n_columns; c++) bytes += len[(size_t)c * n_segments + g];
    const size_t ti = (size_t)n_columns * n_segments + g;
    TimeDesc t;
    const int rc = parse_time_page(data + off[ti], len[ti], t);
    if (rc != D_OK) { if (atomicCAS(err, 0, rc) == 0) err[1] = (int)g; return; }
    atomicAdd(&tot[0], (unsigned long long)rows[g]);
    atomicAdd(&tot[1], bytes);
    if (t.kind != 0 && t.kind != 3) atomicAdd(&tot[2], 1ull);
    atomicMax(max_rows, rows[g]);
    atomicMin(&range[0], (long long)tmin[g]);
    atomicMax(&range[1], (long long)tmax[g]);
}

struct Spliced {
    uint32_t n = 0, n_columns = 0;
    uint64_t *off = nullptr; uint32_t *len = nullptr, *rows = nullptr, *series = nullptr; int64_t *tmin = nullptr, *tmax = nullptr;
    uint8_t *data = nullptr; uint64_t data_len = 0;
};
static int splice_and_gather(const SegSrc src[3], const std::vector<Run> &runs, uint32_t n_out, uint32_t n_columns,
                             const std::vector<const uint8_t *> &regions, Scratch &own, Spliced &out) {
    int rc;
    const uint64_t n_pages = (uint64_t)(n_columns + 1) * n_out;
    out.n = n_out; out.n_columns = n_columns;
    Scratch tmp;
    uint32_t *region; Run *d_runs;
    if ((rc = own.get(&out.off, n_pages)) || (rc = own.get(&out.len, n_pages)) || (rc = own.get(&out.rows, n_out)) ||
        (rc = own.get(&out.series, n_out)) || (rc = own.get(&out.tmin, n_out)) || (rc = own.get(&out.tmax, n_out)) ||
        (rc = tmp.get(&region, n_out)) || (rc = tmp.get(&d_runs, runs.size())))
        return rc;
    if (n_out) {
        CU(cudaMemcpy(d_runs, runs.data(), runs.size() * sizeof(Run), cudaMemcpyHostToDevice));
        SpliceP p;
        for (int k = 0; k < 3; k++) p.src[k] = src[k];
        p.runs = d_runs; p.n_runs = (uint32_t)runs.size(); p.n_out = n_out; p.n_columns = n_columns;
        p.off = out.off; p.len = out.len; p.rows = out.rows; p.series = out.series; p.region = region; p.tmin = out.tmin; p.tmax = out.tmax;
        k_append_splice<<<(n_out + 127) / 128, 128>>>(p);
    }
    if (std::all_of(runs.begin(), runs.end(), [](const Run &r) { return r.kind == SRC_FILES; })) { CU(cudaGetLastError()); return OG_OK; }
    uint64_t *sizes, *dst_off; const uint8_t **d_regions;
    if ((rc = tmp.get(&sizes, n_pages + 1)) || (rc = tmp.get(&dst_off, n_pages + 1)) || (rc = tmp.get(&d_regions, regions.size()))) return rc;
    CU(cudaMemcpy(d_regions, regions.data(), regions.size() * sizeof(void *), cudaMemcpyHostToDevice));
    k_append_sizes<<<(unsigned)((n_pages + 1 + 255) / 256), 256>>>(out.len, n_pages, sizes);
    {
        size_t tb = 0; void *t = nullptr;
        CU(cub::DeviceScan::ExclusiveSum(nullptr, tb, sizes, dst_off, n_pages + 1));
        if ((rc = tmp.get((uint8_t **)&t, tb))) return rc;
        CU(cub::DeviceScan::ExclusiveSum(t, tb, sizes, dst_off, n_pages + 1));
    }
    CU(cudaGetLastError());
    CU(cudaMemcpy(&out.data_len, dst_off + n_pages, 8, cudaMemcpyDeviceToHost));
    if ((rc = own.get(&out.data, out.data_len + 1024))) return rc;
    CU(cudaMemset(out.data + out.data_len, 0, 1024));
    if (n_pages)
        k_append_gather<<<(unsigned)((n_pages * 32 + APPEND_GATHER_THREADS - 1) / APPEND_GATHER_THREADS), APPEND_GATHER_THREADS>>>(
            d_regions, region, out.off, out.len, dst_off, n_out, n_pages, out.data);
    CU(cudaGetLastError());
    CU(cudaMemcpy(out.off, dst_off, n_pages * 8, cudaMemcpyDeviceToDevice));
    CU(cudaDeviceSynchronize());
    return OG_OK;
}


static int add_files(og_shard *s, const og_shard_desc *files, const uint32_t *file_flags, uint32_t n_files, const char *who) {
    int rc;
    const uint32_t onc = s->n_columns, ONSER = s->n_series, ONSEG = s->n_segments;
    std::map<std::string, int32_t> schema;
    for (uint32_t c = 0; c < onc; c++) schema[s->col_names[c]] = s->col_types[c];
    if (schema.size() != onc) { set_error("the shard holds two columns of one name"); return OG_E_UNSUPPORTED; }
    std::map<uint64_t, uint32_t> series_of_sid;
    if ((rc = scan_files(files, n_files, who, schema, series_of_sid))) return rc;
    std::map<uint64_t, uint32_t> old_of_sid;
    for (uint32_t i = 0; i < ONSER; i++) {
        if (!old_of_sid.emplace(s->sids[i], i).second) { set_error("the shard holds sid %llu twice", (unsigned long long)s->sids[i]); return OG_E_UNSUPPORTED; }
        series_of_sid[s->sids[i]] = 0;
    }
    std::vector<std::string> names; std::vector<int32_t> types;
    for (auto &kv : schema) { names.push_back(kv.first); types.push_back(kv.second); }
    std::vector<uint64_t> sids;
    for (auto &kv : series_of_sid) { kv.second = (uint32_t)sids.size(); sids.push_back(kv.first); }
    const uint32_t nc = (uint32_t)names.size(), NSER = (uint32_t)sids.size();
    std::vector<int32_t> col_of_old(nc, -1), identity(nc);
    for (uint32_t c = 0; c < onc; c++) col_of_old[std::lower_bound(names.begin(), names.end(), s->col_names[c]) - names.begin()] = (int32_t)c;
    for (uint32_t c = 0; c < nc; c++) identity[c] = (int32_t)c;
    std::vector<int64_t> old_of(NSER, -1);
    for (auto &kv : old_of_sid) old_of[series_of_sid[kv.first]] = kv.second;
    FileDir fd;
    if ((rc = build_file_dir(files, n_files, names, fd))) return rc;
    const uint32_t NN = fd.n;
    std::vector<std::vector<uint32_t>> ordered(NSER), ooo(NSER);
    og_merge_info info{}; info.n_files = n_files;
    if ((rc = split_segments(files, n_files, file_flags, fd, series_of_sid, sids, ordered, ooo, info))) return rc;
    std::vector<uint32_t> probe_u, probe_old; std::vector<int64_t> probe_lo, probe_hi;
    std::vector<int64_t> span_lo(NSER, INT64_MAX), span_hi(NSER, INT64_MIN);
    for (uint32_t u = 0; u < NSER; u++) {
        span_hull(ooo[u], fd, &span_lo[u], &span_hi[u]);
        if (old_of[u] >= 0 && (!ordered[u].empty() || !ooo[u].empty())) {
            probe_u.push_back(u); probe_old.push_back((uint32_t)old_of[u]); probe_lo.push_back(span_lo[u]); probe_hi.push_back(span_hi[u]);
        }
    }
    const uint32_t NP = (uint32_t)probe_u.size();
    std::vector<uint32_t> old_a(NSER, 0), old_b(NSER, 0);
    {
        Scratch t;
        uint32_t *d_ser, *d_a, *d_b; int64_t *d_lo, *d_hi, *d_last;
        if ((rc = t.get(&d_ser, NP)) || (rc = t.get(&d_lo, NP)) || (rc = t.get(&d_hi, NP)) || (rc = t.get(&d_last, NP)) || (rc = t.get(&d_a, NP)) || (rc = t.get(&d_b, NP))) return rc;
        if (NP) {
            CU(cudaMemcpy(d_ser, probe_old.data(), NP * 4ull, cudaMemcpyHostToDevice));
            CU(cudaMemcpy(d_lo, probe_lo.data(), NP * 8ull, cudaMemcpyHostToDevice));
            CU(cudaMemcpy(d_hi, probe_hi.data(), NP * 8ull, cudaMemcpyHostToDevice));
            k_append_probe<<<(NP + 127) / 128, 128>>>(s->d_series_seg_begin, s->d_tmin, s->d_tmax, d_ser, d_lo, d_hi, NP, d_last, d_a, d_b);
            CU(cudaGetLastError());
            std::vector<int64_t> last(NP); std::vector<uint32_t> a(NP), b(NP);
            CU(cudaMemcpy(last.data(), d_last, NP * 8ull, cudaMemcpyDeviceToHost));
            CU(cudaMemcpy(a.data(), d_a, NP * 4ull, cudaMemcpyDeviceToHost));
            CU(cudaMemcpy(b.data(), d_b, NP * 4ull, cudaMemcpyDeviceToHost));
            for (uint32_t k = 0; k < NP; k++) {
                const uint32_t u = probe_u[k];
                if (!ordered[u].empty() && fd.tmin[ordered[u][0]] <= last[k]) {
                    set_error("series sid %llu: ordered file %u starts at %lld, not after the shard's last time %lld; only out-of-order files may overlap the shard",
                              (unsigned long long)sids[u], fd.src_file[ordered[u][0]], (long long)fd.tmin[ordered[u][0]], (long long)last[k]);
                    return OG_E_UNSUPPORTED;
                }
                old_a[u] = a[k]; old_b[u] = b[k];
            }
        }
    }
    auto n_old = [&](uint32_t u) { return old_of[u] < 0 ? 0u : s->h_series_seg_begin[old_of[u] + 1] - s->h_series_seg_begin[old_of[u]]; };
    auto g0_old = [&](uint32_t u) { return old_of[u] < 0 ? 0u : s->h_series_seg_begin[old_of[u]]; };
    std::vector<uint32_t> before(NSER), after_begin(NSER);
    std::vector<int> span_of(NSER, -1);
    std::vector<Span> span_store;
    for (uint32_t u = 0; u < NSER; u++) {
        const uint32_t no = n_old(u);
        const auto &o = ordered[u];
        if (ooo[u].empty()) { before[u] = after_begin[u] = no + (uint32_t)o.size(); continue; }
        uint32_t na, nb;
        span_bounds(o, fd, span_lo[u], span_hi[u], &na, &nb);
        before[u] = old_a[u] < no ? old_a[u] : no + na;
        after_begin[u] = old_b[u] < no ? old_b[u] : no + nb;
        Span sp; sp.series = u;
        span_of[u] = (int)span_store.size();
        span_store.push_back(std::move(sp));
    }
    std::unique_ptr<og_shard> nw;
    std::vector<uint32_t> new_rows;
    if ((rc = upload_files(files, n_files, names, types, s->device, fd, nw, new_rows))) return rc;
    {
        std::lock_guard<std::mutex> il_lock(s->il_mu);
        for (og_shard::IlCol &c : s->il)
            dev_free_all(c.words, c.grp_off, c.grp_rows, c.grp_col, c.lane_seg, c.lane_rows, c.lane_series, c.lane_win, c.lane_t0, c.lane_dt, c.gen_list);
        s->il.assign(s->n_columns, og_shard::IlCol{});
    }
    Scratch d_maps;
    int32_t *d_col_old, *d_identity;
    if ((rc = d_maps.get(&d_col_old, nc)) || (rc = d_maps.get(&d_identity, nc))) return rc;
    CU(cudaMemcpy(d_col_old, col_of_old.data(), nc * 4ull, cudaMemcpyHostToDevice));
    CU(cudaMemcpy(d_identity, identity.data(), nc * 4ull, cudaMemcpyHostToDevice));
    SegSrc src[3] = {};
    src[SRC_SHARD] = SegSrc{s->d_page_off, s->d_page_len, s->d_seg_rows, s->d_tmin, s->d_tmax, nullptr, 0, d_col_old, ONSEG, onc};
    src[SRC_FILES] = SegSrc{nw->d_page_off, nw->d_page_len, nw->d_seg_rows, nw->d_tmin, nw->d_tmax, nullptr, 1, d_identity, NN, nc};
    cudaEvent_t ev0, ev1;
    CU(cudaEventCreate(&ev0)); CU(cudaEventCreate(&ev1));
    struct FreeEv { cudaEvent_t a, b; ~FreeEv() { cudaEventDestroy(a); cudaEventDestroy(b); } } free_ev{ev0, ev1};
    CU(cudaEventRecord(ev0, 0));
    std::vector<NewSegs> batches;
    Scratch blobs, msrc_own;
    if (!span_store.empty()) {
        std::vector<Run> runs;
        uint32_t n_src = 0;
        for (auto &sp : span_store) {
            const uint32_t u = sp.series, no = n_old(u);
            const auto &o = ordered[u];
            const uint32_t ob = std::min(before[u], no), oe = std::min(after_begin[u], no);
            if (oe > ob) {
                runs.push_back(Run{n_src, g0_old(u) + ob, 0, SRC_SHARD});
                for (uint32_t k = 0; k < oe - ob; k++) { sp.src.push_back(n_src + k); sp.src_file.push_back(n_files); }
                n_src += oe - ob;
            }
            std::vector<uint32_t> news;
            for (uint32_t k = std::max(before[u], no); k < after_begin[u]; k++) news.push_back(o[k - no]);
            news.insert(news.end(), ooo[u].begin(), ooo[u].end());
            sort_oldest_first(news, fd, file_flags);
            for (uint32_t g : news) {
                runs.push_back(Run{n_src, g, 0, SRC_FILES});
                sp.src.push_back(n_src++); sp.src_file.push_back(fd.src_file[g]);
            }
            info.series_merged++;
            info.segments_rewritten_in += sp.src.size();
        }
        for (uint32_t u = 0; u < NSER; u++) for (uint32_t g : ooo[u]) info.out_of_order_rows += new_rows[g];
        Spliced ms;
        if ((rc = splice_and_gather(src, runs, n_src, nc, {s->d_data, nw->d_data}, msrc_own, ms))) return rc;
        {
            std::vector<uint32_t> rows(n_src);
            CU(cudaMemcpy(rows.data(), ms.rows, n_src * 4ull, cudaMemcpyDeviceToHost));
            for (auto &sp : span_store)
                for (uint32_t i : sp.src) { sp.src_rows.push_back(rows[i]); sp.rows += rows[i]; }
        }
        SrcDir dir;
        dir.data = ms.data ? ms.data : nw->d_data; dir.page_off = ms.off; dir.page_len = ms.len; dir.seg_rows = ms.rows; dir.n_segments = ms.n; dir.n_columns = nc;
        std::vector<Span *> sp;
        for (auto &x : span_store) sp.push_back(&x);
        uint64_t replaced = 0;
        if ((rc = merge_spans(dir, runs, types, names, sp, sids, n_files, batches, blobs, &replaced))) return rc;
        info.rows_replaced = replaced;
    }
    std::vector<uint32_t> m_first(batches.size() + 1, 0);
    for (size_t b = 0; b < batches.size(); b++) m_first[b + 1] = m_first[b] + batches[b].n;
    const uint32_t NM = m_first[batches.size()];
    std::vector<const uint8_t *> regions = {s->d_data, nw->d_data};
    Scratch m_own;
    if (NM) {
        std::vector<uint64_t> off((size_t)(nc + 1) * NM); std::vector<uint32_t> len((size_t)(nc + 1) * NM), rows(NM), reg(NM);
        std::vector<int64_t> tmin(NM), tmax(NM);
        for (size_t b = 0; b < batches.size(); b++) {
            const NewSegs &B = batches[b];
            regions.push_back(B.blob);
            for (uint32_t g = 0; g < B.n; g++) {
                const uint32_t m = m_first[b] + g;
                for (uint32_t c = 0; c <= nc; c++) { off[(size_t)c * NM + m] = B.off[(size_t)c * B.n + g]; len[(size_t)c * NM + m] = B.len[(size_t)c * B.n + g]; }
                rows[m] = B.rows[g]; reg[m] = 2 + (uint32_t)b; tmin[m] = B.tmin[g]; tmax[m] = B.tmax[g];
            }
        }
        SegSrc &m = src[SRC_MERGED];
        uint64_t *d_off; uint32_t *d_len, *d_rows, *d_reg; int64_t *d_tmin, *d_tmax;
        if ((rc = m_own.get(&d_off, off.size())) || (rc = m_own.get(&d_len, len.size())) || (rc = m_own.get(&d_rows, NM)) || (rc = m_own.get(&d_reg, NM)) ||
            (rc = m_own.get(&d_tmin, NM)) || (rc = m_own.get(&d_tmax, NM)))
            return rc;
        CU(cudaMemcpy(d_off, off.data(), off.size() * 8, cudaMemcpyHostToDevice));
        CU(cudaMemcpy(d_len, len.data(), len.size() * 4, cudaMemcpyHostToDevice));
        CU(cudaMemcpy(d_rows, rows.data(), NM * 4ull, cudaMemcpyHostToDevice));
        CU(cudaMemcpy(d_reg, reg.data(), NM * 4ull, cudaMemcpyHostToDevice));
        CU(cudaMemcpy(d_tmin, tmin.data(), NM * 8ull, cudaMemcpyHostToDevice));
        CU(cudaMemcpy(d_tmax, tmax.data(), NM * 8ull, cudaMemcpyHostToDevice));
        m = SegSrc{d_off, d_len, d_rows, d_tmin, d_tmax, d_reg, 0, d_identity, NM, nc};
    }
    std::vector<Run> runs;
    std::vector<uint32_t> o_ssb(NSER + 1, 0);
    uint32_t NOUT = 0;
    auto emit = [&](uint32_t u, uint32_t k0, uint32_t k1) {
        const uint32_t no = n_old(u);
        if (std::min(k1, no) > k0) { runs.push_back(Run{NOUT, g0_old(u) + k0, u, SRC_SHARD}); NOUT += std::min(k1, no) - k0; }
        for (uint32_t k = std::max(k0, no); k < k1; k++) runs.push_back(Run{NOUT++, ordered[u][k - no], u, SRC_FILES});
        info.segments_kept += k1 - k0;
    };
    for (uint32_t u = 0; u < NSER; u++) {
        o_ssb[u] = NOUT;
        const uint32_t total = n_old(u) + (uint32_t)ordered[u].size();
        emit(u, 0, before[u]);
        if (span_of[u] >= 0) {
            const Span &sp = span_store[span_of[u]];
            if (sp.n_new) { runs.push_back(Run{NOUT, m_first[sp.batch] + sp.first_new, u, SRC_MERGED}); NOUT += sp.n_new; }
            info.segments_rewritten_out += sp.n_new;
        }
        emit(u, after_begin[u], total);
    }
    o_ssb[NSER] = NOUT;
    std::unique_ptr<og_shard> out(new og_shard);
    Scratch out_own;
    Spliced sd;
    if ((rc = splice_and_gather(src, runs, NOUT, nc, regions, out_own, sd))) return rc;
    if (!sd.data) { sd.data = nw->d_data; sd.data_len = nw->data_len; nw->d_data = nullptr; out_own.bufs.push_back(sd.data); }
    CU(cudaEventRecord(ev1, 0));
    {
        Scratch t;
        unsigned long long *d_tot; uint32_t *d_max; long long *d_range; int *d_err;
        if ((rc = t.get(&d_tot, 3)) || (rc = t.get(&d_max, 1)) || (rc = t.get(&d_range, 2)) || (rc = t.get(&d_err, 2))) return rc;
        const long long r0[2] = {INT64_MAX, INT64_MIN};
        CU(cudaMemset(d_tot, 0, 24)); CU(cudaMemset(d_max, 0, 4)); CU(cudaMemset(d_err, 0, 8));
        CU(cudaMemcpy(d_range, r0, 16, cudaMemcpyHostToDevice));
        if (NOUT) k_append_stats<<<(NOUT + 127) / 128, 128>>>(sd.data, sd.off, sd.len, sd.rows, sd.tmin, sd.tmax, NOUT, nc, d_tot, d_max, d_range, d_err);
        CU(cudaGetLastError());
        unsigned long long tot[3]; long long range[2]; int err[2];
        CU(cudaMemcpy(tot, d_tot, 24, cudaMemcpyDeviceToHost));
        CU(cudaMemcpy(&out->max_seg_rows, d_max, 4, cudaMemcpyDeviceToHost));
        CU(cudaMemcpy(range, d_range, 16, cudaMemcpyDeviceToHost));
        CU(cudaMemcpy(err, d_err, 8, cudaMemcpyDeviceToHost));
        if (err[0]) { set_error("segment %d: time page failed to parse after the append (device code %d)", err[1], err[0]); return OG_E_CORRUPT; }
        out->n_rows = tot[0]; out->page_bytes = tot[1]; out->irregular_time_pages = tot[2]; out->tmin = range[0]; out->tmax = range[1];
    }
    out->rows_merged = s->rows_merged || !batches.empty();
    if (!out->rows_merged) {
        out->snappy_pages = s->snappy_pages + nw->snappy_pages;
        out->snappy_bytes_in = s->snappy_bytes_in + nw->snappy_bytes_in; out->snappy_bytes_out = s->snappy_bytes_out + nw->snappy_bytes_out;
    }
    out->page_bytes = out->page_bytes - out->snappy_bytes_out + out->snappy_bytes_in;
    out->device = s->device; out->n_series = NSER; out->n_segments = NOUT; out->n_columns = nc;
    out->sids = sids; out->col_types = types; out->col_names = names; out->h_series_seg_begin = o_ssb;
    if ((rc = dalloc(&out->d_series_seg_begin, (size_t)NSER + 1)) || (rc = dalloc(&out->d_sids, (size_t)NSER))) return rc;
    CU(cudaMemcpy(out->d_series_seg_begin, o_ssb.data(), ((size_t)NSER + 1) * 4, cudaMemcpyHostToDevice));
    CU(cudaMemcpy(out->d_sids, sids.data(), (size_t)NSER * 8, cudaMemcpyHostToDevice));
    float ms = 0;
    CU(cudaEventElapsedTime(&ms, ev0, ev1));
    info.merge_ms = ms;
    info.rows_after_merge = out->n_rows;
    auto take = [](Scratch &own, void *p) { own.bufs.erase(std::find(own.bufs.begin(), own.bufs.end(), p)); };
    for (void *p : {(void *)sd.off, (void *)sd.len, (void *)sd.rows, (void *)sd.series, (void *)sd.tmin, (void *)sd.tmax, (void *)sd.data}) take(out_own, p);
    out->d_page_off = sd.off; out->d_page_len = sd.len; out->d_seg_rows = sd.rows; out->d_seg_series = sd.series; out->d_tmin = sd.tmin; out->d_tmax = sd.tmax;
    out->d_data = sd.data; out->data_len = sd.data_len; out->owns_data = true;
    out->merge = info;
    CU(cudaDeviceSynchronize());
    std::swap(static_cast<ShardState &>(*s), static_cast<ShardState &>(*out));
    {
        std::lock_guard<std::mutex> il_lock(s->il_mu);
        s->il.assign(s->n_columns, og_shard::IlCol{});
    }
    return OG_OK;
}

}

using namespace ogpu;

extern "C" {

OG_API int og_shard_open_files(const og_shard_desc *files, const uint32_t *file_flags, uint32_t n_files, og_shard **out) {
    if (!files || !out || n_files == 0) { set_error("null argument or no files"); return OG_E_INVAL; }
    *out = nullptr;
    int rc = ensure_device(); if (rc) return rc;
    std::unique_ptr<og_shard> s(new og_shard);
    CU(cudaGetDevice(&s->device));
    s->h_series_seg_begin = {0};
    if ((rc = add_files(s.get(), files, file_flags, n_files, "og_shard_open_files"))) return rc;
    *out = s.release();
    return OG_OK;
}

OG_API int og_shard_append_files(og_shard *s, const og_shard_desc *files, const uint32_t *file_flags, uint32_t n_files) {
    if (!s || !files || n_files == 0) { set_error("null argument or no files"); return OG_E_INVAL; }
    std::lock_guard<std::mutex> lock(s->live->mu);
    if (s->live->n) { set_error("%u queries on this shard are still open: destroy them before appending files", s->live->n); return OG_E_STATE; }
    CU(cudaSetDevice(s->device));
    return add_files(s, files, file_flags, n_files, "og_shard_append_files");
}

OG_API int og_shard_merge_info(const og_shard *s, og_merge_info *out) {
    if (!s || !out) { set_error("null argument"); return OG_E_INVAL; }
    *out = s->merge;
    return OG_OK;
}

}
```

Baseline: 500.4 billion.

## Fetch only live interleaved words, skip padded gcell columns, self-clear gcells

The fused interleaved-decode kernel now bulk-copies only the live words of each group instead of the padded row count, trimming TMA traffic. The gcell fold walks only the populated rank ranges per super-block and clears ok flags as it reads them, so the per-chunk gcell memsets move to a once-per-query clear guarded by a dirty flag. The edge-fold kernel becomes a grid-stride loop with a capped block count, and a fetch-bytes statistic is added. The risks are correctness of the partial-copy sizes and of the self-clearing invariant across queries.

Result: faster. 512.6 billion (median of 6 runs) (+2.4%).

```diff
diff --git a/include/ogpu.h b/include/ogpu.h
--- a/include/ogpu.h
+++ b/include/ogpu.h
@@ -156,6 +156,7 @@
     uint64_t general_segments;
     double merge_ms;
     uint64_t il_packed_segments;
+    uint64_t il_fetch_bytes;
 } og_stats;
 
 typedef struct og_shard og_shard;
diff --git a/opengemini_b200/_lib.py b/opengemini_b200/_lib.py
--- a/opengemini_b200/_lib.py
+++ b/opengemini_b200/_lib.py
@@ -73,7 +73,7 @@
                 ("dir_bytes", C.c_uint64), ("out_bytes", C.c_uint64), ("kernel_ms", C.c_double), ("h2d_ms", C.c_double), ("main_kernel_ms", C.c_double),
                 ("kernel_launches", C.c_uint32), ("path", C.c_int32), ("il_state", C.c_int32), ("per_series_cells_used", C.c_int32),
                 ("il_build_ms", C.c_double), ("il_bytes", C.c_uint64), ("general_segments", C.c_uint64), ("merge_ms", C.c_double),
-                ("il_packed_segments", C.c_uint64)]
+                ("il_packed_segments", C.c_uint64), ("il_fetch_bytes", C.c_uint64)]
 
 
 class SynthColumn(C.Structure):
diff --git a/opengemini_b200/csrc/agg_kernels.cuh b/opengemini_b200/csrc/agg_kernels.cuh
--- a/opengemini_b200/csrc/agg_kernels.cuh
+++ b/opengemini_b200/csrc/agg_kernels.cuh
@@ -25,6 +25,7 @@
     uint32_t *edge_bucket;
     Tri gcells[OG_MAX_CALLS];
     uint32_t gc_cols, gc_tail0, gc_edge0, gc_col0;
+    uint32_t gc_blk_cols, gc_blk_ranks, gc_last_ranks;
     uint32_t J;
     int *err;
     int *flags;
@@ -336,11 +337,7 @@
 __device__ __forceinline__ bool call_has_time(const QueryP &q, uint32_t c) { return q.calls[c].func >= OG_AGG_MIN && !(q.multi && q.calls[c].func <= OG_AGG_MAX); }
 __device__ __forceinline__ int call_ftype(const QueryP &q, uint32_t c) { return q.calls[c].func == OG_AGG_COUNT ? OG_TYPE_INT : q.calls[c].type; }
 
-__global__ void k_fix_edges_fold(DirP d, QueryP q, ChunkP ch) {
-    if (ch.flags[1] == 0) return;
-    const uint32_t w = (blockIdx.x * blockDim.x + threadIdx.x) >> 5, lane = threadIdx.x & 31;
-    const uint32_t n_blk = (ch.series_end - ch.series_begin + 31) / 32;
-    if (w >= n_blk * ch.J) return;
+__device__ __forceinline__ void fix_edges_fold_warp(const DirP &d, const QueryP &q, const ChunkP &ch, uint32_t w, uint32_t lane) {
     const uint32_t blk = w / ch.J, j = w % ch.J;
     const uint32_t series = ch.series_begin + blk * 32 + lane;
     const bool in = series < ch.series_end;
@@ -369,6 +366,15 @@
     }
 }
 
+#define OG_FIX_FOLD_BLOCKS 2048u
+__global__ void k_fix_edges_fold(DirP d, QueryP q, ChunkP ch) {
+    if (ch.flags[1] == 0) return;
+    const uint32_t lane = threadIdx.x & 31;
+    const uint32_t n_blk = (ch.series_end - ch.series_begin + 31) / 32;
+    for (uint32_t w = (blockIdx.x * blockDim.x + threadIdx.x) >> 5; w < n_blk * ch.J; w += (gridDim.x * blockDim.x) >> 5)
+        fix_edges_fold_warp(d, q, ch, w, lane);
+}
+
 struct GroupP {
     const uint32_t *grp_begin;
     const uint32_t *grp_series;
@@ -472,16 +478,38 @@
     const Tri g = ch.gcells[c];
     Part acc = part_empty();
     const size_t row = (size_t)b * ch.gc_cols;
-    for (uint32_t col = lane; col < ch.gc_cols; col += 32) {
-        if (!g.ok[row + col]) continue;
-        Part p; p.ok = 1; p.v = g.val[row + col]; p.t = wt ? g.tim[row + col] : 0;
-        group_update(func, ftype, multi, acc, p);
-    }
+    Part dn; dn.ok = 0; dn.v = 0; dn.t = 0;
+    if (lane == 0) dn = load_part(gp.dense[c], b);
+    auto walk = [&](uint32_t c0, uint32_t c1) {
+        constexpr uint32_t U = 4;
+        for (uint32_t col = c0 + ((lane - c0) & 31u); col < c1; col += 32 * U) {
+            uint8_t okv[U]; uint64_t vv[U]; int64_t tt[U];
+#pragma unroll
+            for (uint32_t u = 0; u < U; u++) okv[u] = col + 32 * u < c1 ? g.ok[row + col + 32 * u] : 0;
+#pragma unroll
+            for (uint32_t u = 0; u < U; u++) { vv[u] = okv[u] ? g.val[row + col + 32 * u] : 0; tt[u] = okv[u] && wt ? g.tim[row + col + 32 * u] : 0; }
+#pragma unroll
+            for (uint32_t u = 0; u < U; u++) {
+                if (!okv[u]) continue;
+                g.ok[row + col + 32 * u] = 0;
+                Part p; p.ok = 1; p.v = vv[u]; p.t = tt[u];
+                group_update(func, ftype, multi, acc, p);
+            }
+        }
+    };
+    if (ch.gc_blk_cols) {
+        const uint32_t n_blk = ch.gc_tail0 / ch.gc_blk_cols;
+        for (uint32_t half = 0; half < 2; half++)
+            for (uint32_t k = 0; k < n_blk; k++) {
+                const uint32_t c0 = half * ch.gc_tail0 + k * ch.gc_blk_cols;
+                walk(c0, c0 + (k + 1 < n_blk ? ch.gc_blk_ranks : ch.gc_last_ranks));
+            }
+    }
+    if (!ch.gc_blk_cols || ch.flags[1]) walk(ch.gc_edge0, ch.gc_cols);
     acc = warp_fold(func, ftype, multi, acc, wt);
     if (lane == 0 && acc.ok) {
-        Part a = load_part(gp.dense[c], b);
-        group_update(func, ftype, multi, a, acc);
-        store_part(gp.dense[c], b, a);
+        group_update(func, ftype, multi, dn, acc);
+        store_part(gp.dense[c], b, dn);
     }
 }
 
diff --git a/opengemini_b200/csrc/api.cu b/opengemini_b200/csrc/api.cu
--- a/opengemini_b200/csrc/api.cu
+++ b/opengemini_b200/csrc/api.cu
@@ -573,7 +573,7 @@
     const size_t n_slots = (size_t)ng * 32;
     if ((rc = dalloc(&ic.lane_seg, n_slots)) || (rc = dalloc(&ic.lane_rows, n_slots)) || (rc = dalloc(&ic.lane_win, n_slots)) || (rc = dalloc(&ic.lane_series, n_slots)) ||
         (rc = dalloc(&ic.lane_t0, n_slots)) || (rc = dalloc(&ic.lane_dt, n_slots)) || (rc = dalloc(&ic.grp_col, (size_t)ng)) ||
-        (rc = dalloc(&ic.grp_rows, (size_t)ng)) || (rc = dalloc(&ic.grp_off, (size_t)ng))) return rc;
+        (rc = dalloc(&ic.grp_rows, (size_t)ng)) || (rc = dalloc(&ic.grp_live, (size_t)ng)) || (rc = dalloc(&ic.grp_off, (size_t)ng))) return rc;
     CU(cudaMemsetAsync(ic.lane_seg, 0xff, n_slots * 4, st));
     CU(cudaMemsetAsync(ic.lane_rows, 0, n_slots * 4, st));
     CU(cudaMemsetAsync(ic.lane_win, 0, n_slots * 2, st));
@@ -583,13 +583,15 @@
     as.lane_seg = ic.lane_seg; as.lane_rows = ic.lane_rows; as.lane_series = ic.lane_series; as.grp_col = ic.grp_col; as.lane_win = ic.lane_win; as.lane_t0 = ic.lane_t0; as.lane_dt = ic.lane_dt;
     as.n_elig = (uint32_t)n_elig; as.J = J; as.cols_per_super = ic.cols_per_super;
     k_il_assign<<<(unsigned)((n_elig + 255) / 256), 256, 0, st>>>(d, as);
-    k_il_group_rows<<<(unsigned)((n_slots + 255) / 256), 256, 0, st>>>(ng, ic.lane_seg, seg_words, ic.grp_rows);
+    k_il_group_rows<<<(unsigned)((n_slots + 255) / 256), 256, 0, st>>>(ng, ic.lane_seg, seg_words, ic.grp_rows, ic.grp_live);
     CU(cudaGetLastError());
-    std::vector<uint32_t> gw(ng); std::vector<uint64_t> go(ng);
+    std::vector<uint32_t> gw(ng), gl(ng); std::vector<uint64_t> go(ng);
     CU(cudaMemcpyAsync(gw.data(), ic.grp_rows, (size_t)ng * 4, cudaMemcpyDeviceToHost, st));
+    CU(cudaMemcpyAsync(gl.data(), ic.grp_live, (size_t)ng * 4, cudaMemcpyDeviceToHost, st));
     CU(cudaStreamSynchronize(st));
     uint64_t total = 0;
-    for (uint32_t g = 0; g < ng; g++) { go[g] = total; total += (uint64_t)gw[g] * 32; }
+    ic.live_first.assign(ng + 1, 0);
+    for (uint32_t g = 0; g < ng; g++) { go[g] = total; total += (uint64_t)gw[g] * 32; ic.live_first[g + 1] = ic.live_first[g] + gl[g]; }
     size_t free_b = 0, total_b = 0;
     CU(dev_mem_info(&free_b, &total_b));
     size_t headroom = (size_t)8 << 30;
@@ -712,21 +714,25 @@
             if ((rc = q->bufs.get(&ch.gcells[c].val, n))) return rc;
             if ((rc = q->bufs.get(&ch.gcells[c].ok, n))) return rc;
             if (sel && (rc = q->bufs.get(&ch.gcells[c].tim, n))) return rc;
+            CU(cudaMemsetAsync(ch.gcells[c].ok, 0, n, st));
         }
     }
     if (pl->fold) {
         ch.gc_tail0 = ic->n_super * ic->cols_per_super; ch.gc_edge0 = 2 * ch.gc_tail0; ch.gc_col0 = 0;
         ch.gc_cols = ch.gc_edge0 + 3 * ((s->n_series + 31) / 32);
+        ch.gc_blk_cols = ic->cols_per_super; ch.gc_blk_ranks = OG_IL_SUPER / 32;
+        ch.gc_last_ranks = (s->n_series - (ic->n_super - 1) * OG_IL_SUPER + 31) / 32;
         const size_t n = (size_t)p.n_buckets * ch.gc_cols;
         for (uint32_t c = 0; c < p.n_calls; c++) {
             bool sel = p.calls[c].func >= OG_AGG_MIN;
             if ((rc = q->bufs.get(&ch.gcells[c].val, n))) return rc;
             if ((rc = q->bufs.get(&ch.gcells[c].ok, n))) return rc;
             if (sel && (rc = q->bufs.get(&ch.gcells[c].tim, n))) return rc;
+            CU(cudaMemsetAsync(ch.gcells[c].ok, 0, n, st));
         }
     }
     if (pl->fast) {
-        pl->il.words = ic->words; pl->il.grp_off = ic->grp_off; pl->il.grp_rows = ic->grp_rows; pl->il.grp_col = ic->grp_col;
+        pl->il.words = ic->words; pl->il.grp_off = ic->grp_off; pl->il.grp_live = ic->grp_live; pl->il.grp_col = ic->grp_col;
         pl->il.lane_seg = ic->lane_seg; pl->il.lane_rows = ic->lane_rows; pl->il.lane_win = ic->lane_win; pl->il.lane_series = ic->lane_series; pl->il.lane_t0 = ic->lane_t0; pl->il.lane_dt = ic->lane_dt;
         pl->fm = 0; pl->times = false;
         for (uint32_t c = 0; c < p.n_calls; c++) {
@@ -782,6 +788,11 @@
     const bool per_series = q->desc.group_mode == OG_GROUP_PER_SERIES;
     if (!per_series) { k_init_dense<<<(unsigned)((cells_dense + 255) / 256), 256, 0, st>>>(p, gp); launches++; }
     const bool clear_cells = !pl->fold || q->cells_dirty || n_chunks > 1;
+    if (pl->fold || pl->blockmerge) {
+        if (q->gcells_dirty) for (uint32_t c = 0; c < p.n_calls; c++) CU(cudaMemsetAsync(ch.gcells[c].ok, 0, (size_t)p.n_buckets * ch.gc_cols, st));
+        q->gcells_dirty = true;
+    }
+    uint64_t fetch_rows = 0;
     uint64_t segs_scanned = 0; uint32_t ci = 0, chunks_run = 0;
     for (uint32_t a = 0; a < s->n_series; a += q->chunk_series, ci++) {
         if (q->aborted) { cudaStreamSynchronize(st); set_error("query aborted"); return OG_E_ABORTED; }
@@ -800,7 +811,6 @@
         }
         segs_scanned += nseg;
         if (clear_cells) for (uint32_t c = 0; c < p.n_calls; c++) CU(cudaMemsetAsync(ch.cells[c].ok, 0, chunk_cells, st));
-        if (pl->fold || pl->blockmerge) for (uint32_t c = 0; c < p.n_calls; c++) CU(cudaMemsetAsync(ch.gcells[c].ok, 0, (size_t)p.n_buckets * ch.gc_cols, st));
         if (pl->fold && ci > 0) CU(cudaMemsetAsync(ch.flags + 1, 0, sizeof(int), st));
         CU(cudaEventRecord(q->main_ev[2 * chunks_run], st));
         if (pl->fused) {
@@ -810,6 +820,7 @@
                 uint32_t g0 = 0, g1 = ic.n_groups;
                 if (ic.J) { g0 = ic.super_grp_first[a / OG_IL_SUPER]; g1 = ic.super_grp_first[std::min<uint32_t>(ic.n_super, (b + OG_IL_SUPER - 1) / OG_IL_SUPER)]; }
                 launch_fast(pl->fm, pl->times, pl->fold, pl->il, g0, g1, p, ch, st); launches++;
+                fetch_rows += ic.live_first[g1] - ic.live_first[g0];
                 auto lo = std::lower_bound(ic.gen_host.begin(), ic.gen_host.end(), ch.seg_begin);
                 auto hi = std::lower_bound(ic.gen_host.begin(), ic.gen_host.end(), ch.seg_end);
                 gl = ic.gen_list + (lo - ic.gen_host.begin()); gn = (uint32_t)(hi - lo);
@@ -846,7 +857,7 @@
         }
         CU(cudaEventRecord(q->main_ev[2 * chunks_run + 1], st));
         chunks_run++;
-        if (pl->fold) k_fix_edges_fold<<<(unsigned)(((size_t)((b - a + 31) / 32) * ch.J * 32 + 127) / 128), 128, 0, st>>>(dir, p, ch);
+        if (pl->fold) k_fix_edges_fold<<<(unsigned)std::min<size_t>(OG_FIX_FOLD_BLOCKS, ((size_t)((b - a + 31) / 32) * ch.J * 32 + 127) / 128), 128, 0, st>>>(dir, p, ch);
         else k_fix_edges<<<(nseg + 127) / 128, 128, 0, st>>>(dir, p, ch);
         if (per_series) k_merge_per_series<<<dim3((unsigned)((chunk_cells + 255) / 256), p.n_calls), 256, 0, st>>>(p, ch, gp);
         else if (pl->blockmerge) k_merge_all_blocks<<<dim3((p.n_buckets + 127) / 128, (b - a + OG_MERGE_SB - 1) / OG_MERGE_SB, p.n_calls), 128, 0, st>>>(p, ch, gp);
@@ -857,6 +868,7 @@
     CU(cudaEventRecord(q->ev1, st));
     CU(cudaGetLastError());
     CU(cudaStreamSynchronize(st));
+    q->gcells_dirty = false;
     int err[16];
     CU(cudaMemcpy(err, q->d_err, 64, cudaMemcpyDeviceToHost));
     if (getenv("OGPU_IL_STATS")) {
@@ -883,6 +895,7 @@
     if (p.n_cols == 1 && p.col_type[0] == OG_TYPE_FLOAT && p.col_index[0] < (int)s->il.size()) {
         const og_shard::IlCol &ic = s->il[p.col_index[0]];
         stt.il_state = ic.state; stt.il_build_ms = ic.build_ms; stt.il_bytes = ic.n_words * 4; stt.il_packed_segments = ic.state == 1 ? ic.n_packed : 0;
+        stt.il_fetch_bytes = fetch_rows * 128;
         stt.general_segments = ic.state == 1 ? (uint64_t)ic.gen_host.size() : s->n_segments;
     }
     stt.per_series_cells_used = err[2] != 0;
diff --git a/opengemini_b200/csrc/fused_il.cuh b/opengemini_b200/csrc/fused_il.cuh
--- a/opengemini_b200/csrc/fused_il.cuh
+++ b/opengemini_b200/csrc/fused_il.cuh
@@ -58,7 +58,7 @@
 struct IlP {
     const uint32_t *words;
     const uint64_t *grp_off;
-    const uint32_t *grp_rows;
+    const uint32_t *grp_live;
     const uint32_t *grp_col;
     const uint32_t *lane_seg;
     const uint32_t *lane_rows;
@@ -129,8 +129,7 @@
     const uint32_t wid = __reduce_max_sync(FULL, threadIdx.x >> 5);
     const uint32_t grp = grp_begin + blockIdx.x * WPB + wid;
     if (grp >= grp_end) return;
-    const uint32_t rows_w = __reduce_max_sync(FULL, il.grp_rows[grp]);
-    if (rows_w == 0) return;
+    const uint32_t live = __reduce_max_sync(FULL, il.grp_live[grp]);
     const size_t slot = (size_t)grp * 32 + lane;
     const uint32_t seg = il.lane_seg[slot];
     bool active = seg != OG_IL_NONE && seg >= ch.seg_begin && seg < ch.seg_end;
@@ -164,7 +163,7 @@
         mbar_init_fence();
     }
     __syncwarp();
-    const uint32_t total_b = rows_w / B;
+    const uint32_t total_b = (live + B - 1) / B;
     uint64_t goff = il.grp_off[grp];
     goff = ((uint64_t)__reduce_max_sync(FULL, (uint32_t)(goff >> 32)) << 32) | __reduce_max_sync(FULL, (uint32_t)goff);
     const uint32_t *gsrc = il.words + goff;
@@ -176,15 +175,17 @@
         const uint32_t k = __reduce_max_sync(FULL, k_any);
         const uint32_t s = k % NB, dst = win + s * (B * 128), bar = bar0 + s * 8;
         const uint32_t *src = gsrc + (size_t)k * (B * 32);
-        if (s == 0)
+        const uint32_t n = live - k * B < B ? live - k * B : B;
+        if (s == 0) {
+            const uint32_t nm = n < 2 ? n : 2u;
             asm volatile("{\n.reg .pred p;\nelect.sync _|p, 0xffffffff;\n@p mbarrier.arrive.expect_tx.shared::cta.b64 _, [%0], %1;\n"
                          "@p cp.async.bulk.shared::cluster.global.mbarrier::complete_tx::bytes.L2::cache_hint [%2], [%3], %4, [%0], %6;\n"
-                         "@p cp.async.bulk.shared::cluster.global.mbarrier::complete_tx::bytes.L2::cache_hint [%5], [%3], 256, [%0], %6;\n}"
-                         ::"r"(bar), "r"(B * 128 + 256u), "r"(dst), "l"(src), "r"(B * 128), "r"(win + NW * 128), "l"(pol) : "memory");
-        else
+                         "@p cp.async.bulk.shared::cluster.global.mbarrier::complete_tx::bytes.L2::cache_hint [%5], [%3], %7, [%0], %6;\n}"
+                         ::"r"(bar), "r"((n + nm) * 128), "r"(dst), "l"(src), "r"(n * 128), "r"(win + NW * 128), "l"(pol), "r"(nm * 128) : "memory");
+        } else
             asm volatile("{\n.reg .pred p;\nelect.sync _|p, 0xffffffff;\n@p mbarrier.arrive.expect_tx.shared::cta.b64 _, [%0], %1;\n"
                          "@p cp.async.bulk.shared::cluster.global.mbarrier::complete_tx::bytes.L2::cache_hint [%2], [%3], %1, [%0], %4;\n}"
-                         ::"r"(bar), "r"(B * 128), "r"(dst), "l"(src), "l"(pol) : "memory");
+                         ::"r"(bar), "r"(n * 128), "r"(dst), "l"(src), "l"(pol) : "memory");
     };
     {
         const uint32_t first = total_b < NB ? total_b : NB;
@@ -312,6 +313,7 @@
         if (skipping) { skipping = false; sum = 0.0; }
         else {
             fin = stop > r_hi;
+            if (fin && CE != 0 && qp + sr > 32u * live) bad = 1;
             sum = 0.0;
             if (!fin) while (stop >= rb) {
                 cur_b++;
@@ -395,7 +397,7 @@
 #pragma unroll 1
         while (issued_b < total_b && (issued_b + 1) * B <= f + NW) { issue(issued_b); issued_b++; }
         const uint32_t qmax = __reduce_max_sync(FULL, done ? 0u : qp);
-        uint32_t need_max = ((qmax + OG_IL_LOOKBITS) >> 5) + 1; if (need_max > rows_w) need_max = rows_w;
+        uint32_t need_max = ((qmax + OG_IL_LOOKBITS) >> 5) + 1; if (need_max > live) need_max = live;
         uint32_t want_b = (need_max + B - 1) / B; if (want_b > issued_b) want_b = issued_b;
 #ifdef OG_IL_STATS
         st_w0 = clock64();
@@ -406,7 +408,7 @@
         st_wait += clock64() - st_w0;
 #endif
         if (hung) break;
-        uint32_t need = ((qp + OG_IL_LOOKBITS) >> 5) + 1; if (need > rows_w) need = rows_w;
+        uint32_t need = ((qp + OG_IL_LOOKBITS) >> 5) + 1; if (need > live) need = live;
         bool go = done || need <= ready_b * B;
         uint32_t run = __reduce_min_sync(FULL, go ? n_ev : 0u);
         if (run >= K) {
@@ -454,7 +456,6 @@
             if (__all_sync(FULL, ev || done)) break;
         }
     }
-    if (active && (qp >> 5) >= rows_w) bad = 1;
 #ifdef OG_IL_STATS
     const long long st_e0 = clock64();
     if (lane == 0) { atomicAdd((unsigned *)&ch.err[4], st_common); atomicAdd((unsigned *)&ch.err[5], st_rare); atomicAdd((unsigned *)&ch.err[6], st_notgo); atomicAdd((unsigned *)&ch.err[7], st_sit); }
diff --git a/opengemini_b200/csrc/il_build.cuh b/opengemini_b200/csrc/il_build.cuh
--- a/opengemini_b200/csrc/il_build.cuh
+++ b/opengemini_b200/csrc/il_build.cuh
@@ -104,14 +104,14 @@
     if ((rank & 31) == 0) a.grp_col[g] = (a.J ? dom / a.J : 0u) * a.cols_per_super + rank / 32;
 }
 
-__global__ void k_il_group_rows(uint32_t n_groups, const uint32_t *lane_seg, const uint32_t *seg_words, uint32_t *grp_rows) {
+__global__ void k_il_group_rows(uint32_t n_groups, const uint32_t *lane_seg, const uint32_t *seg_words, uint32_t *grp_rows, uint32_t *grp_live) {
     uint32_t g = (blockIdx.x * blockDim.x + threadIdx.x) >> 5, lane = threadIdx.x & 31;
     if (g >= n_groups) return;
     uint32_t seg = lane_seg[(size_t)g * 32 + lane];
     uint32_t w = seg != OG_IL_NONE ? seg_words[seg] : 0;
 #pragma unroll
     for (int o = 16; o; o >>= 1) w = max(w, __shfl_xor_sync(0xffffffffu, w, o));
-    if (lane == 0) grp_rows[g] = (w + OG_IL_B - 1) / OG_IL_B * OG_IL_B;
+    if (lane == 0) { grp_rows[g] = (w + OG_IL_B - 1) / OG_IL_B * OG_IL_B; grp_live[g] = w - OG_IL_PAD_WORDS; }
 }
 
 __global__ void k_il_repack(DirP d, int col, const uint32_t *lane_seg, const uint16_t *lane_win, const uint64_t *grp_off, const uint32_t *grp_rows,
diff --git a/opengemini_b200/csrc/internal.h b/opengemini_b200/csrc/internal.h
--- a/opengemini_b200/csrc/internal.h
+++ b/opengemini_b200/csrc/internal.h
@@ -80,12 +80,13 @@
     void *d_seg_buf = nullptr; size_t d_seg_buf_bytes = 0;
     std::vector<og_colval_view> seg_views;
     struct IlCol { int state = 0;
-                   uint32_t *words = nullptr; uint64_t *grp_off = nullptr; uint32_t *grp_rows = nullptr, *grp_col = nullptr;
+                   uint32_t *words = nullptr; uint64_t *grp_off = nullptr; uint32_t *grp_rows = nullptr, *grp_live = nullptr, *grp_col = nullptr;
                    uint32_t *lane_seg = nullptr, *lane_rows = nullptr, *lane_series = nullptr; uint16_t *lane_win = nullptr; int64_t *lane_t0 = nullptr; uint64_t *lane_dt = nullptr;
                    uint32_t *gen_list = nullptr; std::vector<uint32_t> gen_host;
                    uint32_t n_groups = 0, J = 0;
                    bool aligned = false;
                    uint32_t n_super = 1, cols_per_super = 0; std::vector<uint32_t> super_grp_first;
+                   std::vector<uint64_t> live_first;
                    uint64_t n_words = 0, n_packed = 0;  double build_ms = 0; };
     std::vector<IlCol> il;
     std::mutex il_mu;
@@ -96,7 +97,7 @@
         dev_free_all(d_series_seg_begin, d_seg_series, d_seg_rows, d_tmin, d_tmax, d_page_off, d_page_len, d_sids, d_seg_buf);
         if (h_seg_buf) cudaFreeHost(h_seg_buf);
         for (IlCol &c : il)
-            dev_free_all(c.words, c.grp_off, c.grp_rows, c.grp_col, c.lane_seg, c.lane_rows, c.lane_series, c.lane_win, c.lane_t0, c.lane_dt, c.gen_list);
+            dev_free_all(c.words, c.grp_off, c.grp_rows, c.grp_live, c.grp_col, c.lane_seg, c.lane_rows, c.lane_series, c.lane_win, c.lane_t0, c.lane_dt, c.gen_list);
     }
 };
 
@@ -146,6 +147,7 @@
     std::vector<og_colval_view> rv_cols;
     int path_used = 0;
     bool cells_dirty = true;
+    bool gcells_dirty = false;
     bool planned = false;
     uint32_t chunk_series = 0, tile_segs = 0;
     int *d_err = nullptr;
diff --git a/opengemini_b200/csrc/merge.cu b/opengemini_b200/csrc/merge.cu
--- a/opengemini_b200/csrc/merge.cu
+++ b/opengemini_b200/csrc/merge.cu
@@ -641,7 +641,7 @@
     {
         std::lock_guard<std::mutex> il_lock(s->il_mu);
         for (og_shard::IlCol &c : s->il)
-            dev_free_all(c.words, c.grp_off, c.grp_rows, c.grp_col, c.lane_seg, c.lane_rows, c.lane_series, c.lane_win, c.lane_t0, c.lane_dt, c.gen_list);
+            dev_free_all(c.words, c.grp_off, c.grp_rows, c.grp_live, c.grp_col, c.lane_seg, c.lane_rows, c.lane_series, c.lane_win, c.lane_t0, c.lane_dt, c.gen_list);
         s->il.assign(s->n_columns, og_shard::IlCol{});
     }
     Scratch d_maps;
```
